# NSLab-CUK/LiteralKG

Measured on AMD Instinct MI355X. Metric: kg_edges_aggregated_per_sec, higher is better.
Workload: dtype f32

## Files before the change

### include/literalkg_hip.h

```cpp
#ifndef LITERALKG_HIP_H
#define LITERALKG_HIP_H

#include <stdint.h>

#ifdef __cplusplus
extern "C" {
#endif

typedef enum {
    LKG_OK = 0,
    LKG_ERR_INVALID_ARG = -1,
    LKG_ERR_HIP = -2,
    LKG_ERR_UNSUPPORTED = -3,
    LKG_ERR_NOMEM = -4
} lkg_status;

int lkg_version(void);
const char *lkg_last_error(void);
int lkg_preload(void);

int lkg_csr_build(int64_t n_entities, int64_t n_edges, const int64_t *h, const int64_t *t,
                  const int64_t *r, int32_t *rowptr, int32_t *col, int32_t *eptr, int32_t *rel,
                  int64_t *order, int64_t *nnz_out);

int lkg_csr_transpose(int64_t n_rows, int64_t n_cols, int64_t nnz, const int32_t *rowptr,
                      const int32_t *col, int32_t *t_rowptr, int32_t *t_col, int32_t *t_perm);

int64_t lkg_csr_build_device_workspace(int64_t n_entities, int64_t n_edges);
int lkg_csr_build_device(int64_t n_entities, int64_t n_edges, const int64_t *h, const int64_t *t, const int64_t *r,
                         int32_t *rowptr, int32_t *col, int32_t *eptr, int32_t *rel, int32_t *order,
                         int64_t *counts, void *workspace, int64_t workspace_bytes, void *stream);
int64_t lkg_csr_transpose_device_workspace(int64_t n_cols, int64_t nnz);
int lkg_csr_transpose_device(int64_t n_rows, int64_t n_cols, int64_t nnz, const int32_t *rowptr, const int32_t *col,
                             int32_t *t_rowptr, int32_t *t_col, int32_t *t_perm, void *workspace,
                             int64_t workspace_bytes, void *stream);

int lkg_csr_coo_indices_i64(int64_t n_rows, int64_t nnz, const int32_t *rowptr, const int32_t *col,
                            int64_t *indices_out, void *stream);

int lkg_row_partition(int64_t n_rows, const int32_t *rowptr, int32_t n_parts, int64_t *cuts);

int lkg_triples_count(const char *path, int64_t *n_lines);
int lkg_triples_read(const char *path, int64_t capacity, int64_t *h, int64_t *r, int64_t *t,
                     int64_t *n_read);
int lkg_triples_dedup(int64_t n, const int64_t *h, const int64_t *r, const int64_t *t, int64_t *keep,
                      int64_t *n_keep);
int lkg_laplacian_f32(int64_t n_entities, int64_t n_raw, int64_t nnz, const int32_t *rowptr,
                      const int32_t *col, const int32_t *eptr, const int32_t *rel, int32_t kind,
                      float *val_out);
int lkg_laplacian_device_f32(int64_t n_entities, int64_t nnz, int32_t n_rel, const int32_t *rowptr, const int32_t *col,
                             const int32_t *eptr, const int32_t *rel, int32_t kind, int32_t *deg_workspace,
                             float *val_out, void *stream);

int lkg_spmm_csr_f32(int64_t n_rows, int32_t d, const int32_t *rowptr, const int32_t *col,
                     const float *val, const float *x, int64_t ldx, float *out, int64_t ldo,
                     const float *self, int64_t ld_self, const int32_t *long_rows, int32_t n_long,
                     int32_t long_thresh, void *stream);

int lkg_spmm_csr_fused_f32(int64_t n_rows, int32_t d, const int32_t *rowptr, const int32_t *col,
                           const float *val, const float *x, int64_t ldx, float *out, int64_t ldo,
                           const float *self, int64_t ld_self, const float *add2, int64_t ld_add2,
                           const uint8_t *add2_rows, const float *copy_src, int64_t ld_copy_src, float *copy_dst,
                           int64_t ld_copy_dst, float *rowmax_out, const uint8_t *x_rows, const uint8_t *self_rows,
                           uint8_t *out_rows, const int32_t *long_rows, int32_t n_long, int32_t long_thresh,
                           const int32_t *rows_with_entries, int64_t n_rows_with_entries,
                           const int32_t *rows_without_entries, int64_t n_rows_without_entries, void *stream);

int lkg_csr_extract_rows(int64_t n_sel, const int64_t *sel_rows, const int32_t *rowptr, const int32_t *col,
                         const float *val, const int32_t *out_rowptr, int32_t *out_col, float *out_val,
                         void *stream);
int lkg_spmm_csr_scatter_bwd_f32(int64_t n_rows, int32_t d, const int32_t *rowptr, const int32_t *col,
                                 const float *val, const float *g_out, int64_t ldg, float *g_x,
                                 int64_t ldx, void *stream);

int lkg_edge_softmax_f32(int64_t n_rows, int64_t row_offset, int32_t d, const int32_t *rowptr,
                         const int32_t *col, const int32_t *eptr, const int32_t *rel,
                         const int32_t *rel_first, const int32_t *dup_entries,
                         const int32_t *dup_rows, int32_t n_dup, int64_t entry_lo, int64_t entry_hi,
                         const float *ent, int64_t ld_ent, const float *relemb, int64_t ld_rel,
                         float *val_out, float *logits_out, const int32_t *long_rows, int32_t n_long,
                         int32_t long_thresh, int32_t n_rel, void *stream);

int lkg_permute_f32(int64_t n, const int32_t *perm, int64_t n_src, const float *src, float *dst, void *stream);

int lkg_csr_check_i32(int64_t n_rows, const int32_t *rowptr, int64_t nnz, const int32_t *col, int64_t col_offset,
                      int64_t n_cols, int32_t *bad_out, void *stream);

int lkg_transe_score_fwd_f32(int64_t batch, int32_t dim, const float *emb, int64_t ld_emb,
                             const float *relemb, int64_t ld_rel, const int64_t *h,
                             const int64_t *r, const int64_t *pos_t, const int64_t *neg_t,
                             float *pos, float *neg, float *reg, float *rank, void *stream);

int lkg_loss_reduce_f32(int64_t batch, const float *rank, const float *reg, float lambda,
                        float *loss_out, void *stream);

int lkg_transe_score_bwd_f32(int64_t batch, int32_t dim, const float *emb, int64_t ld_emb,
                             const float *relemb, int64_t ld_rel, const int64_t *h,
                             const int64_t *r, const int64_t *pos_t, const int64_t *neg_t,
                             const float *pos, const float *neg, float lambda,
                             const float *g_loss, float *g_emb, int64_t ld_gemb, float *g_rel,
                             int64_t ld_grel, void *stream);

int lkg_group_by_key_i64(int64_t n, int32_t n_keys, const int64_t *keys, int32_t *perm, int32_t *seg,
                         int32_t *n_bad, void *stream);
int lkg_gather_rows_f32(int64_t n, int32_t d, const float *src, int64_t lds, const int64_t *idx,
                        const int32_t *perm, float *dst, int64_t ldd, void *stream);
int lkg_scatter_add_rows_f32(int64_t n, int32_t d, const float *src, int64_t lds, const int64_t *idx,
                             const int32_t *perm, float *dst, int64_t ldd, void *stream);
int lkg_fill_rows_f32(int64_t n, int32_t d, const int64_t *idx, float *dst, int64_t ldd, float value, uint8_t *flags,
                      int32_t flag, void *stream);
int lkg_gather_rows_range_f32(int64_t n, int32_t d, const float *src, int64_t lds, const int64_t *idx,
                              int64_t row_lo, int64_t row_hi, float *dst, int64_t ldd, void *stream);
int lkg_scatter_add_rows_range_f32(int64_t n, int32_t d, const float *src, int64_t lds, const int64_t *idx,
                                   int64_t row_lo, int64_t row_hi, float *dst, int64_t ldd, void *stream);
int lkg_gather_i64(int64_t n, const int64_t *src, const int32_t *perm, int64_t *dst, void *stream);

int lkg_sample_kg_batch(int64_t n_groups, int32_t neg_rate, uint64_t seed, const int64_t *heads,
                        int64_t n_entities, const int32_t *rowptr, const int32_t *col, const int32_t *eptr, const int32_t *rel,
                        int64_t nnz, int64_t n_raw, int64_t *out_h, int64_t *out_r, int64_t *out_pos_t,
                        int64_t *out_neg_t, void *stream);

int lkg_grouped_gemm_f32(int32_t mode, int32_t n_groups, const int32_t *seg, int64_t max_seg_len,
                         int32_t trans_a, int32_t trans_b, int64_t m, int64_t n, int64_t k, float alpha,
                         const float *a, int64_t lda, const float *b, int64_t ldb, int64_t stride_b,
                         int32_t b_period, float beta, float *c, int64_t ldc, int64_t stride_c, void *stream);

int lkg_dot_score_fwd_f32(int64_t batch, int32_t dim, const float *emb, int64_t ld_emb, const int64_t *h,
                          const int64_t *pos_t, const int64_t *neg_t, float *pos, float *neg, float *reg,
                          float *rank, void *stream);
int lkg_dot_score_bwd_f32(int64_t batch, int32_t dim, const float *emb, int64_t ld_emb, const int64_t *h,
                          const int64_t *pos_t, const int64_t *neg_t, const float *pos, const float *neg,
                          float lambda, const float *g_loss, float *g_emb, int64_t ld_gemb, void *stream);

int lkg_relu_batchnorm_fwd_f32(int64_t n, int32_t d, const float *z, int64_t ldz, const float *gamma,
                               const float *beta, float eps, int32_t training, float momentum,
                               float *running_mean, float *running_var, float *y, int64_t ldy,
                               float *save_mean, float *save_invstd, void *stream);
int lkg_relu_batchnorm_bwd_f32(int64_t n, int32_t d, const float *z, int64_t ldz, const float *gamma,
                               const float *save_mean, const float *save_invstd, int32_t training,
                               const float *g_y, int64_t ldgy, float *g_z, int64_t ldgz, float *g_gamma,
                               float *g_beta, void *stream);

int lkg_dense_score_fwd_f32(int64_t batch, int32_t rows_per_group, int32_t dim, const float *ph, const float *pp,
                            const float *pn, int64_t ld, const float *relemb, int64_t ld_rel,
                            const int64_t *r, float *pos, float *neg, float *reg, float *rank,
                            void *stream);
int lkg_dense_score_bwd_f32(int64_t batch, int32_t rows_per_group, int32_t dim, const float *ph, const float *pp,
                            const float *pn, int64_t ld, const float *relemb, int64_t ld_rel,
                            const int64_t *r, const float *pos, const float *neg, float lambda,
                            const float *g_loss, float *g_ph, float *g_pp, float *g_pn,
                            int64_t ldg, float *g_rel, int64_t ld_grel, void *stream);
int lkg_check_grouped_i64(int64_t n, int32_t rows_per_group, const int64_t *h, const int64_t *r,
                          const int64_t *pos_t, int32_t *n_bad, void *stream);
int lkg_expand_groups_i32(int64_t n_groups, int32_t rows_per_group, int32_t n_seg, const int32_t *perm,
                          const int32_t *seg, int32_t *perm_out, int32_t *seg_out, void *stream);

int lkg_sanitize_ids_i64(int64_t n, const int64_t *ids, int64_t lo, int64_t hi, int64_t *out, int32_t *n_bad,
                         void *stream);

int lkg_act_layernorm_fwd_f32(int64_t n, int32_t d, const float *z, int64_t ldz, float slope,
                              const float *gamma, const float *beta, float eps, float *y,
                              int64_t ldy, float *yn, int64_t ldyn, float norm_eps,
                              float *save_mean, float *save_rstd, float drop_p, uint64_t seed,
                              void *stream);

int lkg_act_layernorm_bwd_f32(int64_t n, int32_t d, const float *z, int64_t ldz, float slope,
                              const float *gamma, const float *beta, const float *y, int64_t ldy,
                              const float *save_mean, const float *save_rstd, const float *g_y,
                              int64_t ldgy, const float *g_yn, int64_t ldgyn, float norm_eps,
                              float *g_z, int64_t ldgz, float *g_gamma, float *g_beta,
                              float drop_p, uint64_t seed, float *g_z_rowmax, const uint8_t *g_yn_rows,
                              int32_t sparse_out, const int64_t *row_ids, int64_t n_row_ids, void *stream);

int lkg_gate_blend_fwd_f32(int64_t n, int32_t d, const float *x, int64_t ldx, const float *gpre,
                           int64_t ldg, const float *zpre, int64_t ldz, float *out, int64_t ldo,
                           void *stream);
int lkg_gate_blend_bwd_f32(int64_t n, int32_t d, const float *x, int64_t ldx, const float *gpre,
                           int64_t ldg, const float *zpre, int64_t ldz, const float *g_out,
                           int64_t ldgo, float *g_x, int64_t ldgx, float *g_gpre, int64_t ldgg,
                           float *g_zpre, int64_t ldgz, int32_t activated, float *g_pre_rowmax, void *stream);

int lkg_gate_blend_bwd_stats_f32(int64_t n, int32_t d, const float *x, int64_t ldx, const float *gpre, int64_t ldg,
                                 const float *zpre, int64_t ldz, const float *g_out, int64_t ldgo, float *g_x,
                                 int64_t ldgx, float *g_gpre, int64_t ldgg, float *g_zpre, int64_t ldgz,
                                 int32_t activated, float *g_pre_rowmax, const float *w, int64_t ldw, int32_t n_w,
                                 float *workspace, int64_t workspace_floats, float *stats, void *stream);

int lkg_gemm_wgrad_f32(int64_t m, int64_t n, int64_t k, const float *a, int64_t lda, const float *a_colmax,
                       const float *b, int64_t ldb, const float *b_colmax, float *c, int64_t ldc, void *stream);
int lkg_gemm_longk_ok(int64_t m, int64_t n, int64_t k, const float *a, int64_t lda, const float *b, int64_t ldb);
int lkg_gemm_longk_f32(int64_t m, int64_t n, int64_t k, const float *a, int64_t lda, const float *b, int64_t ldb,
                       float *c, int64_t ldc, void *stream);
int lkg_gemm_smallm_ok(int64_t m, int64_t n, int64_t k, const float *a, int64_t lda, const float *b, int64_t ldb);
int lkg_gemm_smallm_f32(int64_t m, int64_t n, int64_t k, const float *a, int64_t lda, const float *b, int64_t ldb,
                        float *c, int64_t ldc, void *stream);

int64_t lkg_narrow_layer_bwd_workspace(int64_t n);
int lkg_narrow_layer_bwd_ok(int64_t n, int32_t d_in, int32_t d_out, const float *x, int64_t ldx, const float *z, int64_t ldz,
                            const float *y, int64_t ldy, const float *g_y, int64_t ldgy, const float *g_yn, int64_t ldgyn);
int lkg_narrow_layer_bwd_f32(int64_t n, int32_t d_in, int32_t d_out, const float *x, int64_t ldx, const float *w, int64_t ldw,
                             const float *z, int64_t ldz, float slope, const float *gamma, const float *y, int64_t ldy,
                             const float *save_mean, const float *save_rstd, const float *g_y, int64_t ldgy,
                             const float *g_yn, int64_t ldgyn, float norm_eps, float drop_p, uint64_t seed,
                             const uint8_t *g_yn_rows, float *g_x, int64_t ldgx, float *g_w, float *g_bias,
                             float *g_gamma, float *g_beta, float *workspace, int64_t workspace_floats, void *stream);
int lkg_gemm_skinny_ok(int64_t m, int64_t n, int64_t k, const float *a, int64_t lda, const float *c, int64_t ldc);
int lkg_gemm_skinny_f32(int64_t m, int64_t n, int64_t k, const float *a, int64_t lda, const float *b, int64_t ldb,
                        int32_t trans_b, float beta, float *c, int64_t ldc, const float *bias, void *stream);
int lkg_col_absmax_f32(int64_t n, int32_t d, const float *x, int64_t ldx, float *out, void *stream);

int lkg_colsum_f32(int64_t n, int32_t d, const float *x, int64_t ldx, float *out, void *stream);
int lkg_colsum_weighted_f32(int64_t n, int32_t d, const float *x, int64_t ldx, const float *w, int64_t ldw,
                            int32_t n_w, float *out_sum, float *out_w, int64_t ld_out_w, void *stream);

int lkg_bi_mix_fwd_f32(int64_t n, int32_t d, const float *ego, int64_t lde, const float *side, int64_t lds,
                       const float *h0p, int64_t ldh, float alpha, float *out_sum, int64_t ldos, float *out_prod,
                       int64_t ldop, void *stream);
int lkg_bi_mix_bwd_f32(int64_t n, int32_t d, const float *ego, int64_t lde, const float *side, int64_t lds,
                       const float *g_sum, int64_t ldgs, const float *g_prod, int64_t ldgp, int32_t has_h0, float alpha,
                       float *g_ego, float *g_side, float *g_h0p, void *stream);

int lkg_eltwise_f32(int32_t op, int64_t n, int32_t d, const float *a, int64_t lda, const float *b,
                    int64_t ldb, float alpha, float beta, float *out, int64_t ldo, void *stream);

int lkg_adam_step_f32(int64_t n, float *param, const float *grad, float *exp_avg, float *exp_avg_sq,
                      float lr, float beta1, float beta2, float eps, float weight_decay, int64_t step,
                      void *stream);

int64_t lkg_gemm_workspace(int32_t trans_a, int64_t m, int64_t n, int64_t k);
int lkg_gemm_f32_engine(int32_t trans_a, int32_t trans_b, int64_t m, int64_t n, int64_t k, int64_t workspace_bytes);

int lkg_gemm_f64acc_f32(int32_t trans_a, int32_t trans_b, int64_t m, int64_t n, int64_t k, const float *a, int64_t lda,
                        const float *b, int64_t ldb, float *c, int64_t ldc, void *stream);
int lkg_gemm_f32(int32_t trans_a, int32_t trans_b, int64_t m, int64_t n, int64_t k, float alpha,
                 const float *a, int64_t lda, const float *b, int64_t ldb, float beta, float *c,
                 int64_t ldc, const float *bias, void *workspace, int64_t workspace_bytes, void *stream);

int lkg_row_absmax_f32(int64_t n, int32_t d, const float *x, int64_t ldx, float *out, int32_t accumulate,
                       void *stream);
int64_t lkg_gemm_tall_workspace(int32_t n, int32_t n_panels, const int32_t *ka, int32_t epilogue);
int lkg_gemm_tall_f32(int64_t m, int32_t n, int32_t n_panels, const float *const *a, const int64_t *lda,
                      const int32_t *ka, const float *a_rowmax, int32_t n_groups, const float *const *b,
                      const int64_t *ldb, int32_t trans_b, float alpha, float beta, float *c, int64_t ldc,
                      const float *bias, int32_t epilogue, const float *gate_x, int64_t ld_x, float *gate_g,
                      int64_t ld_g, float *gate_z, int64_t ld_z, void *workspace, int64_t workspace_bytes,
                      void *stream);

int64_t lkg_linear_act_layernorm_workspace(int32_t n, int32_t n_panels, const int32_t *ka);
int lkg_linear_act_layernorm_fwd_f32(int64_t m, int32_t n, int32_t n_panels, const float *const *a, const int64_t *lda,
                                     const int32_t *ka, const float *a_rowmax, const float *const *w, const int64_t *ldw,
                                     const float *bias, float slope, const float *gamma, const float *beta, float eps,
                                     float *y, int64_t ldy, float *yn, int64_t ldyn, float norm_eps, float *save_mean,
                                     float *save_rstd, float drop_p, uint64_t seed, void *workspace,
                                     int64_t workspace_bytes, void *stream);

int lkg_rank_sqnorm_f32(int64_t n, int32_t k, const float *p, int64_t ldp, float *out, void *stream);
int lkg_rank_queries_f32(int64_t n, int32_t k, const float *p, int64_t ldp, const int64_t *ids, const float *e,
                         int64_t lde, const int64_t *rel, float alpha, float *q, int64_t ldq, void *stream);
int lkg_rank_prepare_f32(int64_t n_q, int64_t n_cand, int32_t k, const float *q, int64_t ldq, const float *p,
                         int64_t ldp, const float *pn, const int64_t *truth, const int64_t *filter_row,
                         const int64_t *filter_rel, const int32_t *rowptr, const int32_t *col, const int32_t *eptr,
                         const int32_t *rel, float *thr, int32_t *better, int32_t *equal, void *stream);
int lkg_rank_count_f32(int64_t n_q, int64_t n_cand, int32_t k, const float *q, int64_t ldq, const float *p,
                       int64_t ldp, const float *pn, const float *thr, const int64_t *truth, int32_t *better,
                       int32_t *equal, void *stream);

#define LKG_TOPK_MAX 128
#define LKG_TOPK_MAX_SPLITS 64
int32_t lkg_topk_splits(int64_t n_q, int64_t n_cand, int32_t requested);
int lkg_topk_select_f32(int64_t n_q, int64_t n_cand, int32_t k, const float *q, int64_t ldq, const float *p,
                        int64_t ldp, const float *pn, const int64_t *cand_ids, const int64_t *filter_row,
                        const int64_t *filter_rel, const int32_t *rowptr, const int32_t *col, const int32_t *eptr,
                        const int32_t *rel, int32_t top_k, int32_t splits, float *ws_s, int32_t *ws_i, void *stream);
int lkg_topk_merge_f32(int64_t n_q, int32_t top_k, int32_t splits, const float *ws_s, const int32_t *ws_i,
                       const float *qn, int64_t *out_ids, float *out_scores, float *out_values, void *stream);

int lkg_accept_count_f32(int64_t n_q, int64_t n_cand, int32_t k, const float *q, int64_t ldq, const float *p,
                         int64_t ldp, const float *pn, const float *qn, const float *thr, int32_t higher,
                         const int64_t *cand_ids, const int64_t *filter_row, const int64_t *filter_rel,
                         const int32_t *rowptr, const int32_t *col, const int32_t *eptr, const int32_t *rel,
                         int32_t splits, int32_t *counts, void *stream);
int lkg_accept_emit_f32(int64_t n_q, int64_t n_cand, int32_t k, const float *q, int64_t ldq, const float *p,
                        int64_t ldp, const float *pn, const float *qn, const float *thr, int32_t higher,
                        const int64_t *cand_ids, const int64_t *filter_row, const int64_t *filter_rel,
                        const int32_t *rowptr, const int32_t *col, const int32_t *eptr, const int32_t *rel,
                        int32_t splits, const int32_t *counts, const int64_t *base, int32_t *cursor, int64_t *out_ids,
                        float *out_scores, float *out_values, int32_t *flag, void *stream);
int64_t lkg_accept_order_workspace(int64_t m, int64_t n_q);
int lkg_accept_order(int64_t m, int64_t n_q, int64_t id_bound, const int64_t *rowptr, const int64_t *ids,
                     const float *scores, const float *values, int64_t *out_ids, float *out_scores, float *out_values,
                     void *workspace, int64_t workspace_bytes, void *stream);

int lkg_pair_mlp_scores_f32(int64_t n_q, int64_t n_cand, const float *uq, int64_t ldu, const float *v, int64_t ldv,
                            const float *w2, const float *b2, const float *w3, const float *b3, float *out, int64_t ldo,
                            void *stream);
int32_t lkg_pair_mlp_splits(int64_t n_q, int64_t n_cand, int32_t requested);
int lkg_pair_mlp_select_f32(int64_t n_q, int64_t n_cand, const float *uq, int64_t ldu, const float *v, int64_t ldv,
                            const float *w2, const float *b2, const float *w3, const float *b3, const int64_t *cand_ids,
                            const int64_t *filter_row, const int64_t *filter_rel, const int32_t *rowptr,
                            const int32_t *col, const int32_t *eptr, const int32_t *rel, int32_t top_k, int32_t splits,
                            float *ws_s, int32_t *ws_i, void *stream);
int lkg_pair_mlp_prepare_f32(int64_t n_q, int64_t n_cand, const float *uq, int64_t ldu, const float *v, int64_t ldv,
                             const float *w2, const float *b2, const float *w3, const float *b3, const int64_t *truth,
                             int64_t n_rows, const int32_t *cand_slot, const int64_t *filter_row,
                             const int64_t *filter_rel, const int32_t *rowptr, const int32_t *col, const int32_t *eptr,
                             const int32_t *rel, float *thr, int32_t *better, int32_t *equal, void *stream);
int lkg_pair_mlp_count_f32(int64_t n_q, int64_t n_cand, const float *uq, int64_t ldu, const float *v, int64_t ldv,
                           const float *w2, const float *b2, const float *w3, const float *b3, const float *thr,
                           const int64_t *truth, int32_t *better, int32_t *equal, void *stream);

int lkg_pair_mlp_pairs_f32(int64_t n_pairs, const float *u, int64_t ldu, const float *v, int64_t ldv,
                           const int64_t *u_idx, const int64_t *v_idx, const float *w2, const float *b2, const float *w3,
                           const float *b3, const uint8_t *labels, float thr, float *out, int64_t *counts, void *stream);

int64_t lkg_binary_curve_workspace(int64_t n);
int lkg_binary_curve_f32(int64_t n, const float *scores, const uint8_t *labels, int64_t *out_counts, double *out_ap,
                         void *workspace, int64_t workspace_bytes, void *stream);

int lkg_triple_scores_f32(int64_t n, int32_t k, const float *p, int64_t ldp, const int64_t *q_idx, const int64_t *c_idx,
                          const float *pn, const float *e, int64_t lde, const int64_t *rel, float alpha, int32_t flags,
                          const uint8_t *labels, float thr, float *out, int64_t *counts, void *stream);

int64_t lkg_threshold_fit_workspace(int64_t n, int64_t n_relations);
int lkg_threshold_fit_f32(int64_t n, int64_t n_relations, const float *scores, const uint8_t *labels, const int64_t *rel,
                          int32_t lower_is_better, float *thr, int64_t *stats, void *workspace, int64_t workspace_bytes,
                          void *stream);

#define LKG_RELATION_MAX 4096
int lkg_relation_scores_f32(int64_t n, int32_t k, int32_t n_rel, const float *p, int64_t ldp, int64_t rel_stride,
                            const float *pn, int64_t pn_stride, const int64_t *q_idx, const int64_t *c_idx,
                            const float *e, int64_t lde, float alpha, float *out, int64_t ldo, void *stream);
int lkg_relation_order_f32(int64_t n, int32_t n_rel, const float *scores, int64_t lds, const int64_t *truth,
                           const int64_t *filter_row, const int64_t *filter_col, const int32_t *rowptr,
                           const int32_t *col, const int32_t *eptr, const int32_t *rel, int32_t top_k, int32_t *better,
                           int32_t *equal, int64_t *top_ids, float *top_scores, void *stream);

#define LKG_RETRIEVAL_SLICE 32
int lkg_retrieval_prepare_f32(int64_t n_rows, int64_t n_cand, int32_t k, const float *q, int64_t ldq,
                              const int64_t *row_q, const float *p, int64_t ldp, const float *pn, int64_t n_ids,
                              const int32_t *cand_slot, const int64_t *key_off, const int32_t *key_n,
                              const int64_t *qkey_off, const int64_t *qkey_n, const float *key_s, const int64_t *key_id,
                              const int64_t *filter_row, const int64_t *filter_rel, const int32_t *rowptr,
                              const int32_t *col, const int32_t *eptr, const int32_t *rel, int32_t *buckets,
                              void *stream);
int lkg_retrieval_count_f32(int64_t n_rows, int64_t n_cand, int32_t k, const float *q, int64_t ldq, const int64_t *row_q,
                            const float *p, int64_t ldp, const float *pn, const int64_t *cand_ids,
                            const int64_t *key_off, const int32_t *key_n, const float *key_s, const int64_t *key_id,
                            int32_t *buckets, void *stream);
int lkg_retrieval_finish(int64_t n_q, const int64_t *qkey_ptr, const int64_t *row_base, const int64_t *n_answers,
                         const int32_t *buckets, int32_t n_ks, const int64_t *ks, int64_t k_tab, const double *disc,
                         const double *icum, int64_t *before, int64_t *position, int64_t *hits, double *ndcg, double *ap,
                         double *rr, void *stream);

#define LKG_SOFTMAX_MAX_SPLITS 64
int32_t lkg_softmax_all_splits(int64_t n_q, int64_t n_cand, int32_t requested);
int lkg_softmax_all_partial_f32(int64_t n_q, int64_t n_cand, int32_t k, const float *q, int64_t ldq, const float *p,
                                int64_t ldp, const float *pn, float scale, int32_t splits, float *ws_m, float *ws_l,
                                void *stream);
int lkg_softmax_all_finish_f32(int64_t n_q, int64_t n_cand, int32_t k, const float *q, int64_t ldq, const float *p,
                               int64_t ldp, const float *pn, const int64_t *truth, float scale, int32_t splits,
                               const float *ws_m, const float *ws_l, float *lse, float *lse_lo, float *loss,
                               void *stream);
int lkg_softmax_all_weights_f32(int64_t n_q, int64_t n_cand, int32_t k, const float *q, int64_t ldq, const float *p,
                                int64_t ldp, const float *pn, int64_t c_base, const int64_t *truth, const float *lse,
                                const float *lse_lo, const float *g, float scale, float *v, int64_t ldv, void *stream);

int lkg_softmax_excluded(int64_t n_q, int64_t n_rows, int64_t n_cand, const int64_t *filter_row, const int64_t *filter_rel,
                         const int64_t *truth, const int32_t *rowptr, const int32_t *col, const int32_t *eptr,
                         const int32_t *rel, const int32_t *pos, int32_t *count, const int32_t *xptr, int32_t *xcol,
                         void *stream);
int lkg_softmax_all_partial_masked_f32(int64_t n_q, int64_t n_cand, int32_t k, const float *q, int64_t ldq, const float *p,
                                       int64_t ldp, const float *pn, float scale, int32_t splits, const int32_t *xptr,
                                       const int32_t *xcol, int64_t n_excl, float *ws_m, float *ws_l, void *stream);
int lkg_softmax_all_weights_masked_f32(int64_t n_q, int64_t n_cand, int32_t k, const float *q, int64_t ldq, const float *p,
                                       int64_t ldp, const float *pn, int64_t c_base, const int64_t *truth,
                                       const float *lse, const float *lse_lo, const float *g, float scale,
                                       const int32_t *xptr, const int32_t *xcol, int64_t n_excl, float *v, int64_t ldv,
                                       void *stream);

#ifdef __cplusplus
}
#endif
#endif
```

### literalkg_amd/_native.py

```python
import ctypes as C
import os

_LIB_PATH = os.path.join(os.path.dirname(os.path.abspath(__file__)), "lib", "liblkg_hip.so")
_lib = None

i64, i32, f32, vp, u64 = C.c_int64, C.c_int32, C.c_float, C.c_void_p, C.c_uint64

PROTOTYPES = {
    "lkg_version": [],
    "lkg_last_error": [],
    "lkg_preload": [],
    "lkg_csr_build": [i64, i64, vp, vp, vp, vp, vp, vp, vp, vp, vp],
    "lkg_csr_transpose": [i64, i64, i64, vp, vp, vp, vp, vp],
    "lkg_row_partition": [i64, vp, i32, vp],
    "lkg_csr_coo_indices_i64": [i64, i64, vp, vp, vp, vp],
    "lkg_csr_build_device_workspace": [i64, i64],
    "lkg_csr_build_device": [i64, i64, vp, vp, vp, vp, vp, vp, vp, vp, vp, vp, i64, vp],
    "lkg_csr_transpose_device_workspace": [i64, i64],
    "lkg_csr_transpose_device": [i64, i64, i64, vp, vp, vp, vp, vp, vp, i64, vp],
    "lkg_triples_count": [C.c_char_p, vp],
    "lkg_triples_read": [C.c_char_p, i64, vp, vp, vp, vp],
    "lkg_triples_dedup": [i64, vp, vp, vp, vp, vp],
    "lkg_laplacian_f32": [i64, i64, i64, vp, vp, vp, vp, i32, vp],
    "lkg_laplacian_device_f32": [i64, i64, i32, vp, vp, vp, vp, i32, vp, vp, vp],
    "lkg_spmm_csr_f32": [i64, i32, vp, vp, vp, vp, i64, vp, i64, vp, i64, vp, i32, i32, vp],
    "lkg_spmm_csr_fused_f32": [i64, i32, vp, vp, vp, vp, i64, vp, i64, vp, i64, vp, i64, vp, vp, i64, vp, i64, vp, vp,
                               vp, vp, vp, i32, i32, vp, i64, vp, i64, vp],
    "lkg_csr_extract_rows": [i64, vp, vp, vp, vp, vp, vp, vp, vp],
    "lkg_spmm_csr_scatter_bwd_f32": [i64, i32, vp, vp, vp, vp, i64, vp, i64, vp],
    "lkg_edge_softmax_f32": [i64, i64, i32, vp, vp, vp, vp, vp, vp, vp, i32, i64, i64, vp, i64, vp, i64, vp, vp, vp,
                             i32, i32, i32, vp],
    "lkg_permute_f32": [i64, vp, i64, vp, vp, vp],
    "lkg_csr_check_i32": [i64, vp, i64, vp, i64, i64, vp, vp],
    "lkg_transe_score_fwd_f32": [i64, i32, vp, i64, vp, i64, vp, vp, vp, vp, vp, vp, vp, vp, vp],
    "lkg_loss_reduce_f32": [i64, vp, vp, f32, vp, vp],
    "lkg_transe_score_bwd_f32": [i64, i32, vp, i64, vp, i64, vp, vp, vp, vp, vp, vp, f32, vp, vp, i64, vp, i64, vp],
    "lkg_group_by_key_i64": [i64, i32, vp, vp, vp, vp, vp],
    "lkg_gather_rows_f32": [i64, i32, vp, i64, vp, vp, vp, i64, vp],
    "lkg_scatter_add_rows_f32": [i64, i32, vp, i64, vp, vp, vp, i64, vp],
    "lkg_fill_rows_f32": [i64, i32, vp, vp, i64, f32, vp, i32, vp],
    "lkg_gather_i64": [i64, vp, vp, vp, vp],
    "lkg_gather_rows_range_f32": [i64, i32, vp, i64, vp, i64, i64, vp, i64, vp],
    "lkg_scatter_add_rows_range_f32": [i64, i32, vp, i64, vp, i64, i64, vp, i64, vp],
    "lkg_sample_kg_batch": [i64, i32, u64, vp, i64, vp, vp, vp, vp, i64, i64, vp, vp, vp, vp, vp],
    "lkg_grouped_gemm_f32": [i32, i32, vp, i64, i32, i32, i64, i64, i64, f32, vp, i64, vp, i64, i64, i32, f32, vp, i64,
                             i64, vp],
    "lkg_dense_score_fwd_f32": [i64, i32, i32, vp, vp, vp, i64, vp, i64, vp, vp, vp, vp, vp, vp],
    "lkg_dense_score_bwd_f32": [i64, i32, i32, vp, vp, vp, i64, vp, i64, vp, vp, vp, f32, vp, vp, vp, vp, i64, vp, i64,
                                vp],
    "lkg_check_grouped_i64": [i64, i32, vp, vp, vp, vp, vp],
    "lkg_sanitize_ids_i64": [i64, vp, i64, i64, vp, vp, vp],
    "lkg_expand_groups_i32": [i64, i32, i32, vp, vp, vp, vp, vp],
    "lkg_act_layernorm_fwd_f32": [i64, i32, vp, i64, f32, vp, vp, f32, vp, i64, vp, i64, f32, vp, vp, f32, u64, vp],
    "lkg_act_layernorm_bwd_f32": [i64, i32, vp, i64, f32, vp, vp, vp, i64, vp, vp, vp, i64, vp, i64, f32, vp, i64, vp,
                                  vp, f32, u64, vp, vp, i32, vp, i64, vp],
    "lkg_dot_score_fwd_f32": [i64, i32, vp, i64, vp, vp, vp, vp, vp, vp, vp, vp],
    "lkg_dot_score_bwd_f32": [i64, i32, vp, i64, vp, vp, vp, vp, vp, f32, vp, vp, i64, vp],
    "lkg_relu_batchnorm_fwd_f32": [i64, i32, vp, i64, vp, vp, f32, i32, f32, vp, vp, vp, i64, vp, vp, vp],
    "lkg_relu_batchnorm_bwd_f32": [i64, i32, vp, i64, vp, vp, vp, i32, vp, i64, vp, i64, vp, vp, vp],
    "lkg_gate_blend_fwd_f32": [i64, i32, vp, i64, vp, i64, vp, i64, vp, i64, vp],
    "lkg_gate_blend_bwd_f32": [i64, i32, vp, i64, vp, i64, vp, i64, vp, i64, vp, i64, vp, i64, vp, i64, i32, vp, vp],
    "lkg_gate_blend_bwd_stats_f32": [i64, i32, vp, i64, vp, i64, vp, i64, vp, i64, vp, i64, vp, i64, vp, i64, i32, vp, vp,
                                     i64, i32, vp, i64, vp, vp],
    "lkg_row_absmax_f32": [i64, i32, vp, i64, vp, i32, vp],
    "lkg_gemm_tall_workspace": [i32, i32, vp, i32],
    "lkg_gemm_tall_f32": [i64, i32, i32, vp, vp, vp, vp, i32, vp, vp, i32, f32, f32, vp, i64, vp, i32, vp, i64, vp, i64,
                          vp, i64, vp, i64, vp],
    "lkg_linear_act_layernorm_workspace": [i32, i32, vp],
    "lkg_linear_act_layernorm_fwd_f32": [i64, i32, i32, vp, vp, vp, vp, vp, vp, vp, f32, vp, vp, f32, vp, i64, vp, i64, f32,
                                         vp, vp, f32, u64, vp, i64, vp],
    "lkg_gemm_workspace": [i32, i64, i64, i64],
    "lkg_gemm_f32_engine": [i32, i32, i64, i64, i64, i64],
    "lkg_gemm_f32": [i32, i32, i64, i64, i64, f32, vp, i64, vp, i64, f32, vp, i64, vp, vp, i64, vp],
    "lkg_gemm_f64acc_f32": [i32, i32, i64, i64, i64, vp, i64, vp, i64, vp, i64, vp],
    "lkg_colsum_f32": [i64, i32, vp, i64, vp, vp],
    "lkg_col_absmax_f32": [i64, i32, vp, i64, vp, vp],
    "lkg_gemm_longk_ok": [i64, i64, i64, vp, i64, vp, i64],
    "lkg_gemm_longk_f32": [i64, i64, i64, vp, i64, vp, i64, vp, i64, vp],
    "lkg_gemm_smallm_ok": [i64, i64, i64, vp, i64, vp, i64],
    "lkg_gemm_skinny_ok": [i64, i64, i64, vp, i64, vp, i64],
    "lkg_gemm_skinny_f32": [i64, i64, i64, vp, i64, vp, i64, i32, f32, vp, i64, vp, vp],
    "lkg_gemm_smallm_f32": [i64, i64, i64, vp, i64, vp, i64, vp, i64, vp],
    "lkg_gemm_wgrad_f32": [i64, i64, i64, vp, i64, vp, vp, i64, vp, vp, i64, vp],
    "lkg_narrow_layer_bwd_ok": [i64, i32, i32, vp, i64, vp, i64, vp, i64, vp, i64, vp, i64],
    "lkg_narrow_layer_bwd_workspace": [i64],
    "lkg_narrow_layer_bwd_f32": [i64, i32, i32, vp, i64, vp, i64, vp, i64, f32, vp, vp, i64, vp, vp, vp, i64, vp, i64, f32, f32,
                                 u64, vp, vp, i64, vp, vp, vp, vp, vp, i64, vp],
    "lkg_colsum_weighted_f32": [i64, i32, vp, i64, vp, i64, i32, vp, vp, i64, vp],
    "lkg_eltwise_f32": [i32, i64, i32, vp, i64, vp, i64, f32, f32, vp, i64, vp],
    "lkg_bi_mix_fwd_f32": [i64, i32, vp, i64, vp, i64, vp, i64, f32, vp, i64, vp, i64, vp],
    "lkg_bi_mix_bwd_f32": [i64, i32, vp, i64, vp, i64, vp, i64, vp, i64, i32, f32, vp, vp, vp, vp],
    "lkg_adam_step_f32": [i64, vp, vp, vp, vp, f32, f32, f32, f32, f32, i64, vp],
    "lkg_rank_sqnorm_f32": [i64, i32, vp, i64, vp, vp],
    "lkg_rank_queries_f32": [i64, i32, vp, i64, vp, vp, i64, vp, f32, vp, i64, vp],
    "lkg_rank_prepare_f32": [i64, i64, i32, vp, i64, vp, i64, vp, vp, vp, vp, vp, vp, vp, vp, vp, vp, vp, vp],
    "lkg_rank_count_f32": [i64, i64, i32, vp, i64, vp, i64, vp, vp, vp, vp, vp, vp],
    "lkg_topk_splits": [i64, i64, i32],
    "lkg_topk_select_f32": [i64, i64, i32, vp, i64, vp, i64, vp, vp, vp, vp, vp, vp, vp, vp, i32, i32, vp, vp, vp],
    "lkg_topk_merge_f32": [i64, i32, i32, vp, vp, vp, vp, vp, vp, vp],
    "lkg_pair_mlp_scores_f32": [i64, i64, vp, i64, vp, i64, vp, vp, vp, vp, vp, i64, vp],
    "lkg_pair_mlp_splits": [i64, i64, i32],
    "lkg_pair_mlp_select_f32": [i64, i64, vp, i64, vp, i64, vp, vp, vp, vp, vp, vp, vp, vp, vp, vp, vp, i32, i32, vp, vp,
                                vp],
    "lkg_pair_mlp_prepare_f32": [i64, i64, vp, i64, vp, i64, vp, vp, vp, vp, vp, i64, vp, vp, vp, vp, vp, vp, vp, vp, vp,
                                 vp, vp],
    "lkg_pair_mlp_count_f32": [i64, i64, vp, i64, vp, i64, vp, vp, vp, vp, vp, vp, vp, vp, vp],
    "lkg_pair_mlp_pairs_f32": [i64, vp, i64, vp, i64, vp, vp, vp, vp, vp, vp, vp, f32, vp, vp, vp],
    "lkg_binary_curve_workspace": [i64],
    "lkg_binary_curve_f32": [i64, vp, vp, vp, vp, vp, i64, vp],
    "lkg_triple_scores_f32": [i64, i32, vp, i64, vp, vp, vp, vp, i64, vp, f32, i32, vp, f32, vp, vp, vp],
    "lkg_threshold_fit_workspace": [i64, i64],
    "lkg_threshold_fit_f32": [i64, i64, vp, vp, vp, i32, vp, vp, vp, i64, vp],
    "lkg_relation_scores_f32": [i64, i32, i32, vp, i64, i64, vp, i64, vp, vp, vp, i64, f32, vp, i64, vp],
    "lkg_relation_order_f32": [i64, i32, vp, i64, vp, vp, vp, vp, vp, vp, vp, i32, vp, vp, vp, vp, vp],
    "lkg_accept_count_f32": [i64, i64, i32, vp, i64, vp, i64, vp, vp, vp, i32, vp, vp, vp, vp, vp, vp, vp, i32, vp, vp],
    "lkg_accept_emit_f32": [i64, i64, i32, vp, i64, vp, i64, vp, vp, vp, i32, vp, vp, vp, vp, vp, vp, vp, i32, vp, vp, vp,
                            vp, vp, vp, vp, vp],
    "lkg_accept_order_workspace": [i64, i64],
    "lkg_accept_order": [i64, i64, i64, vp, vp, vp, vp, vp, vp, vp, vp, i64, vp],
    "lkg_retrieval_prepare_f32": [i64, i64, i32, vp, i64, vp, vp, i64, vp, i64, vp, vp, vp, vp, vp, vp, vp, vp, vp, vp, vp,
                                  vp, vp, vp, vp],
    "lkg_retrieval_count_f32": [i64, i64, i32, vp, i64, vp, vp, i64, vp, vp, vp, vp, vp, vp, vp, vp],
    "lkg_retrieval_finish": [i64, vp, vp, vp, vp, i32, vp, i64, vp, vp, vp, vp, vp, vp, vp, vp, vp],
    "lkg_softmax_all_splits": [i64, i64, i32],
    "lkg_softmax_all_partial_f32": [i64, i64, i32, vp, i64, vp, i64, vp, f32, i32, vp, vp, vp],
    "lkg_softmax_all_finish_f32": [i64, i64, i32, vp, i64, vp, i64, vp, vp, f32, i32, vp, vp, vp, vp, vp, vp],
    "lkg_softmax_all_weights_f32": [i64, i64, i32, vp, i64, vp, i64, vp, i64, vp, vp, vp, vp, f32, vp, i64, vp],
    "lkg_softmax_excluded": [i64, i64, i64, vp, vp, vp, vp, vp, vp, vp, vp, vp, vp, vp, vp],
    "lkg_softmax_all_partial_masked_f32": [i64, i64, i32, vp, i64, vp, i64, vp, f32, i32, vp, vp, i64, vp, vp, vp],
    "lkg_softmax_all_weights_masked_f32": [i64, i64, i32, vp, i64, vp, i64, vp, i64, vp, vp, vp, vp, f32, vp, vp, i64, vp,
                                           i64, vp],
}
f64 = C.c_double
EXTRA_PROTOTYPES = {
    "lkg_sigmoid_all_partial_f32": [i64, i64, i32, vp, i64, vp, i64, vp, vp, f32, f64, i32, vp, vp, i64, vp, vp],
    "lkg_sigmoid_all_finish_f32": [i64, i32, vp, vp, vp],
    "lkg_sigmoid_all_weights_f32": [i64, i64, i32, vp, i64, vp, i64, vp, vp, i64, i64, vp, f32, f64, vp, vp, i64, vp, i64,
                                    vp, vp],
}
TRAIN_PROTOTYPES = {
    "lkg_nssa_fwd_f32": [i64, i64, i32, vp, i64, vp, i64, vp, i64, i32, f32, f32, f32, vp, vp, vp, vp, vp],
    "lkg_nssa_bwd_f32": [i64, i64, i32, vp, i64, vp, i64, vp, i64, i32, f32, vp, vp, vp, vp, vp, i64, vp, i64, vp, i64, vp],
}
SAMPLE_PROTOTYPES = {
    "lkg_sample_negatives": [i64, i64, u64, i64, vp, vp, vp, i64, i64, i32, i32, i32, vp, vp, vp, vp, vp, vp, vp, vp, vp, vp,
                             vp, i64, vp, i64, vp, vp, vp, vp],
    "lkg_relation_cardinality": [i64, i64, i64, vp, vp, vp, i64, vp, vp, vp, vp, vp, vp, vp],
    "lkg_answer_counts": [i64, vp, vp, vp, i64, vp, vp, vp, vp, vp, vp, vp, vp, vp],
}
RELATION_TRAIN_PROTOTYPES = {
    "lkg_relation_loss_fwd_f32": [i64, i32, i32, vp, i64, i64, vp, i64, vp, vp, vp, vp, vp, vp, vp, f32, vp, i64, vp, vp, vp],
    "lkg_relation_loss_bwd_f32": [i64, i32, i32, vp, i64, i64, vp, i64, vp, f32, vp, vp, i64, vp, i64, vp, i64, vp],
}
ORDERED_GEMM_PROTOTYPES = {
    "lkg_gemm_ordered_splits": [i32, i32, i64, i64, i64],
    "lkg_gemm_ordered_partition": [i64, i32, vp],
    "lkg_gemm_ordered_workspace": [i64, i64, i64, i32],
    "lkg_gemm_ordered_f32": [i32, i32, i64, i64, i64, i32, f32, vp, i64, vp, i64, f32, vp, i64, vp, vp, i64, vp],
}
_RESTYPE = {"lkg_last_error": C.c_char_p, "lkg_csr_build_device_workspace": C.c_int64,
            "lkg_gemm_tall_workspace": C.c_int64, "lkg_gemm_workspace": C.c_int64,
            "lkg_linear_act_layernorm_workspace": C.c_int64, "lkg_narrow_layer_bwd_workspace": C.c_int64,
            "lkg_csr_transpose_device_workspace": C.c_int64, "lkg_binary_curve_workspace": C.c_int64,
            "lkg_threshold_fit_workspace": C.c_int64, "lkg_accept_order_workspace": C.c_int64,
            "lkg_gemm_ordered_splits": C.c_int32, "lkg_gemm_ordered_partition": C.c_int64,
            "lkg_gemm_ordered_workspace": C.c_int64}


class LkgError(RuntimeError):
    pass


def lib_path():
    return _LIB_PATH


def load():
    global _lib
    if _lib is not None:
        return _lib
    if not os.path.exists(_LIB_PATH):
        raise LkgError(
            f"{_LIB_PATH} is missing: the HIP extension has not been built. Run "
            "`python -c 'import __graft_entry__ as g; g.build()'` (or `python -m literalkg_amd.build`). "
            "literalkg_amd has no CPU fallback.")
    lib = C.CDLL(_LIB_PATH)
    for name, argtypes in list(PROTOTYPES.items()) + list(EXTRA_PROTOTYPES.items()) + list(TRAIN_PROTOTYPES.items()) + \
            list(SAMPLE_PROTOTYPES.items()) + list(RELATION_TRAIN_PROTOTYPES.items()) + \
            list(ORDERED_GEMM_PROTOTYPES.items()):
        fn = getattr(lib, name)
        fn.argtypes = argtypes
        fn.restype = _RESTYPE.get(name, C.c_int)
    _lib = lib
    return lib


_preloaded = False


def preload():
    global _preloaded
    if _preloaded:
        return
    import torch
    if not torch.cuda.is_initialized():
        return
    _preloaded = True
    lib = load()
    if lib.lkg_preload() != 0:
        msg = lib.lkg_last_error()
        raise LkgError(f"lkg_preload failed: {msg.decode() if msg else '?'}")


def call(name, *args):
    lib = load()
    if not _preloaded:
        preload()
    rc = getattr(lib, name)(*args)
    if rc != 0:
        msg = lib.lkg_last_error()
        raise LkgError(f"{name} failed ({rc}): {msg.decode() if msg else '?'}")


_empty_stand_ins = {}


def ptr(t):
    if t is None:
        return None
    if hasattr(t, "data_ptr"):
        p = t.data_ptr()
        if p == 0 and t.numel() == 0:
            key = str(t.device)
            if key not in _empty_stand_ins:
                import torch
                _empty_stand_ins[key] = torch.zeros(64, dtype=torch.float32, device=t.device)
            p = _empty_stand_ins[key].data_ptr()
        return p
    return t.ctypes.data
```

### literalkg_amd/build.py

```python
import hashlib
import os
import shutil
import subprocess
import sys
from concurrent.futures import ThreadPoolExecutor

HERE = os.path.dirname(os.path.abspath(__file__))
CSRC = os.path.join(HERE, "csrc")
LIB = os.path.join(HERE, "lib", "liblkg_hip.so")
OBJ = os.path.join(HERE, "lib", "obj")
SOURCES = ["lkg_graph_host.cpp", "lkg_spmm.hip", "lkg_attention.hip", "lkg_score.hip", "lkg_rowwise.hip",
           "lkg_gemm.hip", "lkg_batch.hip", "lkg_csr_device.hip", "lkg_gemm_tall.hip", "lkg_gemm_wgrad.hip", "lkg_layer.hip",
           "lkg_rank.hip", "lkg_topk.hip", "lkg_pairmlp.hip", "lkg_triples.hip", "lkg_relations.hip",
           "lkg_accept.hip", "lkg_retrieval.hip", "lkg_softmax.hip", "lkg_kvsall.hip", "lkg_nssa.hip", "lkg_negatives.hip",
           "lkg_relation_loss.hip", "lkg_gemm_ordered.hip"]
FLAGS = ["-O3", "--offload-arch=gfx950", "-fPIC", "-std=c++17"]


def _headers():
    return [os.path.join(CSRC, f) for f in sorted(os.listdir(CSRC)) if f.endswith(".h")] + \
           [os.path.join(HERE, "..", "include", h) for h in ("literalkg_hip.h", "literalkg_hip_ext.h", "literalkg_hip_train.h",
                                                                "literalkg_hip_sample.h", "literalkg_hip_relation_train.h",
                                                                "literalkg_hip_gemm_ordered.h")]


TAG_FILE = os.path.join(HERE, "lib", "flags.tag")


def _stale(tag):
    if not os.path.exists(LIB):
        return True
    if os.path.exists(TAG_FILE) and open(TAG_FILE).read().strip() != tag:
        return True
    t = os.path.getmtime(LIB)
    deps = [os.path.join(CSRC, f) for f in os.listdir(CSRC)] + _headers()
    return any(os.path.getmtime(d) > t for d in deps)


def _flag_tag(extra):
    return hashlib.sha256(" ".join(FLAGS + extra).encode()).hexdigest()[:12]


def build(force=False, verbose=True):
    extra = os.environ.get("LKG_EXTRA_HIPCC_FLAGS", "").split()
    tag = _flag_tag(extra)
    if not force and not _stale(tag):
        return LIB
    hipcc = shutil.which("hipcc") or "/opt/rocm/bin/hipcc"
    if not os.path.exists(hipcc):
        raise RuntimeError("hipcc not found: cannot build literalkg_amd/lib/liblkg_hip.so")
    os.makedirs(OBJ, exist_ok=True)
    newest_header = max(os.path.getmtime(h) for h in _headers())
    todo, objs = [], []
    for s in SOURCES:
        src = os.path.join(CSRC, s)
        obj = os.path.join(OBJ, f"{os.path.splitext(s)[0]}.{tag}.o")
        objs.append(obj)
        if force or not os.path.exists(obj) or os.path.getmtime(obj) < max(os.path.getmtime(src), newest_header):
            todo.append((src, obj))

    def compile_one(job):
        src, obj = job
        cmd = [hipcc] + FLAGS + extra + ["-c", src, "-o", obj]
        if verbose:
            print(" ".join(cmd), file=sys.stderr)
        subprocess.run(cmd, check=True)

    workers = max(1, min(len(todo), int(os.environ.get("LKG_BUILD_JOBS", "6"))))
    if todo:
        with ThreadPoolExecutor(workers) as pool:
            list(pool.map(compile_one, todo))
    cmd = [hipcc, "--offload-arch=gfx950", "-fPIC", "-shared", "-o", LIB] + objs
    if verbose:
        print(" ".join(cmd), file=sys.stderr)
    subprocess.run(cmd, check=True)
    with open(TAG_FILE, "w") as f:
        f.write(tag + "\n")
    return LIB


if __name__ == "__main__":
    build(force="--force" in sys.argv)
```

### literalkg_amd/csrc/lkg_gemm_wgrad.hip

```cpp
#include <algorithm>
#include <cstdlib>
#include <type_traits>

#include "lkg_common.h"

namespace {

constexpr int BM = 128, BN = 128, BK = 16, PLANE = BM * BK;
typedef _Float16 f16x8 __attribute__((ext_vector_type(8)));
typedef __fp16 fp16x2 __attribute__((ext_vector_type(2)));
typedef float f32x16 __attribute__((ext_vector_type(16)));
typedef short s16x4 __attribute__((ext_vector_type(4)));
typedef short s16x8 __attribute__((ext_vector_type(8)));

struct WgArgs {
    const float *a, *b;
    long lda, ldb;
    const float *a_colmax, *b_colmax;
    float *c;
    long ldc;
    long m, n, k;
    int tiles_m, tiles_n, k_splits;
    int a_aligned, b_aligned;
};

__device__ __forceinline__ int kmajor_off(int k, int c) {
    return k * BM + ((((c >> 5) ^ (k & 3)) << 5) | (c & 31));
}
__device__ __forceinline__ f16x8 kmajor_frag(const _Float16 *plane, int c0, int lane) {
    const int q = (lane & 15) >> 2, pp = lane & 3;
    const int col = c0 + (lane & 16) + 4 * pp;
    const int k0 = 8 * (lane >> 5) + q;
    typedef __attribute__((address_space(3))) s16x4 lds_s16x4;
    const s16x4 lo = __builtin_amdgcn_ds_read_tr16_b64_v4i16((lds_s16x4 *)(plane + kmajor_off(k0, col)));
    const s16x4 hi = __builtin_amdgcn_ds_read_tr16_b64_v4i16((lds_s16x4 *)(plane + kmajor_off(k0 + 4, col)));
    const s16x8 both = __builtin_shufflevector(lo, hi, 0, 1, 2, 3, 4, 5, 6, 7);
    return __builtin_bit_cast(f16x8, both);
}

__device__ __forceinline__ void split_store(const float (&v)[8], const int *exp8, _Float16 *planes, int t) {
    typedef __fp16 fp16x8 __attribute__((ext_vector_type(8)));
    fp16x8 hv, mv;
    const int4 s0 = *reinterpret_cast<const int4 *>(exp8), s1 = *reinterpret_cast<const int4 *>(exp8 + 4);
    const int sc[8] = {s0.x, s0.y, s0.z, s0.w, s1.x, s1.y, s1.z, s1.w};
#pragma unroll
    for (int j = 0; j < 8; j += 2) {
        const float a0 = ldexpf(v[j], sc[j]), a1 = ldexpf(v[j + 1], sc[j + 1]);
        const fp16x2 h = __builtin_amdgcn_cvt_pkrtz(a0, a1);
        const fp16x2 m = __builtin_amdgcn_cvt_pkrtz((a0 - (float)h[0]) * 2048.f, (a1 - (float)h[1]) * 2048.f);
        hv[j] = h[0]; hv[j + 1] = h[1];
        mv[j] = m[0]; mv[j + 1] = m[1];
    }
    _Float16 *p = planes + kmajor_off(t >> 4, (t & 15) * 8);
    *reinterpret_cast<fp16x8 *>(p) = hv;
    *reinterpret_cast<fp16x8 *>(p + PLANE) = mv;
}

__global__ __launch_bounds__(256) __attribute__((amdgpu_waves_per_eu(3, 3))) void wgrad_f16x2_kernel(WgArgs g) {
    __shared__ __attribute__((aligned(16))) _Float16 smem[2][2][2 * PLANE];
    const int t = threadIdx.x, lane = t & 63, wave = t >> 6;
    const int wm = wave >> 1, wn = wave & 1;
    const int tiles = g.tiles_m * g.tiles_n;
    const int xcd = blockIdx.x & 7, slot = blockIdx.x >> 3;
    const int split = (slot / tiles) * 8 + xcd, tile = slot % tiles;
    if (split >= g.k_splits) return;
    const int tm = tile / g.tiles_n, tn = tile % g.tiles_n;
    const long m0 = (long)tm * BM, n0 = (long)tn * BN;
    const long per = ((g.k + g.k_splits - 1) / g.k_splits + BK - 1) / BK * BK;
    const long k_lo = (long)split * per, k_hi = min(g.k, k_lo + per);
    if (k_lo >= k_hi) return;

    const int kr = t >> 4, c8 = (t & 15) * 8;
    __shared__ __attribute__((aligned(16))) int scale_s[2][BM];
    if (t < BM) scale_s[0][t] = scale_exponent(g.a_colmax[min(m0 + t, g.m - 1)]);
    else scale_s[1][t - BM] = scale_exponent(g.b_colmax[min(n0 + t - BM, g.n - 1)]);
    __syncthreads();

    f32x16 acc[2][2];
#pragma unroll
    for (int i = 0; i < 2; ++i)
#pragma unroll
        for (int j = 0; j < 2; ++j)
#pragma unroll
            for (int r = 0; r < 16; ++r) acc[i][j][r] = 0.f;

    float la[8], lb[8];
    auto load8 = [&](float (&v)[8], const float *src, long ld, long c0, long c_end, long k, bool fast) {
        if (fast) {
            const float4 *p = reinterpret_cast<const float4 *>(src + k * ld + c0 + c8);
            const float4 x0 = p[0], x1 = p[1];
            v[0] = x0.x; v[1] = x0.y; v[2] = x0.z; v[3] = x0.w; v[4] = x1.x; v[5] = x1.y; v[6] = x1.z; v[7] = x1.w;
        } else {
            const float *row = src + min(k, k_hi - 1) * ld;
#pragma unroll
            for (int j = 0; j < 8; ++j) {
                const float x = row[min(c0 + c8 + j, c_end - 1)];
                v[j] = (k < k_hi && c0 + c8 + j < c_end) ? x : 0.f;
            }
        }
    };
    auto stage = [&](_Float16 (*D)[2 * PLANE]) {
        split_store(la, scale_s[0] + c8, D[0], t);
        __builtin_amdgcn_sched_barrier(0);
        split_store(lb, scale_s[1] + c8, D[1], t);
    };
    auto mma = [&](const _Float16 (*S)[2 * PLANE]) {
        f16x8 ah[2], am[2], bh[2], bm[2];
#pragma unroll
        for (int i = 0; i < 2; ++i) {
            ah[i] = kmajor_frag(S[0], wm * 64 + i * 32, lane);
            bh[i] = kmajor_frag(S[1], wn * 64 + i * 32, lane);
        }
#pragma unroll
        for (int i = 0; i < 2; ++i)
#pragma unroll
            for (int j = 0; j < 2; ++j) acc[i][j] = __builtin_amdgcn_mfma_f32_32x32x16_f16(ah[i], bh[j], acc[i][j], 0, 0, 0);
        const _Float16 sc = (_Float16)(1.f / 2048.f);
#pragma unroll
        for (int i = 0; i < 2; ++i) {
            bm[i] = kmajor_frag(S[1] + PLANE, wn * 64 + i * 32, lane);
            ah[i] = ah[i] * sc;
        }
#pragma unroll
        for (int i = 0; i < 2; ++i)
#pragma unroll
            for (int j = 0; j < 2; ++j) acc[i][j] = __builtin_amdgcn_mfma_f32_32x32x16_f16(ah[i], bm[j], acc[i][j], 0, 0, 0);
#pragma unroll
        for (int i = 0; i < 2; ++i) {
            am[i] = kmajor_frag(S[0] + PLANE, wm * 64 + i * 32, lane);
            bh[i] = bh[i] * sc;
        }
#pragma unroll
        for (int i = 0; i < 2; ++i)
#pragma unroll
            for (int j = 0; j < 2; ++j) acc[i][j] = __builtin_amdgcn_mfma_f32_32x32x16_f16(am[i], bh[j], acc[i][j], 0, 0, 0);
    };
    auto pipeline = [&](auto fast_tag) {
        constexpr int FAST = decltype(fast_tag)::value;
        auto fetch = [&](long tile_k) {
            const long k = k_lo + tile_k * BK + kr;
            load8(la, g.a, g.lda, m0, g.m, k, (FAST & 2) != 0);
            load8(lb, g.b, g.ldb, n0, g.n, k, (FAST & 1) != 0);
            __builtin_amdgcn_sched_barrier(0);
        };
        const long count = (k_hi - k_lo + BK - 1) / BK;
        fetch(0);
        stage(smem[0]);
        fetch(min(1L, count - 1));
        for (long it = 0; it < count; ++it) {
            __syncthreads();
            stage(smem[(it + 1) & 1]);
            fetch(min(it + 2, count - 1));
            mma(smem[it & 1]);
        }
    };
    const bool a_fast = g.a_aligned && m0 + BM <= g.m, b_fast = g.b_aligned && n0 + BN <= g.n;
    if (a_fast && b_fast) pipeline(std::integral_constant<int, 3>{});
    else if (a_fast) pipeline(std::integral_constant<int, 2>{});
    else if (b_fast) pipeline(std::integral_constant<int, 1>{});
    else pipeline(std::integral_constant<int, 0>{});

    const bool atomic_out = g.k_splits > 1;
#pragma unroll
    for (int i = 0; i < 2; ++i)
#pragma unroll
        for (int j = 0; j < 2; ++j) {
            const long col = n0 + wn * 64 + j * 32 + (lane & 31);
            const long row0 = m0 + wm * 64 + i * 32 + 4 * (lane >> 5);
            if (col >= g.n) continue;
            const int ecol = scale_exponent(g.b_colmax[col]);
#pragma unroll
            for (int r = 0; r < 16; ++r) {
                const long row = row0 + (r & 3) + 8 * (r >> 2);
                if (row >= g.m) continue;
                const float v = ldexpf(acc[i][j][r], -(scale_exponent(g.a_colmax[row]) + ecol));
                if (atomic_out) atomicAdd(g.c + row * g.ldc + col, v);
                else g.c[row * g.ldc + col] = v;
            }
        }
}

__global__ __launch_bounds__(256) void col_absmax_kernel(long n, int d, const float *__restrict__ x, long ldx,
                                                          int *__restrict__ out, long rows_per_block) {
    const long r0 = (long)blockIdx.x * rows_per_block, r1 = min(n, r0 + rows_per_block);
    for (int c = threadIdx.x; c < d; c += blockDim.x) {
        float m0 = 0.f, m1 = 0.f, m2 = 0.f, m3 = 0.f;
        long r = r0;
        for (; r + 4 <= r1; r += 4) {
            m0 = fmaxf(m0, fabsf(x[r * ldx + c]));
            m1 = fmaxf(m1, fabsf(x[(r + 1) * ldx + c]));
            m2 = fmaxf(m2, fabsf(x[(r + 2) * ldx + c]));
            m3 = fmaxf(m3, fabsf(x[(r + 3) * ldx + c]));
        }
        for (; r < r1; ++r) m0 = fmaxf(m0, fabsf(x[r * ldx + c]));
        atomicMax(out + c, __float_as_int(fmaxf(fmaxf(m0, m1), fmaxf(m2, m3))));
    }
}

}

extern "C" int lkg_col_absmax_f32(int64_t n, int32_t d, const float *x, int64_t ldx, float *out, void *stream) {
    LKG_REQUIRE(n >= 0 && d > 0 && ldx >= d && out, "lkg_col_absmax_f32: bad arguments");
    hipStream_t s = (hipStream_t)stream;
    if (hipMemsetAsync(out, 0, sizeof(float) * d, s) != hipSuccess) {
        lkg_set_error("lkg_col_absmax_f32: hipMemsetAsync failed");
        return LKG_ERR_HIP;
    }
    if (n == 0) return LKG_OK;
    LKG_REQUIRE(x, "lkg_col_absmax_f32: null pointer");
    const long blocks = std::min<int64_t>((n + 63) / 64, 2048);
    const long rpb = (n + blocks - 1) / blocks;
    hipLaunchKernelGGL(col_absmax_kernel, dim3((unsigned)blocks), dim3(256), 0, s, (long)n, d, x, (long)ldx,
                       reinterpret_cast<int *>(out), rpb);
    LKG_CHECK_LAUNCH("lkg_col_absmax_f32");
    return LKG_OK;
}

extern "C" int lkg_gemm_longk_ok(int64_t m, int64_t n, int64_t k, const float *a, int64_t lda, const float *b, int64_t ldb);
static int longk_launch(bool f16, int64_t m, int64_t n, int64_t k, const float *a, int64_t lda, const float *a_colmax,
                        const float *b, int64_t ldb, const float *b_colmax, float *c, int64_t ldc, hipStream_t s);

extern "C" int lkg_gemm_wgrad_f32(int64_t m, int64_t n, int64_t k, const float *a, int64_t lda, const float *a_colmax,
                                  const float *b, int64_t ldb, const float *b_colmax, float *c, int64_t ldc,
                                  void *stream) {
    LKG_REQUIRE(m >= 0 && n >= 0 && k >= 0, "lkg_gemm_wgrad_f32: negative size");
    if (m == 0 || n == 0) return LKG_OK;
    LKG_REQUIRE(c && ldc >= n, "lkg_gemm_wgrad_f32: bad C (ldc=%lld, n=%lld)", (long long)ldc, (long long)n);
    if (a && b && a_colmax && b_colmax && lda >= m && ldb >= n && lkg_gemm_longk_ok(m, n, k, a, lda, b, ldb))
        return longk_launch(true, m, n, k, a, lda, a_colmax, b, ldb, b_colmax, c, ldc, (hipStream_t)stream);
    hipStream_t s = (hipStream_t)stream;
    WgArgs g{};
    g.a = a; g.b = b; g.lda = lda; g.ldb = ldb; g.a_colmax = a_colmax; g.b_colmax = b_colmax; g.c = c; g.ldc = ldc;
    g.m = m; g.n = n; g.k = k;
    g.tiles_m = (int)((m + BM - 1) / BM);
    g.tiles_n = (int)((n + BN - 1) / BN);
    const long tiles = (long)g.tiles_m * g.tiles_n;
    LKG_REQUIRE(tiles < INT32_MAX, "lkg_gemm_wgrad_f32: too many tiles");
    int splits = 1;
    if (tiles < 256 && k >= 8192) splits = (int)std::max<long>(1, std::min<long>(std::min<long>(1024 / tiles, k / 2048), 65535));
    g.k_splits = splits;
    if (splits > 1 || k == 0) {
        const hipError_t rc = ldc == n ? hipMemsetAsync(c, 0, sizeof(float) * m * n, s)
                                       : hipMemset2DAsync(c, sizeof(float) * ldc, 0, sizeof(float) * n, m, s);
        if (rc != hipSuccess) {
            lkg_set_error("lkg_gemm_wgrad_f32: hipMemsetAsync failed");
            return LKG_ERR_HIP;
        }
        if (k == 0) return LKG_OK;
    }
    LKG_REQUIRE(a && b && a_colmax && b_colmax && lda >= m && ldb >= n, "lkg_gemm_wgrad_f32: null operand / leading dimension too small");
    g.a_aligned = k % BK == 0 && lda % 4 == 0 && lkg_aligned16(a);
    g.b_aligned = k % BK == 0 && ldb % 4 == 0 && lkg_aligned16(b);
    const long groups = ((long)splits + 7) / 8;
    LKG_REQUIRE(groups * tiles * 8 < INT32_MAX, "lkg_gemm_wgrad_f32: grid too large");
    hipLaunchKernelGGL(wgrad_f16x2_kernel, dim3((unsigned)(groups * tiles * 8)), dim3(256), 0, s, g);
    LKG_CHECK_LAUNCH("lkg_gemm_wgrad_f32");
    return LKG_OK;
}


namespace {

typedef __bf16 bf16x8 __attribute__((ext_vector_type(8)));
typedef __bf16 bf16x4 __attribute__((ext_vector_type(4)));
typedef __bf16 bf16x2 __attribute__((ext_vector_type(2)));
typedef float f32x2 __attribute__((ext_vector_type(2)));
typedef float f32x4 __attribute__((ext_vector_type(4)));
constexpr int RM = 256, RN = 128, RK = 16;
constexpr int RA_PLANE = RM * RK, RB_PLANE = RN * RK;
constexpr int RBUF = 3 * (RA_PLANE + RB_PLANE);

template <int COLS>
__device__ __forceinline__ int roff(int k, int c) {
    return k * COLS + ((((c >> 5) ^ (k & 3)) << 5) | (c & 31));
}
template <int COLS>
__device__ __forceinline__ bf16x8 rfrag(const __bf16 *plane, int c0, int lane) {
    const int q = (lane & 15) >> 2, pp = lane & 3;
    const int col = c0 + (lane & 16) + 4 * pp;
    const int k0 = 8 * (lane >> 5) + q;
    typedef __attribute__((address_space(3))) s16x4 lds_s16x4;
    const s16x4 lo = __builtin_amdgcn_ds_read_tr16_b64_v4i16((lds_s16x4 *)(plane + roff<COLS>(k0, col)));
    const s16x4 hi = __builtin_amdgcn_ds_read_tr16_b64_v4i16((lds_s16x4 *)(plane + roff<COLS>(k0 + 4, col)));
    const s16x8 both = __builtin_shufflevector(lo, hi, 0, 1, 2, 3, 4, 5, 6, 7);
    return __builtin_bit_cast(bf16x8, both);
}

__global__ __launch_bounds__(512) __attribute__((amdgpu_waves_per_eu(2, 2))) void wgrad_longk_kernel(WgArgs g) {
    extern __shared__ __attribute__((aligned(16))) unsigned char longk_smem[];
    __bf16 *planes = reinterpret_cast<__bf16 *>(longk_smem);

    const int t = threadIdx.x, lane = t & 63, wave = t >> 6;
    const int wm = wave >> 1, wn = wave & 1;
    const int tiles = g.tiles_m * g.tiles_n;
    const int xcd = blockIdx.x & 7, slot = blockIdx.x >> 3;
    const int split = (slot / tiles) * 8 + xcd, tile = slot % tiles;
    if (split >= g.k_splits) return;
    const int tm = tile / g.tiles_n, tn = tile % g.tiles_n;
    const long m0 = (long)tm * RM, n0 = (long)tn * RN;
    const long per = ((g.k + g.k_splits - 1) / g.k_splits + RK - 1) / RK * RK;
    const long k_lo = (long)split * per, k_hi = min(g.k, k_lo + per);
    if (k_lo >= k_hi) return;
    const int count = (int)((k_hi - k_lo) / RK);

    const int ka = t >> 6, ca = 4 * (t & 63), kb = t >> 5, cb = 4 * (t & 31);
    const int keep_a = (m0 + ca + 3 < g.m) ? -1 : 0, keep_b = (n0 + cb + 3 < g.n) ? -1 : 0;
    const float *pa0 = g.a + (k_lo + ka) * g.lda + min(m0 + ca, g.m - 4);
// ... 43 lines not shown
    auto write_piece = [&](int p, __bf16 *D) {
        __bf16 *plane0 = p == 2 ? D + 3 * RA_PLANE : D;
        const int pe = p == 2 ? RB_PLANE : RA_PLANE, off = p == 0 ? off_a0 : (p == 1 ? off_a1 : off_b);
        const bf16x4 h = {ph[2 * p][0], ph[2 * p][1], ph[2 * p + 1][0], ph[2 * p + 1][1]};
        const bf16x4 m = {pm[2 * p][0], pm[2 * p][1], pm[2 * p + 1][0], pm[2 * p + 1][1]};
        const bf16x4 l = {pl[2 * p][0], pl[2 * p][1], pl[2 * p + 1][0], pl[2 * p + 1][1]};
        *reinterpret_cast<bf16x4 *>(plane0 + off) = h;
        *reinterpret_cast<bf16x4 *>(plane0 + pe + off) = m;
        *reinterpret_cast<bf16x4 *>(plane0 + 2 * pe + off) = l;
    };
    auto slice = [&](f32x4 (&r)[3], int i, __bf16 *D, int live) {
        if (i == 21) { fetch(r); return; }
        if (i > 21) return;
        const int p = i / 7, rr = i % 7;
        if (rr < 2) s1(r, 2 * p + rr, live);
        else if (rr < 4) s2(2 * p + rr - 2);
        else if (rr < 6) s3(2 * p + rr - 4);
        else write_piece(p, D);
    };
#define LKG_PIN() __builtin_amdgcn_sched_barrier(0)
#define LKG_MF(I, J, PA, PB) acc[I][J] = __builtin_amdgcn_mfma_f32_32x32x16_bf16(a[I][PA], b[J][PB], acc[I][J], 0, 0, 0)
#define LKG_TERM4(PA, PB, S0)                                                                                       \
    LKG_MF(0, 0, PA, PB); slice(r, S0, D, live); LKG_PIN(); LKG_MF(0, 1, PA, PB); slice(r, S0 + 1, D, live); LKG_PIN();  \
    LKG_MF(1, 0, PA, PB); slice(r, S0 + 2, D, live); LKG_PIN(); LKG_MF(1, 1, PA, PB); slice(r, S0 + 3, D, live); LKG_PIN();
    auto step = [&](const __bf16 *S, __bf16 *D, f32x4 (&r)[3], int live) {
        const __bf16 *SA = S, *SB = S + 3 * RA_PLANE;
        bf16x8 a[2][3], b[2][3];
#pragma unroll
        for (int i = 0; i < 2; ++i) {
            a[i][2] = rfrag<RM>(SA + 2 * RA_PLANE, wm * 64 + i * 32, lane);
            b[i][0] = rfrag<RN>(SB, wn * 64 + i * 32, lane);
        }
#pragma unroll
        for (int i = 0; i < 2; ++i) {
            a[i][0] = rfrag<RM>(SA, wm * 64 + i * 32, lane);
            b[i][2] = rfrag<RN>(SB + 2 * RB_PLANE, wn * 64 + i * 32, lane);
            a[i][1] = rfrag<RM>(SA + RA_PLANE, wm * 64 + i * 32, lane);
            b[i][1] = rfrag<RN>(SB + RB_PLANE, wn * 64 + i * 32, lane);
        }
        LKG_PIN();
        LKG_TERM4(2, 0, 0)
        LKG_TERM4(0, 2, 4)
        LKG_TERM4(1, 1, 8)
        LKG_TERM4(1, 0, 12)
        LKG_TERM4(0, 1, 16)
        LKG_TERM4(0, 0, 20)
    };
#undef LKG_TERM4
#undef LKG_MF
#undef LKG_PIN

    fetch(rs0);
    fetch(rs1);
    fetch(rs2);
    for (int i = 0; i < 21; ++i) slice(rs0, i, planes, -1);
    fetch(rs0);
    auto P = [&](int j) { return planes + (j & 1) * RBUF; };
    for (int it = 0; it < count; it += 3) {
        __syncthreads();
        step(P(it), P(it + 1), rs1, it + 1 < count ? -1 : 0);
        __syncthreads();
        step(P(it + 1), P(it + 2), rs2, it + 2 < count ? -1 : 0);
        __syncthreads();
        step(P(it + 2), P(it + 3), rs0, it + 3 < count ? -1 : 0);
    }

    const bool atomic_out = g.k_splits > 1;
#pragma unroll
    for (int i = 0; i < 2; ++i)
#pragma unroll
        for (int j = 0; j < 2; ++j) {
            const long col = n0 + wn * 64 + j * 32 + (lane & 31);
            const long row0 = m0 + wm * 64 + i * 32 + 4 * (lane >> 5);
            if (col >= g.n) continue;
#pragma unroll
            for (int r = 0; r < 16; ++r) {
                const long row = row0 + (r & 3) + 8 * (r >> 2);
                if (row >= g.m) continue;
                if (atomic_out) atomicAdd(g.c + row * g.ldc + col, acc[i][j][r]);
                else g.c[row * g.ldc + col] = acc[i][j][r];
            }
        }
}

}

namespace {
constexpr int HBUF = 2 * (RA_PLANE + RB_PLANE);

__global__ __launch_bounds__(512) __attribute__((amdgpu_waves_per_eu(2, 2))) void wgrad_longk_f16_kernel(WgArgs g) {
    extern __shared__ __attribute__((aligned(16))) unsigned char longk_smem[];
    _Float16 *planes = reinterpret_cast<_Float16 *>(longk_smem);
    typedef __fp16 fp16x4 __attribute__((ext_vector_type(4)));

    const int t = threadIdx.x, lane = t & 63, wave = t >> 6;
    const int tiles = g.tiles_m * g.tiles_n;
    const int xcd = blockIdx.x & 7, slot = blockIdx.x >> 3;
    const int split = (slot / tiles) * 8 + xcd, tile = slot % tiles;
    if (split >= g.k_splits) return;
    const int tm = tile / g.tiles_n, tn = tile % g.tiles_n;
    const long m0 = (long)tm * RM, n0 = (long)tn * RN;
    const long per = ((g.k + g.k_splits - 1) / g.k_splits + RK - 1) / RK * RK;
    const long k_lo = (long)split * per, k_hi = min(g.k, k_lo + per);
    if (k_lo >= k_hi) return;
    const int count = (int)((k_hi - k_lo) / RK);
    const int m_live = (int)min(4l, (g.m - m0 + 63) / 64), n_live = (int)min(2l, (g.n - n0 + 63) / 64);
    const int wave_u = __builtin_amdgcn_readfirstlane(wave);
    const bool by_cols = n_live == 1;
    const int wm = by_cols ? (wave & 3) : (wave >> 1), wn = by_cols ? (wave >> 2) : (wave & 1);
    const bool wave_live = (by_cols ? (wave_u & 3) : (wave_u >> 1)) < m_live && (by_cols ? (wave_u >> 2) : (wave_u & 1)) < n_live;

    const int ka = t >> 6, ca = 4 * (t & 63), kb = t >> 5, cb = 4 * (t & 31);
    const int keep_a = (m0 + ca + 3 < g.m) ? -1 : 0, keep_b = (n0 + cb + 3 < g.n) ? -1 : 0;
    const float *pa0 = g.a + (k_lo + ka) * g.lda + min(m0 + ca, g.m - 4);
    const float *pa1 = pa0 + 8 * g.lda;
    const float *pb = g.b + (k_lo + kb) * g.ldb + min(n0 + cb, g.n - 4);
    const long step_a = RK * g.lda, step_b = RK * g.ldb;
    int sa[4], sb[4];
#pragma unroll
    for (int j = 0; j < 4; ++j) {
        sa[j] = scale_exponent(g.a_colmax[min(m0 + ca + j, g.m - 1)]);
        sb[j] = scale_exponent(g.b_colmax[min(n0 + cb + j, g.n - 1)]);
    }

    f32x16 acc[2][2];
#pragma unroll
    for (int i = 0; i < 2; ++i)
#pragma unroll
        for (int j = 0; j < 2; ++j)
#pragma unroll
            for (int r = 0; r < 16; ++r) acc[i][j][r] = 0.f;

    f32x4 rs0[3], rs1[3], rs2[3];
    int fetched = 0;
    auto fetch = [&](f32x4 (&r)[3]) {
        r[0] = *reinterpret_cast<const f32x4 *>(pa0);
        r[1] = *reinterpret_cast<const f32x4 *>(pa1);
        r[2] = *reinterpret_cast<const f32x4 *>(pb);
        ++fetched;
        const bool more = fetched < count;
        pa0 += more ? step_a : 0;
        pa1 += more ? step_a : 0;
        pb += more ? step_b : 0;
    };
    float px[6][2];
    fp16x2 ph[6], pm[6];
    auto t1 = [&](const f32x4 (&r)[3], int q, int live) {
        const f32x4 v = r[q >> 1];
        const bool isb = (q >> 1) == 2;
        const int keep = (isb ? keep_b : keep_a) & live, e0 = 2 * (q & 1);
        px[q][0] = ldexpf(__int_as_float(__float_as_int(v[e0]) & keep), isb ? sb[e0] : sa[e0]);
        px[q][1] = ldexpf(__int_as_float(__float_as_int(v[e0 + 1]) & keep), isb ? sb[e0 + 1] : sa[e0 + 1]);
        ph[q] = __builtin_amdgcn_cvt_pkrtz(px[q][0], px[q][1]);
    };
    auto t2 = [&](int q) {
        pm[q] = __builtin_amdgcn_cvt_pkrtz((px[q][0] - (float)ph[q][0]) * 2048.f, (px[q][1] - (float)ph[q][1]) * 2048.f);
    };
    const int off_a0 = roff<RM>(ka, ca), off_a1 = roff<RM>(ka + 8, ca), off_b = roff<RN>(kb, cb);
    auto write_piece = [&](int p, _Float16 *D) {
        _Float16 *plane0 = p == 2 ? D + 2 * RA_PLANE : D;
        const int pe = p == 2 ? RB_PLANE : RA_PLANE, off = p == 0 ? off_a0 : (p == 1 ? off_a1 : off_b);
        const fp16x4 h = {ph[2 * p][0], ph[2 * p][1], ph[2 * p + 1][0], ph[2 * p + 1][1]};
        const fp16x4 m = {pm[2 * p][0], pm[2 * p][1], pm[2 * p + 1][0], pm[2 * p + 1][1]};
        *reinterpret_cast<fp16x4 *>(plane0 + off) = h;
        *reinterpret_cast<fp16x4 *>(plane0 + pe + off) = m;
    };
#define LKG_PIN() __builtin_amdgcn_sched_barrier(0)
#define LKG_MF(C, A_, B_) C = __builtin_amdgcn_mfma_f32_32x32x16_f16(A_, B_, C, 0, 0, 0)
    auto hfrag = [&](const _Float16 *plane, int cols, int c0) {
        return cols == RM ? __builtin_bit_cast(f16x8, rfrag<RM>(reinterpret_cast<const __bf16 *>(plane), c0, lane))
                          : __builtin_bit_cast(f16x8, rfrag<RN>(reinterpret_cast<const __bf16 *>(plane), c0, lane));
    };
    auto step = [&](const _Float16 *S, _Float16 *D, f32x4 (&r)[3], int live, auto LIVE) {
        if constexpr (!decltype(LIVE)::value) {
#pragma unroll
            for (int q = 0; q < 6; ++q) { t1(r, q, live); t2(q); }
#pragma unroll
            for (int p = 0; p < 3; ++p) write_piece(p, D);
            fetch(r);
            return;
        }
        const _Float16 *SA = S, *SB = S + 2 * RA_PLANE;
        f16x8 ah[2], am[2], bh[2], bm[2], ahs[2], bhs[2];
#pragma unroll
        for (int i = 0; i < 2; ++i) {
            ah[i] = hfrag(SA, RM, wm * 64 + i * 32);
            bh[i] = hfrag(SB, RN, wn * 64 + i * 32);
        }
#pragma unroll
        for (int i = 0; i < 2; ++i) {
            bm[i] = hfrag(SB + RB_PLANE, RN, wn * 64 + i * 32);
            am[i] = hfrag(SA + RA_PLANE, RM, wm * 64 + i * 32);
        }
        const _Float16 sc = (_Float16)(1.f / 2048.f);
        LKG_PIN();
        LKG_MF(acc[0][0], ah[0], bh[0]); ahs[0] = ah[0] * sc; t1(r, 0, live); LKG_PIN();
        LKG_MF(acc[0][1], ah[0], bh[1]); ahs[1] = ah[1] * sc; t1(r, 1, live); LKG_PIN();
        LKG_MF(acc[1][0], ah[1], bh[0]); t1(r, 2, live); t1(r, 3, live); LKG_PIN();
        LKG_MF(acc[1][1], ah[1], bh[1]); t1(r, 4, live); t1(r, 5, live); LKG_PIN();
        LKG_MF(acc[0][0], ahs[0], bm[0]); bhs[0] = bh[0] * sc; t2(0); LKG_PIN();
        LKG_MF(acc[0][1], ahs[0], bm[1]); bhs[1] = bh[1] * sc; t2(1); LKG_PIN();
        LKG_MF(acc[1][0], ahs[1], bm[0]); t2(2); write_piece(0, D); LKG_PIN();
        LKG_MF(acc[1][1], ahs[1], bm[1]); t2(3); LKG_PIN();
        LKG_MF(acc[0][0], am[0], bhs[0]); t2(4); write_piece(1, D); LKG_PIN();
        LKG_MF(acc[0][1], am[0], bhs[1]); t2(5); LKG_PIN();
        LKG_MF(acc[1][0], am[1], bhs[0]); write_piece(2, D); LKG_PIN();
        LKG_MF(acc[1][1], am[1], bhs[1]); fetch(r);
    };
#undef LKG_MF
#undef LKG_PIN

    fetch(rs0);
    fetch(rs1);
    fetch(rs2);
    for (int q = 0; q < 6; ++q) { t1(rs0, q, -1); t2(q); }
    for (int p = 0; p < 3; ++p) write_piece(p, planes);
    fetch(rs0);
    auto P = [&](int j) { return planes + (j & 1) * HBUF; };
    auto k_loop = [&](auto LIVE) {
        for (int it = 0; it < count; it += 3) {
            __syncthreads();
            step(P(it), P(it + 1), rs1, it + 1 < count ? -1 : 0, LIVE);
            __syncthreads();
            step(P(it + 1), P(it + 2), rs2, it + 2 < count ? -1 : 0, LIVE);
            __syncthreads();
            step(P(it + 2), P(it + 3), rs0, it + 3 < count ? -1 : 0, LIVE);
        }
    };
    if (wave_live) k_loop(std::true_type{});
    else { k_loop(std::false_type{}); return; }

    const bool atomic_out = g.k_splits > 1;
#pragma unroll
    for (int i = 0; i < 2; ++i)
#pragma unroll
        for (int j = 0; j < 2; ++j) {
            const long col = n0 + wn * 64 + j * 32 + (lane & 31);
            const long row0 = m0 + wm * 64 + i * 32 + 4 * (lane >> 5);
            if (col >= g.n) continue;
            const int ecol = scale_exponent(g.b_colmax[col]);
#pragma unroll
            for (int r = 0; r < 16; ++r) {
                const long row = row0 + (r & 3) + 8 * (r >> 2);
                if (row >= g.m) continue;
                const float v = ldexpf(acc[i][j][r], -(scale_exponent(g.a_colmax[row]) + ecol));
                if (atomic_out) atomicAdd(g.c + row * g.ldc + col, v);
                else g.c[row * g.ldc + col] = v;
            }
        }
}
}

extern "C" int lkg_gemm_longk_ok(int64_t m, int64_t n, int64_t k, const float *a, int64_t lda, const float *b, int64_t ldb) {
    return k >= 8192 && k % RK == 0 && m >= 4 && n >= 4 && m % 4 == 0 && n % 4 == 0 && lda % 4 == 0 && ldb % 4 == 0 &&
           lkg_aligned16(a) && lkg_aligned16(b);
}

static int longk_launch(bool f16, int64_t m, int64_t n, int64_t k, const float *a, int64_t lda, const float *a_colmax,
                        const float *b, int64_t ldb, const float *b_colmax, float *c, int64_t ldc, hipStream_t s) {
    WgArgs g{};
    g.a = a; g.b = b; g.lda = lda; g.ldb = ldb; g.a_colmax = a_colmax; g.b_colmax = b_colmax; g.c = c; g.ldc = ldc;
    g.m = m; g.n = n; g.k = k;
    g.tiles_m = (int)((m + RM - 1) / RM);
    g.tiles_n = (int)((n + RN - 1) / RN);
    const long tiles = (long)g.tiles_m * g.tiles_n;
    LKG_REQUIRE(tiles < 65536, "lkg_gemm_longk_f32: too many tiles");
    int splits = (int)std::max<long>(1, std::min<long>((512 + tiles - 1) / tiles, k / 1024));
    g.k_splits = splits;
    if (splits > 1) {
        const hipError_t rc = ldc == n ? hipMemsetAsync(c, 0, sizeof(float) * m * n, s)
                                       : hipMemset2DAsync(c, sizeof(float) * ldc, 0, sizeof(float) * n, m, s);
        if (rc != hipSuccess) {
            lkg_set_error("lkg_gemm_longk_f32: hipMemsetAsync failed");
            return LKG_ERR_HIP;
        }
    }
    const int lds = (f16 ? HBUF : RBUF) * 2 * 2;
    static bool raised[2] = {false, false};
    if (!raised[f16]) {
        const void *fn = f16 ? reinterpret_cast<const void *>(wgrad_longk_f16_kernel) : reinterpret_cast<const void *>(wgrad_longk_kernel);
        if (hipFuncSetAttribute(fn, hipFuncAttributeMaxDynamicSharedMemorySize, lds) != hipSuccess) {
            lkg_set_error("lkg_gemm_longk_f32: cannot raise the dynamic LDS limit");
            return LKG_ERR_HIP;
        }
        raised[f16] = true;
    }
    const long groups = ((long)splits + 7) / 8;
    if (f16) hipLaunchKernelGGL(wgrad_longk_f16_kernel, dim3((unsigned)(groups * tiles * 8)), dim3(512), lds, s, g);
    else hipLaunchKernelGGL(wgrad_longk_kernel, dim3((unsigned)(groups * tiles * 8)), dim3(512), lds, s, g);
    LKG_CHECK_LAUNCH("lkg_gemm_longk_f32");
    return LKG_OK;
}

extern "C" int lkg_gemm_longk_f32(int64_t m, int64_t n, int64_t k, const float *a, int64_t lda, const float *b, int64_t ldb,
                                  float *c, int64_t ldc, void *stream) {
    LKG_REQUIRE(m > 0 && n > 0 && k > 0 && a && b && c && ldc >= n && lda >= m && ldb >= n, "lkg_gemm_longk_f32: bad arguments");
    LKG_REQUIRE(lkg_gemm_longk_ok(m, n, k, a, lda, b, ldb), "lkg_gemm_longk_f32: needs k >= 8192 in whole 16-row tiles, widths and "
                "row strides that are multiples of 4 floats and 16-byte aligned operands (lkg_gemm_longk_ok)");
    return longk_launch(false, m, n, k, a, lda, nullptr, b, ldb, nullptr, c, ldc, (hipStream_t)stream);
}

namespace {

template <int MT>
__global__ __launch_bounds__(256) void smallm_wgrad_kernel(long m, long n, long k, const float *__restrict__ a, long lda,
                                                            const float *__restrict__ b, long ldb, float *__restrict__ c,
                                                            long ldc, long rows_per_block) {
    constexpr int RM_ = MT / 16;
    constexpr int R = 32;
    __shared__ __attribute__((aligned(16))) float as[R][MT], bs[R][64];
    const int t = threadIdx.x;
    const int bi = t >> 4, bj = t & 15;
    const long n0 = (long)blockIdx.y * 64;
    const long k_lo = (long)blockIdx.x * rows_per_block, k_hi = min(k, k_lo + rows_per_block);
    if (k_lo >= k_hi) return;
    float acc[RM_][4];
#pragma unroll
    for (int i = 0; i < RM_; ++i)
#pragma unroll
        for (int j = 0; j < 4; ++j) acc[i][j] = 0.f;
    constexpr int APIECES = R * MT / 4, A_PER_ROW = MT / 4, NA = APIECES / 256, NB = 2;
    float4 ra[NA], rb[NB];
    auto load_tile = [&](long k0) {
#pragma unroll
        for (int q = 0; q < NA; ++q) {
            const int p = t + 256 * q, r = p / A_PER_ROW, cq = (p % A_PER_ROW) * 4;
            const long row = min(k0 + r, k_hi - 1);
            const bool on = k0 + r < k_hi && cq < m;
            const float4 v = *reinterpret_cast<const float4 *>(a + row * lda + (cq < m ? cq : 0));
            ra[q] = on ? v : make_float4(0.f, 0.f, 0.f, 0.f);
        }
#pragma unroll
        for (int q = 0; q < NB; ++q) {
            const int p = t + 256 * q, r = p >> 4, cq = (p & 15) * 4;
            const long row = min(k0 + r, k_hi - 1);
            const bool on = k0 + r < k_hi && n0 + cq < n;
            const float4 v = *reinterpret_cast<const float4 *>(b + row * ldb + (n0 + cq < n ? n0 + cq : 0));
            rb[q] = on ? v : make_float4(0.f, 0.f, 0.f, 0.f);
        }
    };
    auto store_tile = [&]() {
#pragma unroll
        for (int q = 0; q < NA; ++q) {
            const int p = t + 256 * q;
            *reinterpret_cast<float4 *>(&as[p / A_PER_ROW][(p % A_PER_ROW) * 4]) = ra[q];
        }
#pragma unroll
        for (int q = 0; q < NB; ++q) {
            const int p = t + 256 * q;
            *reinterpret_cast<float4 *>(&bs[p >> 4][(p & 15) * 4]) = rb[q];
        }
    };
    load_tile(k_lo);
    store_tile();
    __syncthreads();
    for (long k0 = k_lo; k0 < k_hi; k0 += R) {
        const bool more = k0 + R < k_hi;
        if (more) load_tile(k0 + R);
#pragma unroll 8
        for (int r = 0; r < R; ++r) {
            const float4 bv = *reinterpret_cast<const float4 *>(&bs[r][4 * bj]);
            float av[RM_];
            if constexpr (RM_ == 4) {
                const float4 x = *reinterpret_cast<const float4 *>(&as[r][4 * bi]);
                av[0] = x.x; av[1] = x.y; av[2] = x.z; av[3] = x.w;
            } else {
                const float2 x = *reinterpret_cast<const float2 *>(&as[r][2 * bi]);
                av[0] = x.x; av[1] = x.y;
            }
#pragma unroll
            for (int i = 0; i < RM_; ++i) {
                acc[i][0] = fmaf(av[i], bv.x, acc[i][0]);
                acc[i][1] = fmaf(av[i], bv.y, acc[i][1]);
                acc[i][2] = fmaf(av[i], bv.z, acc[i][2]);
                acc[i][3] = fmaf(av[i], bv.w, acc[i][3]);
            }
        }
        __syncthreads();
        if (more) store_tile();
        __syncthreads();
    }
#pragma unroll
    for (int i = 0; i < RM_; ++i) {
        const long row = RM_ * bi + i;
        if (row >= m) continue;
#pragma unroll
        for (int j = 0; j < 4; ++j) {
            const long col = n0 + 4 * bj + j;
            if (col < n) atomicAdd(c + row * ldc + col, acc[i][j]);
        }
    }
}

}

extern "C" int lkg_gemm_smallm_ok(int64_t m, int64_t n, int64_t k, const float *a, int64_t lda, const float *b, int64_t ldb) {
    return k >= 4096 && m >= 4 && m <= 64 && n >= 4 && m % 4 == 0 && n % 4 == 0 && lda % 4 == 0 && ldb % 4 == 0 &&
           lkg_aligned16(a) && lkg_aligned16(b);
}

extern "C" int lkg_gemm_smallm_f32(int64_t m, int64_t n, int64_t k, const float *a, int64_t lda, const float *b, int64_t ldb,
                                   float *c, int64_t ldc, void *stream) {
    LKG_REQUIRE(m > 0 && n > 0 && k > 0 && a && b && c && ldc >= n && lda >= m && ldb >= n, "lkg_gemm_smallm_f32: bad arguments");
    LKG_REQUIRE(lkg_gemm_smallm_ok(m, n, k, a, lda, b, ldb), "lkg_gemm_smallm_f32: needs m <= 64, k >= 4096, widths and row "
                "strides that are multiples of 4 floats and 16-byte aligned operands (lkg_gemm_smallm_ok)");
    hipStream_t s = (hipStream_t)stream;
    const hipError_t rc = ldc == n ? hipMemsetAsync(c, 0, sizeof(float) * m * n, s)
                                   : hipMemset2DAsync(c, sizeof(float) * ldc, 0, sizeof(float) * n, m, s);
    if (rc != hipSuccess) {
        lkg_set_error("lkg_gemm_smallm_f32: hipMemsetAsync failed");
        return LKG_ERR_HIP;
    }
    const int64_t chunks = (n + 63) / 64;
    static const int64_t target = getenv("LKG_SMALLM_BLOCKS") ? atoll(getenv("LKG_SMALLM_BLOCKS")) : 768;
    int64_t blocks = std::max<int64_t>(1, std::min<int64_t>(target / chunks + 1, k / 256));
    int64_t per = ((k + blocks - 1) / blocks + 31) / 32 * 32;
    blocks = (k + per - 1) / per;
    const dim3 grid((unsigned)blocks, (unsigned)chunks);
    if (m <= 32)
        hipLaunchKernelGGL((smallm_wgrad_kernel<32>), grid, dim3(256), 0, s, (long)m, (long)n, (long)k, a, (long)lda, b, (long)ldb,
                           c, (long)ldc, (long)per);
    else
        hipLaunchKernelGGL((smallm_wgrad_kernel<64>), grid, dim3(256), 0, s, (long)m, (long)n, (long)k, a, (long)lda, b, (long)ldb,
                           c, (long)ldc, (long)per);
    LKG_CHECK_LAUNCH("lkg_gemm_smallm_f32");
    return LKG_OK;
}

namespace {

template <int CPT>
__global__ __launch_bounds__(256) void skinny_gemm_kernel(long m, int n, int k, const float *__restrict__ a, long lda,
                                                           const float *__restrict__ b, long ldb, int trans_b, float beta,
                                                           float *__restrict__ c, long ldc, const float *__restrict__ bias) {
    constexpr int KP = 68;
    __shared__ __attribute__((aligned(16))) float ws[64][4 * CPT], xs[64][KP];
    const int t = threadIdx.x;
    const int r = t >> 2, cg = t & 3;
    for (int i = t; i < k * 4 * CPT; i += 256) {
        const int kk = i / (4 * CPT), col = i % (4 * CPT);
        ws[kk][col] = col < n ? (trans_b ? b[(long)col * ldb + kk] : b[(long)kk * ldb + col]) : 0.f;
    }
    float bv[CPT];
#pragma unroll
    for (int j = 0; j < CPT; ++j) bv[j] = (bias && cg * CPT + j < n) ? bias[cg * CPT + j] : 0.f;
    const int k4 = k >> 2;
    for (long m0 = (long)blockIdx.x * 64; m0 < m; m0 += (long)gridDim.x * 64) {
        __syncthreads();
        for (int p = t; p < 64 * k4; p += 256) {
            const int rr = p / k4, q = p % k4;
            const long row = min(m0 + rr, m - 1);
            *reinterpret_cast<float4 *>(&xs[rr][4 * q]) = *reinterpret_cast<const float4 *>(a + row * lda + 4 * q);
        }
        __syncthreads();
        float acc[CPT];
#pragma unroll
        for (int j = 0; j < CPT; ++j) acc[j] = bv[j];
        for (int q = 0; q < k4; ++q) {
            const float4 xv = *reinterpret_cast<const float4 *>(&xs[r][4 * q]);
            const float xe[4] = {xv.x, xv.y, xv.z, xv.w};
#pragma unroll
            for (int e = 0; e < 4; ++e)
#pragma unroll
                for (int j = 0; j < CPT; j += 4) {
                    const float4 wv = *reinterpret_cast<const float4 *>(&ws[4 * q + e][cg * CPT + j]);
                    acc[j] = fmaf(xe[e], wv.x, acc[j]);
                    acc[j + 1] = fmaf(xe[e], wv.y, acc[j + 1]);
                    acc[j + 2] = fmaf(xe[e], wv.z, acc[j + 2]);
                    acc[j + 3] = fmaf(xe[e], wv.w, acc[j + 3]);
                }
        }
        const long row = m0 + r;
        if (row < m) {
            float *dst = c + row * ldc + cg * CPT;
#pragma unroll
            for (int j = 0; j < CPT; j += 4) {
                if (cg * CPT + j >= n) break;
                float4 o = make_float4(acc[j], acc[j + 1], acc[j + 2], acc[j + 3]);
                if (beta != 0.f) {
                    const float4 old = *reinterpret_cast<const float4 *>(dst + j);
                    o.x = fmaf(beta, old.x, o.x); o.y = fmaf(beta, old.y, o.y); o.z = fmaf(beta, old.z, o.z); o.w = fmaf(beta, old.w, o.w);
                }
                *reinterpret_cast<float4 *>(dst + j) = o;
            }
        }
    }
}

}

extern "C" int lkg_gemm_skinny_ok(int64_t m, int64_t n, int64_t k, const float *a, int64_t lda, const float *c, int64_t ldc) {
    return m >= 4096 && k >= 4 && k <= 64 && n >= 4 && n <= 64 && k % 4 == 0 && n % 4 == 0 && lda % 4 == 0 && ldc % 4 == 0 &&
           lkg_aligned16(a) && lkg_aligned16(c);
}

extern "C" int lkg_gemm_skinny_f32(int64_t m, int64_t n, int64_t k, const float *a, int64_t lda, const float *b, int64_t ldb,
                                   int32_t trans_b, float beta, float *c, int64_t ldc, const float *bias, void *stream) {
    LKG_REQUIRE(m > 0 && a && b && c && lda >= k && ldc >= n && ldb >= (trans_b ? k : n), "lkg_gemm_skinny_f32: bad arguments");
    LKG_REQUIRE(lkg_gemm_skinny_ok(m, n, k, a, lda, c, ldc), "lkg_gemm_skinny_f32: needs m >= 4096, k and n <= 64 in multiples "
                "of 4 and 16-byte aligned rows (lkg_gemm_skinny_ok)");
    hipStream_t s = (hipStream_t)stream;
    const unsigned blocks = (unsigned)std::min<int64_t>((m + 63) / 64, 256 * 8);
#define LKG_SKINNY(CPT_)                                                                                                    \
    hipLaunchKernelGGL((skinny_gemm_kernel<CPT_>), dim3(blocks), dim3(256), 0, s, (long)m, (int)n, (int)k, a, (long)lda, b,  \
                       (long)ldb, (int)trans_b, beta, c, (long)ldc, bias)
    if (n <= 16) LKG_SKINNY(4);
    else if (n <= 32) LKG_SKINNY(8);
    else if (n <= 48) LKG_SKINNY(12);
    else LKG_SKINNY(16);
#undef LKG_SKINNY
    LKG_CHECK_LAUNCH("lkg_gemm_skinny_f32");
    return LKG_OK;
}

int lkg_internal_preload_gemm_wgrad() {
    hipFuncAttributes attr;
    return hipFuncGetAttributes(&attr, reinterpret_cast<const void *>(&wgrad_f16x2_kernel)) == hipSuccess ? 0 : 1;
}
```

### literalkg_amd/csrc/lkg_graph_host.cpp

```cpp
#include <fcntl.h>
#include <sys/mman.h>
#include <sys/stat.h>
#include <unistd.h>

#include <algorithm>
#include <atomic>
#include <cerrno>
#include <cmath>
#include <cstdlib>
#include <cstring>
#include <new>
#include <thread>
#include <vector>

#include "lkg_common.h"

static thread_local char g_err[512] = "";

void lkg_set_error(const char *fmt, ...) {
    va_list ap;
    va_start(ap, fmt);
    vsnprintf(g_err, sizeof(g_err), fmt, ap);
    va_end(ap);
}

extern "C" const char *lkg_last_error(void) { return g_err; }
extern "C" int lkg_version(void) { return 100;  }

int lkg_internal_preload_spmm();
int lkg_internal_preload_attention();
int lkg_internal_preload_batch();
int lkg_internal_preload_csr_device();
int lkg_internal_preload_gemm();
int lkg_internal_preload_gemm_tall();
int lkg_internal_preload_gemm_wgrad();
int lkg_internal_preload_rowwise();
int lkg_internal_preload_score();
int lkg_internal_preload_layer();
int lkg_internal_preload_rank();
int lkg_internal_preload_topk();
int lkg_internal_preload_pairmlp();
int lkg_internal_preload_triples();
int lkg_internal_preload_relations();
int lkg_internal_preload_accept();
int lkg_internal_preload_retrieval();
int lkg_internal_preload_softmax();
int lkg_internal_preload_kvsall();
int lkg_internal_preload_nssa();
int lkg_internal_preload_negatives();
int lkg_internal_preload_relation_loss();
int lkg_internal_preload_gemm_ordered();

extern "C" int lkg_preload(void) {
    const int failed = lkg_internal_preload_spmm() + lkg_internal_preload_attention() + lkg_internal_preload_batch() + lkg_internal_preload_csr_device() + lkg_internal_preload_gemm() + lkg_internal_preload_gemm_tall() + lkg_internal_preload_gemm_wgrad() + lkg_internal_preload_rowwise() + lkg_internal_preload_score() + lkg_internal_preload_layer() + lkg_internal_preload_rank() + lkg_internal_preload_topk() + lkg_internal_preload_pairmlp() + lkg_internal_preload_triples() + lkg_internal_preload_relations() + lkg_internal_preload_accept() + lkg_internal_preload_retrieval() + lkg_internal_preload_softmax() + lkg_internal_preload_kvsall() + lkg_internal_preload_nssa() + lkg_internal_preload_negatives() + lkg_internal_preload_relation_loss() + lkg_internal_preload_gemm_ordered();
    if (failed) {
        lkg_set_error("lkg_preload: %d of the library's code objects could not be loaded on the current device", failed);
        return LKG_ERR_HIP;
    }
    return LKG_OK;
}

namespace {
template <class F>
void parallel_rows(int64_t n, F &&fn) {
    unsigned hw = std::thread::hardware_concurrency();
    int nt = (int)std::min<int64_t>(std::max(1u, std::min(hw, 32u)), std::max<int64_t>(1, n / 65536));
    if (nt <= 1) {
        fn(0, n);
        return;
    }
    std::vector<std::thread> th;
    int64_t step = (n + nt - 1) / nt;
    for (int i = 0; i < nt; ++i) {
        int64_t lo = i * step, hi = std::min(n, lo + step);
        if (lo < hi) th.emplace_back([=, &fn] { fn(lo, hi); });
    }
    for (auto &x : th) x.join();
}
}

extern "C" int lkg_csr_build(int64_t n_entities, int64_t n_edges, const int64_t *h,
                             const int64_t *t, const int64_t *r, int32_t *rowptr, int32_t *col,
                             int32_t *eptr, int32_t *rel, int64_t *order, int64_t *nnz_out) {
    LKG_REQUIRE(n_entities >= 0 && n_entities < INT32_MAX, "lkg_csr_build: n_entities %lld out of int32 range",
                (long long)n_entities);
    LKG_REQUIRE(n_edges >= 0 && n_edges < INT32_MAX, "lkg_csr_build: n_edges %lld out of int32 range",
                (long long)n_edges);
    LKG_REQUIRE(rowptr && nnz_out && (n_edges == 0 || (h && t && col && eptr && rel && order)),
                "lkg_csr_build: null pointer");
    for (int64_t e = 0; e < n_edges; ++e) {
        if ((uint64_t)h[e] >= (uint64_t)n_entities || (uint64_t)t[e] >= (uint64_t)n_entities) {
            lkg_set_error("lkg_csr_build: edge %lld (%lld -> %lld) outside [0, %lld)", (long long)e,
                          (long long)h[e], (long long)t[e], (long long)n_entities);
            return LKG_ERR_INVALID_ARG;
        }
        if (r && (r[e] < 0 || r[e] > INT32_MAX)) {
            lkg_set_error("lkg_csr_build: relation id %lld of edge %lld out of range", (long long)r[e],
                          (long long)e);
            return LKG_ERR_INVALID_ARG;
        }
    }
    std::vector<int64_t> start;
    try {
        start.assign((size_t)n_entities + 1, 0);
    } catch (...) {
        lkg_set_error("lkg_csr_build: out of host memory");
        return LKG_ERR_NOMEM;
    }
    for (int64_t e = 0; e < n_edges; ++e) start[h[e] + 1]++;
    for (int64_t i = 0; i < n_entities; ++i) start[i + 1] += start[i];
    {
        std::vector<int64_t> pos(start.begin(), start.end() - 1);
        for (int64_t e = 0; e < n_edges; ++e) order[pos[h[e]]++] = e;
    }
    parallel_rows(n_entities, [&](int64_t lo, int64_t hi) {
        for (int64_t i = lo; i < hi; ++i) {
            int64_t a = start[i], b = start[i + 1];
            if (b - a > 1)
                std::stable_sort(order + a, order + b, [&](int64_t x, int64_t y) { return t[x] < t[y]; });
        }
    });
    int64_t nnz = 0;
    for (int64_t i = 0; i < n_entities; ++i) {
        rowptr[i] = (int32_t)nnz;
        int64_t prev_t = -1;
        for (int64_t k = start[i]; k < start[i + 1]; ++k) {
            int64_t e = order[k];
            rel[k] = r ? (int32_t)r[e] : 0;
            if (t[e] != prev_t) {
                col[nnz] = (int32_t)t[e];
                eptr[nnz] = (int32_t)k;
                ++nnz;
                prev_t = t[e];
            }
        }
    }
    rowptr[n_entities] = (int32_t)nnz;
    if (eptr) eptr[nnz] = (int32_t)n_edges;
    *nnz_out = nnz;
    return LKG_OK;
}

extern "C" int lkg_csr_transpose(int64_t n_rows, int64_t n_cols, int64_t nnz, const int32_t *rowptr,
                                 const int32_t *col, int32_t *t_rowptr, int32_t *t_col,
                                 int32_t *t_perm) {
    LKG_REQUIRE(n_rows >= 0 && n_cols >= 0 && nnz >= 0 && nnz < INT32_MAX, "lkg_csr_transpose: bad sizes");
    LKG_REQUIRE(rowptr && t_rowptr && (nnz == 0 || (col && t_col && t_perm)), "lkg_csr_transpose: null pointer");
    LKG_REQUIRE(rowptr[n_rows] == nnz, "lkg_csr_transpose: rowptr[n_rows]=%d != nnz=%lld", rowptr[n_rows],
                (long long)nnz);
    std::vector<int32_t> pos((size_t)n_cols + 1, 0);
    for (int64_t j = 0; j < nnz; ++j) {
        if ((uint32_t)col[j] >= (uint64_t)n_cols) {
            lkg_set_error("lkg_csr_transpose: col[%lld]=%d outside [0,%lld)", (long long)j, col[j],
                          (long long)n_cols);
            return LKG_ERR_INVALID_ARG;
        }
        pos[col[j] + 1]++;
    }
    for (int64_t c = 0; c < n_cols; ++c) pos[c + 1] += pos[c];
    std::memcpy(t_rowptr, pos.data(), sizeof(int32_t) * ((size_t)n_cols + 1));
    for (int64_t i = 0; i < n_rows; ++i)
        for (int32_t j = rowptr[i]; j < rowptr[i + 1]; ++j) {
            int32_t p = pos[col[j]]++;
            t_col[p] = (int32_t)i;
            t_perm[p] = j;
        }
    return LKG_OK;
}

extern "C" int lkg_row_partition(int64_t n_rows, const int32_t *rowptr, int32_t n_parts, int64_t *cuts) {
    LKG_REQUIRE(n_rows >= 0 && n_parts >= 1 && rowptr && cuts, "lkg_row_partition: bad arguments");
    int64_t nnz = rowptr[n_rows] - rowptr[0];
    cuts[0] = 0;
    for (int32_t p = 1; p < n_parts; ++p) {
        int64_t want = rowptr[0] + (nnz * p) / n_parts;
        const int32_t *it = std::lower_bound(rowptr, rowptr + n_rows + 1, (int32_t)want);
        int64_t row = it - rowptr;
        cuts[p] = std::max(cuts[p - 1], std::min<int64_t>(row, n_rows));
    }
    cuts[n_parts] = n_rows;
    return LKG_OK;
}

namespace {
struct Mapped {
    const char *p = nullptr;
    size_t n = 0;
    int fd = -1;
    ~Mapped() {
        if (p && n) munmap(const_cast<char *>(p), n);
        if (fd >= 0) close(fd);
    }
};

int map_file(const char *path, Mapped &m) {
    m.fd = open(path, O_RDONLY);
    if (m.fd < 0) {
        lkg_set_error("cannot open %s: %s", path, strerror(errno));
        return LKG_ERR_INVALID_ARG;
    }
    struct stat st;
    if (fstat(m.fd, &st) != 0) {
        lkg_set_error("cannot stat %s: %s", path, strerror(errno));
        return LKG_ERR_INVALID_ARG;
    }
    m.n = (size_t)st.st_size;
    if (m.n == 0) return LKG_OK;
    void *a = mmap(nullptr, m.n, PROT_READ, MAP_PRIVATE, m.fd, 0);
    if (a == MAP_FAILED) {
        m.n = 0;
        lkg_set_error("cannot mmap %s: %s", path, strerror(errno));
        return LKG_ERR_NOMEM;
    }
    m.p = (const char *)a;
    return LKG_OK;
}

inline bool parse_line(const char *&c, const char *end, int64_t out[3], bool &bad) {
    while (c < end && (*c == ' ' || *c == '\t' || *c == '\r')) ++c;
    if (c >= end || *c == '\n') {
        if (c < end) ++c;
        return false;
    }
    for (int f = 0; f < 3; ++f) {
        while (c < end && (*c == ' ' || *c == '\t')) ++c;
        bool neg = false;
        if (c < end && *c == '-') {
            neg = true;
            ++c;
        }
        if (c >= end || *c < '0' || *c > '9') {
            bad = true;
            return false;
        }
        int64_t v = 0;
        while (c < end && *c >= '0' && *c <= '9') v = v * 10 + (*c++ - '0');
        out[f] = neg ? -v : v;
    }
    while (c < end && (*c == ' ' || *c == '\t' || *c == '\r')) ++c;
    if (c < end && *c != '\n') {
        bad = true;
        return false;
    }
    if (c < end) ++c;
    return true;
}
}

namespace {
std::vector<size_t> line_chunks(const Mapped &m, int n_chunks) {
    std::vector<size_t> cut((size_t)n_chunks + 1, m.n);
    cut[0] = 0;
    for (int k = 1; k < n_chunks; ++k) {
        size_t p = std::max(cut[k - 1], m.n / n_chunks * (size_t)k);
        while (p < m.n && m.p[p] != '\n') ++p;
        cut[k] = std::min(m.n, p + 1);
    }
    return cut;
}

int parser_threads(size_t bytes) {
    const unsigned hw = std::max(1u, std::thread::hardware_concurrency());
    return (int)std::max<size_t>(1, std::min<size_t>(std::min(hw, 32u), bytes / (4u << 20)));
}

int64_t parse_range(const Mapped &m, size_t lo, size_t hi, int64_t *h, int64_t *r, int64_t *t, int64_t at) {
    const char *c = m.p + lo, *end = m.p + hi;
    int64_t n = 0, v[3];
    bool bad = false;
    while (c < end) {
        if (parse_line(c, end, v, bad)) {
            if (h) {
                h[at + n] = v[0];
                r[at + n] = v[1];
                t[at + n] = v[2];
            }
            ++n;
        }
        if (bad) return -1 - (int64_t)(c - m.p);
    }
    return n;
}

void parse_chunks(const Mapped &m, const std::vector<size_t> &cut, std::vector<int64_t> &counts, int64_t *h, int64_t *r,
                  int64_t *t, const std::vector<int64_t> *offsets) {
    const int nc = (int)cut.size() - 1;
    counts.assign((size_t)nc, 0);
    std::vector<std::thread> th;
    for (int k = 0; k < nc; ++k)
        th.emplace_back([&, k] { counts[k] = parse_range(m, cut[k], cut[k + 1], h, r, t, offsets ? (*offsets)[k] : 0); });
    for (auto &x : th) x.join();
}
}

extern "C" int lkg_triples_count(const char *path, int64_t *n_lines) {
    LKG_REQUIRE(path && n_lines, "lkg_triples_count: null pointer");
    Mapped m;
    int rc = map_file(path, m);
    if (rc != LKG_OK) return rc;
    const auto cut = line_chunks(m, parser_threads(m.n));
    std::vector<int64_t> counts;
    parse_chunks(m, cut, counts, nullptr, nullptr, nullptr, nullptr);
    int64_t n = 0;
    for (int64_t c : counts) {
        if (c < 0) {
            lkg_set_error("%s: malformed line near byte %lld (expected 'h r t')", path, (long long)(-1 - c));
            return LKG_ERR_INVALID_ARG;
        }
        n += c;
    }
    *n_lines = n;
    return LKG_OK;
}

extern "C" int lkg_triples_read(const char *path, int64_t capacity, int64_t *h, int64_t *r, int64_t *t,
                                int64_t *n_read) {
    LKG_REQUIRE(path && n_read && (capacity == 0 || (h && r && t)), "lkg_triples_read: null pointer");
    Mapped m;
    int rc = map_file(path, m);
    if (rc != LKG_OK) return rc;
    const auto cut = line_chunks(m, parser_threads(m.n));
    std::vector<int64_t> counts, offsets(cut.size() - 1, 0);
    parse_chunks(m, cut, counts, nullptr, nullptr, nullptr, nullptr);
    int64_t n = 0;
    for (size_t k = 0; k < counts.size(); ++k) {
        if (counts[k] < 0) {
            lkg_set_error("%s: malformed line near byte %lld (expected 'h r t')", path, (long long)(-1 - counts[k]));
            return LKG_ERR_INVALID_ARG;
        }
        offsets[k] = n;
        n += counts[k];
    }
    if (n > capacity) {
        lkg_set_error("%s holds more than the %lld triples the caller sized for", path, (long long)capacity);
        return LKG_ERR_INVALID_ARG;
    }
    parse_chunks(m, cut, counts, h, r, t, &offsets);
    *n_read = n;
    return LKG_OK;
}

extern "C" int lkg_triples_dedup(int64_t n, const int64_t *h, const int64_t *r, const int64_t *t, int64_t *keep,
                                 int64_t *n_keep) {
    LKG_REQUIRE(n >= 0 && n_keep && (n == 0 || (h && r && t && keep)), "lkg_triples_dedup: bad arguments");
    const unsigned hw = std::max(1u, std::thread::hardware_concurrency());
    const int nt = (int)std::min<int64_t>(std::min(hw, 32u), n / (1 << 18));
    if (nt <= 1) {
        std::vector<int64_t> idx((size_t)n);
        for (int64_t i = 0; i < n; ++i) idx[i] = i;
        std::sort(idx.begin(), idx.end(), [&](int64_t a, int64_t b) {
            if (h[a] != h[b]) return h[a] < h[b];
            if (r[a] != r[b]) return r[a] < r[b];
            if (t[a] != t[b]) return t[a] < t[b];
            return a < b;
        });
        int64_t m = 0;
        for (int64_t i = 0; i < n; ++i) {
// ... 113 lines not shown
```

### literalkg_amd/ops.py

```python
from __future__ import annotations

from typing import Optional, Sequence, Tuple

import torch
from torch.autograd import Function

from . import _native as N
from .graph import KGStructure, LONG_ROW_THRESHOLD

LEAKY_SLOPE = 0.01
LN_EPS = 1e-5
NORMALIZE_EPS = 1e-12


_raw_stream = getattr(torch._C, "_cuda_getCurrentRawStream", None)


def _stream():
    if _raw_stream is not None:
        return _raw_stream(torch.cuda.current_device())
    return torch.cuda.current_stream().cuda_stream


def _need_gpu(*ts):
    for t in ts:
        if t is not None and not t.is_cuda:
            raise RuntimeError(
                "literalkg_amd ops run only on an MI355X device tensor (got a CPU tensor); there is no CPU "
                "fallback -- move the model and its inputs to the GPU (model.to('cuda')).")


def _f32_rows(t: torch.Tensor) -> torch.Tensor:
    if t.dtype != torch.float32:
        raise TypeError(f"expected float32, got {t.dtype}")
    if t.dim() != 2:
        raise ValueError(f"expected a 2-D tensor, got shape {tuple(t.shape)}")
    if t.stride(1) != 1 or (t.shape[0] > 1 and t.stride(0) < t.shape[1]):
        t = t.contiguous()
    return t


def _ld(t: torch.Tensor) -> int:
    return t.stride(0) if t.shape[0] > 1 else max(t.shape[1], t.stride(0))


def _i64(t: torch.Tensor) -> torch.Tensor:
    if t.dtype != torch.int64:
        t = t.long()
    return t.contiguous()


class _Deferred:
    pending = []
    _lock = None

    @classmethod
    def _guard(cls):
        if cls._lock is None:
            import threading
            cls._lock = threading.Lock()
        return cls._lock

    @classmethod
    def watch(cls, counter: torch.Tensor, exc, message: str):
        host = torch.empty(counter.shape, dtype=counter.dtype, pin_memory=True)
        host.copy_(counter, non_blocking=True)
        ev = torch.cuda.Event()
        ev.record()
        with cls._guard():
            cls.pending.append((ev, host, exc, message))

    @classmethod
    def poll(cls, wait: bool = False):
        with cls._guard():
            mine, cls.pending = cls.pending, []
        keep, err = [], None
        for ev, host, exc, message in mine:
            if wait:
                ev.synchronize()
            if not ev.query():
                keep.append((ev, host, exc, message))
            elif int(host.sum()) != 0 and err is None:
                err = exc(message.format(n=int(host.sum())))
        if keep:
            with cls._guard():
                cls.pending = keep + cls.pending
        if err is not None:
            raise err


def check_deferred_errors():
    _Deferred.poll(wait=True)


def checked_ids(n_rows: int, *id_lists: torch.Tensor, what: str = "entity"):
    _need_gpu(*id_lists)
    shapes = [tuple(i.shape) for i in id_lists]
    flat = [_i64(i.reshape(-1)) for i in id_lists]
    src = flat[0] if len(flat) == 1 else torch.cat(flat)
    out = torch.empty_like(src)
    bad = torch.empty(1, dtype=torch.int32, device=src.device)
    N.call("lkg_sanitize_ids_i64", src.numel(), N.ptr(src), 0, int(n_rows), N.ptr(out), N.ptr(bad), _stream())
    _Deferred.poll()
    _Deferred.watch(bad, IndexError, "{n} " + what + f" id(s) outside [0, {int(n_rows)}) in the ids handed to the model "
                    "(replaced by row 0 on the device; the results of that call are meaningless)")
    res, o = [], 0
    for sh, f in zip(shapes, flat):
        res.append(out[o:o + f.numel()].view(sh))
        o += f.numel()
    return res


def count_ids_outside(n_rows: int, ids: torch.Tensor) -> int:
    _need_gpu(ids)
    src = _i64(ids.reshape(-1))
    if src.numel() == 0:
        return 0
    out = torch.empty_like(src)
    bad = torch.empty(1, dtype=torch.int32, device=src.device)
    N.call("lkg_sanitize_ids_i64", src.numel(), N.ptr(src), 0, int(n_rows), N.ptr(out), N.ptr(bad), _stream())
    return int(bad.item())


import os as _os

CHECK_STRUCTURES = _os.environ.get("LKG_CHECK_STRUCTURES", "0") not in ("", "0")


def check_csr(rowptr: torch.Tensor, col: torch.Tensor, n_rows: int, n_cols: int, col_offset: int = 0,
              what: str = "structure") -> None:
    _need_gpu(rowptr, col)
    if rowptr.dtype != torch.int32 or col.dtype != torch.int32 or not rowptr.is_contiguous() or not col.is_contiguous():
        raise TypeError(f"{what}: rowptr and col must be contiguous int32 tensors")
    if rowptr.numel() < n_rows + 1:
        raise ValueError(f"{what}: {rowptr.numel()} offsets for {n_rows} rows")
    bad = torch.empty(1, dtype=torch.int32, device=col.device)
    N.call("lkg_csr_check_i32", int(n_rows), N.ptr(rowptr), col.numel(), N.ptr(col), int(col_offset), int(n_cols),
           N.ptr(bad), _stream())
    n_bad = int(bad.item())
    if n_bad:
        raise N.LkgError(f"{what}: {n_bad} offset(s) / column id(s) would make the SpMM read outside its operands "
                         f"({n_rows} rows, {col.numel()} stored entries, a source table of {n_cols} rows at offset {col_offset})")


def spmm_raw(rowptr, col, val, x, n_rows: int, out: Optional[torch.Tensor] = None,
             x_row_offset: int = 0, long_rows: Optional[torch.Tensor] = None,
             add_self: Optional[torch.Tensor] = None, add2: Optional[torch.Tensor] = None,
             copy: Optional[Tuple[torch.Tensor, torch.Tensor]] = None,
             rowmax: Optional[torch.Tensor] = None, add2_rows: Optional[torch.Tensor] = None,
             x_rows: Optional[torch.Tensor] = None, self_rows: Optional[torch.Tensor] = None,
             out_rows: Optional[torch.Tensor] = None, bias: Optional[torch.Tensor] = None,
             row_lists: Optional[Tuple[torch.Tensor, torch.Tensor]] = None) -> torch.Tensor:
    _need_gpu(x, val, rowptr, col)
    x = _f32_rows(x)
    d = x.shape[1]
    if out is None:
        out = torch.empty((n_rows, d), dtype=torch.float32, device=x.device)
    elif tuple(out.shape) != (n_rows, d) or out.dtype != torch.float32 or out.stride(1) != 1:
        raise ValueError(f"spmm_raw: out must be a float32 {n_rows} x {d} tensor with unit column stride (got {tuple(out.shape)})")
    if rowptr.numel() < n_rows + 1 or col.numel() != val.numel():
        raise ValueError("spmm_raw: rowptr needs n_rows + 1 offsets, col and val one element per stored entry")
    if rowptr.dtype != torch.int32 or col.dtype != torch.int32 or val.dtype != torch.float32:
        raise TypeError("spmm_raw: int32 offsets and column ids, float32 values")
    if CHECK_STRUCTURES:
        check_csr(rowptr, col, n_rows, x.shape[0], x_row_offset, what="spmm_raw")
    if bias is not None:
        if add2 is not None or bias.numel() != d or bias.dtype != torch.float32 or not bias.is_contiguous():
            raise ValueError(f"spmm_raw: bias must be a contiguous float32 vector of {d} elements and excludes add2")
    for name_, t_ in (("add_self", add_self), ("add2", add2)):
        if t_ is not None and tuple(t_.shape) != (n_rows, d):
            raise ValueError(f"spmm_raw: {name_} must be {n_rows} x {d} (got {tuple(t_.shape)})")
    if add_self is not None:
        add_self = _f32_rows(add_self)
    if add2 is not None:
        add2 = _f32_rows(add2)
    csrc, cdst = (_f32_rows(copy[0]), copy[1]) if copy is not None else (None, None)
    if cdst is not None and (cdst.stride(1) != 1 or cdst.shape != (n_rows, d)):
        raise ValueError("spmm_raw: copy destination must be an n_rows x d view with unit column stride")
    N.call("lkg_spmm_csr_fused_f32", n_rows, d, N.ptr(rowptr), N.ptr(col), N.ptr(val),
           N.ptr(x) - 4 * x_row_offset * _ld(x), _ld(x), N.ptr(out), _ld(out), N.ptr(add_self),
           _ld(add_self) if add_self is not None else 0, N.ptr(add2 if bias is None else bias),
           _ld(add2) if add2 is not None else 0, N.ptr(add2_rows if add2 is not None else None), N.ptr(csrc), _ld(csrc) if csrc is not None else 0, N.ptr(cdst), _ld(cdst) if cdst is not None else 0,
           N.ptr(rowmax), (x_rows.data_ptr() - x_row_offset) if x_rows is not None else None,
           N.ptr(self_rows if add_self is not None else None), N.ptr(out_rows), N.ptr(long_rows),
           0 if long_rows is None else long_rows.numel(), LONG_ROW_THRESHOLD,
           *((N.ptr(row_lists[0]), row_lists[0].numel(), N.ptr(row_lists[1]), row_lists[1].numel())
             if (row_lists is not None and x_rows is None and row_lists[0].numel() + row_lists[1].numel() == n_rows)
             else (None, 0, None, 0)), _stream())
    return out


GEMM_F32_ENGINES = ("f32_mfma", "bf16x3_rows", "bf16x3_kmajor")


def gemm_engine(a: torch.Tensor, b: torch.Tensor, trans_a: bool = False, trans_b: bool = False, alpha: float = 1.0,
                beta: float = 0.0, out: Optional[torch.Tensor] = None, bias: Optional[torch.Tensor] = None) -> str:
    a_, b_ = _f32_rows(a), _f32_rows(b)
    m, k = (a_.shape[1], a_.shape[0]) if trans_a else a_.shape
    n = b_.shape[0] if trans_b else b_.shape[1]
    out_ptr, out_ld = (N.ptr(out), _ld(out)) if out is not None else (None, n)
    if (not trans_a and alpha == 1.0 and _ENGINE != "f32" and (k * n <= 2048 or m < TALL_MIN_ROWS)
            and N.load().lkg_gemm_skinny_ok(m, n, k, N.ptr(a_), _ld(a_), out_ptr if out is not None else N.ptr(a_), out_ld)):
        return "skinny"
    if not trans_a and k > 0 and tall_ok(m, n, (k,), single_panel_too=tagged_rowmax(a) is not None):
        return "tall_f16x2"
    if trans_a and not trans_b and alpha == 1.0 and beta == 0.0 and bias is None and _WGRAD_ENGINE == "longk":
        if N.load().lkg_gemm_smallm_ok(m, n, k, N.ptr(a_), _ld(a_), N.ptr(b_), _ld(b_)):
            return "smallm"
        if N.load().lkg_gemm_longk_ok(m, n, k, N.ptr(a_), _ld(a_), N.ptr(b_), _ld(b_)):
            return "longk"
    need = int(N.load().lkg_gemm_workspace(int(trans_a), m, n, k)) if _ENGINE != "f32" else 0
    return GEMM_F32_ENGINES[int(N.load().lkg_gemm_f32_engine(int(trans_a), int(trans_b), m, n, k, need))]


def gemm(a: torch.Tensor, b: torch.Tensor, trans_a: bool = False, trans_b: bool = False, alpha: float = 1.0,
         beta: float = 0.0, out: Optional[torch.Tensor] = None, bias: Optional[torch.Tensor] = None) -> torch.Tensor:
    a, b = _f32_rows(a), _f32_rows(b)
    m, k = (a.shape[1], a.shape[0]) if trans_a else a.shape
    kb, n = (b.shape[1], b.shape[0]) if trans_b else b.shape
    if k != kb:
        raise ValueError(f"gemm: inner dimensions differ ({k} vs {kb})")
    if out is None:
        if beta != 0.0:
            raise ValueError("gemm: beta != 0 needs out")
        out = torch.empty((m, n), dtype=torch.float32, device=a.device)
    elif tuple(out.shape) != (m, n) or out.dtype != torch.float32 or out.stride(1) != 1:
        raise ValueError(f"gemm: out must be a float32 {m} x {n} tensor with unit column stride (got {tuple(out.shape)})")
    if bias is not None and bias.numel() != n:
        raise ValueError(f"gemm: bias of {bias.numel()} elements for {n} output columns")
    engine = gemm_engine(a, b, trans_a, trans_b, alpha, beta, out, bias)
    if engine == "skinny":
        N.call("lkg_gemm_skinny_f32", m, n, k, N.ptr(a), _ld(a), N.ptr(b), _ld(b), int(trans_b), float(beta), N.ptr(out),
               _ld(out), N.ptr(bias), _stream())
        return out
    if engine == "tall_f16x2":
        return gemm_tall((a,), ((b,),), bool(trans_b), bias, alpha, beta, out)
    if engine == "smallm":
        N.call("lkg_gemm_smallm_f32", m, n, k, N.ptr(a), _ld(a), N.ptr(b), _ld(b), N.ptr(out), _ld(out), _stream())
        return out
    if engine == "longk":
        N.call("lkg_gemm_longk_f32", m, n, k, N.ptr(a), _ld(a), N.ptr(b), _ld(b), N.ptr(out), _ld(out), _stream())
        return out
    need = int(N.load().lkg_gemm_workspace(int(trans_a), m, n, k)) if _ENGINE != "f32" else 0
    ws = _workspace(need, out.device) if need else None
    N.call("lkg_gemm_f32", int(trans_a), int(trans_b), m, n, k, float(alpha), N.ptr(a), _ld(a), N.ptr(b), _ld(b),
           float(beta), N.ptr(out), _ld(out), N.ptr(bias), N.ptr(ws), ws.numel() if ws is not None else 0, _stream())
    return out


def colsum(x: torch.Tensor) -> torch.Tensor:
    x = _f32_rows(x)
    out = torch.empty(x.shape[1], dtype=torch.float32, device=x.device)
    N.call("lkg_colsum_f32", x.shape[0], x.shape[1], N.ptr(x), _ld(x), N.ptr(out), _stream())
    return out


def col_absmax(x: torch.Tensor) -> torch.Tensor:
    _need_gpu(x)
    x = _f32_rows(x)
    out = torch.empty(x.shape[1], dtype=torch.float32, device=x.device)
    N.call("lkg_col_absmax_f32", x.shape[0], x.shape[1], N.ptr(x), _ld(x), N.ptr(out), _stream())
    return out


def tag_colmax(t: torch.Tensor, cm: Optional[torch.Tensor]) -> torch.Tensor:
    if cm is not None:
        t._lkg_colmax = (t._version, cm)
    return t


def tagged_colmax(t: torch.Tensor, cache: bool = False) -> Optional[torch.Tensor]:
    tag = getattr(t, "_lkg_colmax", None)
    if tag is not None and tag[0] == t._version and tag[1].shape[0] == t.shape[1] and tag[1].device == t.device:
        return tag[1]
    if not cache:
        return None
    cm = col_absmax(t)
    try:
        t._lkg_colmax = (t._version, cm)
    except AttributeError:
        pass
    return cm


def gemm_wgrad(a: torch.Tensor, b: torch.Tensor, a_colmax: torch.Tensor, b_colmax: torch.Tensor) -> torch.Tensor:
    _need_gpu(a, b, a_colmax, b_colmax)
    a, b = _f32_rows(a), _f32_rows(b)
    if a.shape[0] != b.shape[0]:
        raise ValueError(f"gemm_wgrad: the operands have {a.shape[0]} and {b.shape[0]} rows")
    out = torch.empty((a.shape[1], b.shape[1]), dtype=torch.float32, device=a.device)
    N.call("lkg_gemm_wgrad_f32", a.shape[1], b.shape[1], a.shape[0], N.ptr(a), _ld(a), N.ptr(a_colmax), N.ptr(b), _ld(b),
           N.ptr(b_colmax), N.ptr(out), b.shape[1], _stream())
    return out


FRONTIER_GROWTH = 24
NARROW_PANEL = 8


def narrow_weight_grad(gy: torch.Tensor, panel: torch.Tensor, want_sum: bool):
    gy, panel = _f32_rows(gy), _f32_rows(panel)
    d, n_w = gy.shape[1], panel.shape[1]
    gw = torch.empty((d, n_w), dtype=torch.float32, device=gy.device)
    gs = torch.empty(d, dtype=torch.float32, device=gy.device) if want_sum else None
    N.call("lkg_colsum_weighted_f32", gy.shape[0], d, N.ptr(gy), _ld(gy), N.ptr(panel), _ld(panel), n_w, N.ptr(gs),
           N.ptr(gw), n_w, _stream())
    return gw, gs


def weight_grads(gy: torch.Tensor, panels: Sequence[torch.Tensor], needed: Sequence[bool], want_sum: bool):
    gws = [None] * len(panels)
    gs = None
    for i, p in enumerate(panels):
        if needed[i] and p.shape[1] <= NARROW_PANEL and gy.shape[0] >= 2048:
            gws[i], s_ = narrow_weight_grad(gy, p, want_sum and gs is None)
            gs = s_ if s_ is not None else gs
    if want_sum and gs is None:
        gs = colsum(gy)
    for i, p in enumerate(panels):
        if needed[i] and gws[i] is None:
            gws[i] = gemm(gy, p, trans_a=True)
    return gws, gs


import ctypes as _C
import os as _os

TALL_MIN_ROWS = 16384
_ENGINE = _os.environ.get("LKG_GEMM_ENGINE", "f16x2")
_WGRAD_ENGINE = _os.environ.get("LKG_WGRAD_ENGINE", "longk")
_workspaces = {}


def _workspace(nbytes: int, device) -> torch.Tensor:
    key = (device, _stream())
    w = _workspaces.get(key)
    if w is None or w.numel() < nbytes:
        w = torch.empty(max(nbytes, 1 << 20), dtype=torch.uint8, device=device)
        _workspaces[key] = w
    return w


def _wants_rowmax(n_rows: int) -> bool:
    return _ENGINE in ("f16x2", "f16x2-all") and n_rows >= TALL_MIN_ROWS


def tag_rowmax(t: torch.Tensor, rm: Optional[torch.Tensor]) -> torch.Tensor:
    if rm is not None:
        t._lkg_rowmax = (t._version, rm)
    return t


def tagged_rowmax(t: torch.Tensor) -> Optional[torch.Tensor]:
    tag = getattr(t, "_lkg_rowmax", None)
    if tag is None or tag[0] != t._version or tag[1].shape[0] != t.shape[0] or tag[1].device != t.device:
        return None
    return tag[1]


class RowSet:

    def __init__(self, flags: torch.Tensor, id_lists: Sequence[torch.Tensor], unique: bool = False):
        self.flags = flags
        self.id_lists = [i.reshape(-1) for i in id_lists]
        self.n_max = sum(i.numel() for i in self.id_lists)
        self._ids = self.id_lists[0] if (unique and len(self.id_lists) == 1) else None

    def compact_ids(self) -> torch.Tensor:
        if self._ids is None:
            s_ = torch.sort(torch.cat(self.id_lists)).values
            dup = torch.zeros_like(s_, dtype=torch.bool)
            dup[1:] = s_[1:] == s_[:-1]
            self._ids = torch.where(dup, torch.full_like(s_, -1), s_)
        return self._ids


def union_rows(a: Optional[RowSet], b: Optional[RowSet]) -> Optional[RowSet]:
    if a is None or b is None:
        return a if b is None else b
    if a is b:
        return a
    for ids in b.id_lists:
        N.call("lkg_fill_rows_f32", ids.numel(), 0, N.ptr(ids), None, 0, 0.0, N.ptr(a.flags), 1, _stream())
    return RowSet(a.flags, [a.compact_ids(), *b.id_lists])


def tag_rows(t: torch.Tensor, rows: Optional[RowSet]) -> torch.Tensor:
    if rows is not None:
        t._lkg_rows = (t._version, rows)
    return t


def tagged_rows(t: Optional[torch.Tensor]) -> Optional[RowSet]:
    tag = getattr(t, "_lkg_rows", None) if t is not None else None
    if tag is None or tag[0] != t._version or tag[1].flags.shape[0] != t.shape[0] or tag[1].flags.device != t.device:
        return None
    return tag[1]


def _flags(rows: Optional[RowSet]) -> Optional[torch.Tensor]:
    return rows.flags if rows is not None else None


def rows_worth_compacting(rows: Optional[RowSet], n: int) -> bool:
    return rows is not None and n >= TALL_MIN_ROWS and rows.n_max * 8 <= n


_HAS_USE_COUNT = hasattr(torch._C, "_storage_Use_Count")


def _storage_users(t: torch.Tensor) -> int:
    if not _HAS_USE_COUNT:
        return -1
    return torch._C._storage_Use_Count(t.untyped_storage()._cdata)


import threading as _threading


class _RowScratch:

    _tables: dict = {}
    _lock = _threading.Lock()
    MAX_TABLES = 16

    def __init__(self, shape, device, with_flags: bool):
        self.buf = torch.zeros(tuple(shape), dtype=torch.float32, device=device)
        self.flags = torch.zeros(shape[0], dtype=torch.uint8, device=device) if with_flags else None
        self.users = _storage_users(self.buf)
        self.dirty: list = []
        self.unknown = False

    @classmethod
    def acquire(cls, n: int, c: int, device, pool: str = "loss") -> "_RowScratch":
        key = (device, n, c, pool, _stream())
        with cls._lock:
            ent = cls._tables.pop(key, None)
        if ent is None or ent.users < 0 or _storage_users(ent.buf) != ent.users:
            ent = _RowScratch((n, c), device, pool == "loss")
        with cls._lock:
            cls._tables[key] = ent
            while len(cls._tables) > cls.MAX_TABLES:
                cls._tables.pop(next(iter(cls._tables)))
        if ent.unknown:
            ent.buf.zero_()
            if ent.flags is not None:
                ent.flags.zero_()
            ent.unknown = False
        else:
            for ids in ent.dirty:
                N.call("lkg_fill_rows_f32", ids.numel(), ent.buf.shape[1], N.ptr(ids), N.ptr(ent.buf), _ld(ent.buf), 0.0,
                       N.ptr(ent.flags), 0, _stream())
        ent.dirty = []
        return ent

    def mark(self, *id_lists: torch.Tensor):
        for ids in id_lists:
            if self.flags is not None:
                N.call("lkg_fill_rows_f32", ids.numel(), 0, N.ptr(ids), None, 0, 0.0, N.ptr(self.flags), 1, _stream())
            self.dirty.append(ids)

    def table(self, rows: RowSet) -> torch.Tensor:
        return tag_rows(self.buf.view(self.buf.shape), rows)


def _loss_grad_table(emb: torch.Tensor, sparse_rows: bool, *id_lists: torch.Tensor) -> torch.Tensor:
    if not sparse_rows:
        return torch.zeros_like(emb, memory_format=torch.contiguous_format)
    ent = _RowScratch.acquire(emb.shape[0], emb.shape[1], emb.device)
    ent.mark(*id_lists)
    return ent.table(RowSet(ent.flags, id_lists))


def gather_rows_range(table: torch.Tensor, ids: torch.Tensor, lo: int, hi: int) -> torch.Tensor:
    table = _f32_rows(table)
    out = torch.empty((ids.numel(), table.shape[1]), dtype=torch.float32, device=table.device)
    N.call("lkg_gather_rows_range_f32", ids.numel(), table.shape[1], N.ptr(table), _ld(table), N.ptr(ids), int(lo), int(hi),
           N.ptr(out), table.shape[1], _stream())
    return out


def zero_table_for(rows: RowSet, n: int, c: int, device, pool: str) -> torch.Tensor:
    ent = _RowScratch.acquire(n, c, device, pool)
    ent.mark(rows.compact_ids())
    return ent.table(rows)


def row_absmax(x: torch.Tensor, out: Optional[torch.Tensor] = None, accumulate: bool = False) -> torch.Tensor:
    _need_gpu(x)
    x = _f32_rows(x)
    if out is None:
        out = torch.empty(x.shape[0], dtype=torch.float32, device=x.device)
        accumulate = False
    N.call("lkg_row_absmax_f32", x.shape[0], x.shape[1], N.ptr(x), _ld(x), N.ptr(out), int(accumulate), _stream())
    return out


def rows_absmax(panels: Sequence[torch.Tensor]) -> torch.Tensor:
    out = None
    for p in panels:
        rm = tagged_rowmax(p)
        if rm is not None and out is None and len(panels) == 1:
            return rm
        if rm is not None:
            out = rm.clone() if out is None else torch.maximum(out, rm, out=out)
        else:
            out = row_absmax(p, out, accumulate=out is not None)
    return out


def tall_ok(m: int, n: int, ks: Sequence[int], single_panel_too: bool = False) -> bool:
    if _ENGINE not in ("f16x2", "f16x2-all") or m < TALL_MIN_ROWS or not 1 <= len(ks) <= 3 or min(ks) <= 0:
        return False
    if len(ks) == 1 and not (single_panel_too or _ENGINE == "f16x2-all"):
        return False
    return n * sum(ks) <= (1 << 22)


TALL_VARIANTS = {"256x2": 0, "128x1": 1, "256x1": 2, "256x1w": 3, "ws": 4, "256r": 5}
DEFAULT_TALL_VARIANT: Optional[str] = None


def gemm_tall(a_panels: Sequence[torch.Tensor], b_blocks: Sequence[Sequence[torch.Tensor]], trans_b: bool,
              bias: Optional[torch.Tensor] = None, alpha: float = 1.0, beta: float = 0.0,
              out: Optional[torch.Tensor] = None, rowmax: Optional[torch.Tensor] = None, gate_x=None, keep=None,
              variant: Optional[str] = None):
    if rowmax is None:
        rowmax = rows_absmax(a_panels)
    a_panels = [_f32_rows(a) for a in a_panels]
    m = a_panels[0].shape[0]
    if any(a.shape[0] != m for a in a_panels):
        raise ValueError(f"gemm_tall: the K-panels have {[a.shape[0] for a in a_panels]} rows")
    if rowmax.numel() != m:
        raise ValueError(f"gemm_tall: {rowmax.numel()} row maxima for {m} rows")
    ks = [a.shape[1] for a in a_panels]
    n_groups = len(b_blocks)
    gate = gate_x is not None
    if gate != (n_groups == 2):
        raise ValueError("gemm_tall: two weight groups go with the gate epilogue (and only with it)")
    blocks = [[_f32_rows(b) for b in grp] for grp in b_blocks]
    rows = blocks[0][0].shape[0] if trans_b else blocks[0][0].shape[1]
# ... 46 lines not shown
                             drop_p: float, seed: int, want_y: bool = True, want_norm: bool = True,
                             yn_out: Optional[torch.Tensor] = None, rowmax: Optional[torch.Tensor] = None):
    if rowmax is None:
        rowmax = rows_absmax(a_panels)
    a_panels = [_f32_rows(a) for a in a_panels]
    ws_ = [_f32_rows(w) for w in w_blocks]
    _need_gpu(*a_panels, *ws_, gamma, beta)
    m, n = a_panels[0].shape[0], ws_[0].shape[0]
    ks = [a.shape[1] for a in a_panels]
    if any(a.shape[0] != m for a in a_panels) or any(tuple(w.shape) != (n, k) for w, k in zip(ws_, ks)) or len(ws_) != len(ks):
        raise ValueError("linear_act_layernorm: panels / weight blocks do not match")
    if not (want_y or want_norm):
        raise ValueError("linear_act_layernorm: neither output wanted")
    if rowmax.numel() != m or gamma.numel() != n or beta.numel() != n or (bias is not None and bias.numel() != n):
        raise ValueError("linear_act_layernorm: row maxima / gamma / beta / bias do not match the product's shape")
    dev = a_panels[0].device
    y = torch.empty((m, n), dtype=torch.float32, device=dev) if want_y else None
    yn = None
    if want_norm:
        yn = yn_out if yn_out is not None else torch.empty((m, n), dtype=torch.float32, device=dev)
        if tuple(yn.shape) != (m, n) or yn.stride(1) != 1 or yn.dtype != torch.float32:
            raise ValueError("linear_act_layernorm: the normalised copy's destination must be an m x n float32 view with unit column stride")
    mean = torch.empty(m, dtype=torch.float32, device=dev)
    rstd = torch.empty(m, dtype=torch.float32, device=dev)
    np_ = len(ks)
    a_ptr = (_C.c_void_p * np_)(*[a.data_ptr() for a in a_panels])
    a_ld = (_C.c_int64 * np_)(*[_ld(a) for a in a_panels])
    a_k = (_C.c_int32 * np_)(*ks)
    w_ptr = (_C.c_void_p * np_)(*[w.data_ptr() for w in ws_])
    w_ld = (_C.c_int64 * np_)(*[_ld(w) for w in ws_])
    need = N.load().lkg_linear_act_layernorm_workspace(n, np_, a_k)
    ws = _workspace(int(need), dev)
    N.call("lkg_linear_act_layernorm_fwd_f32", m, n, np_, a_ptr, a_ld, a_k, N.ptr(rowmax), w_ptr, w_ld, N.ptr(bias),
           float(slope), N.ptr(gamma), N.ptr(beta), float(eps), N.ptr(y), _ld(y) if y is not None else 0, N.ptr(yn),
           _ld(yn) if yn is not None else 0, float(norm_eps), N.ptr(mean), N.ptr(rstd), float(drop_p), int(seed), N.ptr(ws),
           ws.numel(), _stream())
    return y, yn, mean, rstd


@torch.no_grad()
def edge_softmax(g: KGStructure, ent: torch.Tensor, relemb: torch.Tensor, want_logits: bool = False,
                 row_lo: int = 0, row_hi: Optional[int] = None, out: Optional[torch.Tensor] = None
                 ) -> Tuple[torch.Tensor, Optional[torch.Tensor]]:
    _need_gpu(ent, relemb, g.rowptr)
    ent, relemb = _f32_rows(ent), _f32_rows(relemb)
    if ent.shape[1] != relemb.shape[1]:
        raise ValueError("update_att adds entity and relation embeddings: embed_dim must equal relation_dim "
                         "(model.py:441)")
    row_hi = g.n if row_hi is None else row_hi
    if ent.shape[0] != g.n or not 0 <= row_lo <= row_hi <= g.n:
        raise ValueError(f"edge_softmax: entity table of {ent.shape[0]} rows / row range [{row_lo}, {row_hi}) for a structure "
                         f"of {g.n} entities")
    if out is not None and (out.numel() != g.nnz or out.dtype != torch.float32 or not out.is_contiguous()):
        raise ValueError(f"edge_softmax: out must be a contiguous float32 array of {g.nnz} values")
    long_rows = g.long_rows(False, row_lo, row_hi)
    val = out if out is not None else torch.empty(g.nnz, dtype=torch.float32, device=ent.device)
    logits = torch.empty(g.nnz, dtype=torch.float32, device=ent.device) if want_logits else None
    if g.nnz == 0:
        return val, logits
    dup = (None, None, 0)
    if g.has_dups:
        de, dr = g.dup_entries, g.dup_rows
        if row_lo != 0 or row_hi != g.n:
            keep = (dr >= row_lo) & (dr < row_hi)
            de, dr = de[keep].contiguous(), (dr[keep] - row_lo).contiguous()
        dup = (N.ptr(de), N.ptr(dr), de.numel())
    if row_lo == 0 and row_hi == g.n:
        e_lo, e_hi = 0, g.nnz
    else:
        rp = g.host("rowptr")
        e_lo, e_hi = int(rp[row_lo]), int(rp[row_hi])
    N.call("lkg_edge_softmax_f32", row_hi - row_lo, row_lo, ent.shape[1], g.rowptr.data_ptr() + 4 * row_lo,
           N.ptr(g.col), N.ptr(g.eptr), N.ptr(g.rel), N.ptr(g.rel_first), *dup, e_lo, e_hi,
           N.ptr(ent), _ld(ent), N.ptr(relemb), _ld(relemb), N.ptr(val),
           N.ptr(logits), N.ptr(long_rows), 0 if long_rows is None else long_rows.numel(), LONG_ROW_THRESHOLD,
           relemb.shape[0], _stream())
    return val, logits


def permute_values(val: torch.Tensor, perm: torch.Tensor) -> torch.Tensor:
    _need_gpu(val, perm)
    if perm.dtype != torch.int32 or val.dtype != torch.float32 or not perm.is_contiguous() or not val.is_contiguous():
        raise TypeError("permute_values: contiguous float32 values and a contiguous int32 index list")
    out = torch.empty(perm.numel(), dtype=val.dtype, device=val.device)
    N.call("lkg_permute_f32", perm.numel(), N.ptr(perm), val.numel(), N.ptr(val), N.ptr(out), _stream())
    return out


def _check_table(ego: torch.Tensor, g: KGStructure, val: torch.Tensor):
    if ego.dim() != 2 or ego.shape[0] != g.n:
        raise ValueError(f"aggregate: the table has shape {tuple(ego.shape)}, the structure {g.n} entities")
    if val.numel() != g.nnz:
        raise ValueError(f"aggregate: {val.numel()} attention values for {g.nnz} stored entries")


class _Aggregate(Function):

    @staticmethod
    def forward(ctx, ego, g: KGStructure, val, val_t, plus_self, bias=None):
        _need_gpu(ego, val, bias)
        _check_table(ego, g, val)
        ctx.g = g
        ctx.val_t = val_t
        ctx.plus_self = plus_self
        ctx.has_bias = bias is not None
        rm = torch.empty(g.n, dtype=torch.float32, device=ego.device) if _wants_rowmax(g.n) else None
        return tag_rowmax(spmm_raw(g.rowptr, g.col, val, ego, g.n, long_rows=g.long_rows(False),
                                   add_self=ego if plus_self else None, rowmax=rm,
                                   bias=bias.detach().contiguous() if bias is not None else None,
                                   row_lists=g.row_lists(False)), rm)

    @staticmethod
    def backward(ctx, grad):
        g_ego, *rest = _Aggregate._backward_ego(ctx, grad)
        g_bias = None
        if ctx.has_bias and ctx.needs_input_grad[5]:
            rs = tagged_rows(grad)
            g_bias = (colsum(gather_rows_range(grad, rs.compact_ids(), 0, grad.shape[0]))
                      if rows_worth_compacting(rs, grad.shape[0]) else colsum(grad))
        return (g_ego, *rest, g_bias)

    @staticmethod
    def _backward_ego(ctx, grad):
        g = ctx.g
        if g.t_rowptr is None:
            raise RuntimeError("KGStructure was built without its transpose; backward needs the CSC")
        rs = tagged_rows(grad)
        rows = _flags(rs) if rows_worth_compacting(rs, g.n) else None
        grad = _f32_rows(grad)
        d = grad.shape[1]
        if (rows_worth_compacting(rs, g.n) and rs.n_max * FRONTIER_GROWTH <= g.n and d % 4 == 0 and d <= 1024
                and grad.data_ptr() % 16 == 0 and _ld(grad) % 4 == 0):
            ent = _RowScratch.acquire(g.n, d, grad.device, "g_agg")
            out = ent.buf.view(ent.buf.shape)
            reached = torch.empty(g.n, dtype=torch.uint8, device=grad.device)
            ent.unknown = True
            spmm_raw(g.t_rowptr, g.t_col, ctx.val_t, grad, g.n, out=out, long_rows=g.long_rows(True),
                     add_self=grad if ctx.plus_self else None, x_rows=rows, self_rows=rows, out_rows=reached)
            ids = torch.nonzero(reached).flatten()
            ent.dirty.append(ids)
            ent.unknown = False
            return tag_rows(out, RowSet(reached, [ids], unique=True)), None, None, None, None
        return spmm_raw(g.t_rowptr, g.t_col, ctx.val_t, grad, g.n, long_rows=g.long_rows(True),
                        add_self=grad if ctx.plus_self else None, x_rows=rows, self_rows=rows,
                        row_lists=g.row_lists(True)), None, None, None, None


def aggregate(ego: torch.Tensor, g: KGStructure, val: torch.Tensor, val_t: torch.Tensor,
              plus_self: bool = False, bias: Optional[torch.Tensor] = None) -> torch.Tensor:
    return _Aggregate.apply(ego, g, val, val_t, plus_self, bias)


class _AggregateKeep(Function):

    @staticmethod
    def forward(ctx, ego, g: KGStructure, val, val_t, plus_self, keep_dst):
        _need_gpu(ego, val)
        _check_table(ego, g, val)
        ctx.g, ctx.val_t, ctx.plus_self = g, val_t, plus_self
        ctx.follow_frontier = not ego.is_leaf
        ctx.set_materialize_grads(False)
        copy = None
        kept = ego
        if keep_dst is not None and not _same_view(keep_dst, ego):
            copy, kept = (ego, keep_dst), keep_dst
        rm = torch.empty(g.n, dtype=torch.float32, device=ego.device) if _wants_rowmax(g.n) else None
        side = spmm_raw(g.rowptr, g.col, val, ego, g.n, long_rows=g.long_rows(False),
                        add_self=ego if plus_self else None, copy=copy, rowmax=rm, row_lists=g.row_lists(False))
        return tag_rowmax(side, rm), kept

    @staticmethod
    def backward(ctx, g_side, g_kept):
        g = ctx.g
        if g_side is None:
            return g_kept, None, None, None, None, None
        if g.t_rowptr is None:
            raise RuntimeError("KGStructure was built without its transpose; backward needs the CSC")
        rs = tagged_rows(g_side)
        rows = _flags(rs) if rows_worth_compacting(rs, g.n) else None
        g_side = _f32_rows(g_side)
        rk = tagged_rows(g_kept)
        d = g_side.shape[1]
        if (ctx.follow_frontier and rows is not None and (g_kept is None or rk is not None) and rs.n_max * FRONTIER_GROWTH <= g.n and d % 4 == 0
                and d <= 1024 and g_side.data_ptr() % 16 == 0 and _ld(g_side) % 4 == 0
                and (g_kept is None or (g_kept.data_ptr() % 16 == 0 and _ld(g_kept) % 4 == 0))):
            ent = _RowScratch.acquire(g.n, d, g_side.device, "g_agg_keep")
            out = ent.buf.view(ent.buf.shape)
            reached = torch.empty(g.n, dtype=torch.uint8, device=g_side.device)
            ent.unknown = True
            spmm_raw(g.t_rowptr, g.t_col, ctx.val_t, g_side, g.n, out=out, long_rows=g.long_rows(True),
                     add_self=g_side if ctx.plus_self else None, add2=g_kept, add2_rows=_flags(rk), x_rows=rows, self_rows=rows,
                     out_rows=reached)
            ids = torch.nonzero(reached).flatten()
            ent.dirty.append(ids)
            ent.unknown = False
            return tag_rows(out, RowSet(reached, [ids], unique=True)), None, None, None, None, None
        return spmm_raw(g.t_rowptr, g.t_col, ctx.val_t, g_side, g.n, long_rows=g.long_rows(True),
                        add_self=g_side if ctx.plus_self else None, add2=g_kept,
                        add2_rows=_flags(rk), x_rows=rows, self_rows=rows, row_lists=g.row_lists(True)), None, None, None, None, None


def aggregate_keep(ego, g: KGStructure, val, val_t, plus_self: bool = False, keep_dst: Optional[torch.Tensor] = None):
    return _AggregateKeep.apply(ego, g, val, val_t, plus_self, keep_dst)


class _Fanout(Function):

    @staticmethod
    def forward(ctx, x):
        ctx.set_materialize_grads(False)
        return x.view_as(x), x.view_as(x)

    @staticmethod
    def backward(ctx, ga, gb):
        if ga is None or gb is None:
            return ga if gb is None else gb
        ra, rb = tagged_rows(ga), tagged_rows(gb)
        n, d = ga.shape
        if ra is not None and rb is not None and rows_worth_compacting(ra, n) and rows_worth_compacting(rb, n):
            flags = ra.flags.clone()
            rows = union_rows(RowSet(flags, ra.id_lists), rb)
            if rows_worth_compacting(rows, n):
                out = zero_table_for(rows, n, d, ga.device, "g_fanout")
                for g_, r_ in ((ga, ra), (gb, rb)):
                    ids = r_.compact_ids()
                    part = gather_rows_range(g_, ids, 0, n)
                    N.call("lkg_scatter_add_rows_range_f32", ids.numel(), d, N.ptr(part), d, N.ptr(ids), 0, n, N.ptr(out), _ld(out),
                           _stream())
                return out
        return _elt(0, ga, gb, 1.0, 1.0)


def fanout(x: torch.Tensor):
    return _Fanout.apply(x)


class _MultiLinear(Function):

    @staticmethod
    def forward(ctx, bias, n_terms, *xw):
        xs, ws = xw[:n_terms], xw[n_terms:]
        _need_gpu(*xs, *ws)
        y = None
        if n_terms == 1 and _skinny(xs[0], ws[0].shape[0]):
            y = gemm(xs[0], ws[0], trans_b=True, bias=bias)
        elif tall_ok(xs[0].shape[0], ws[0].shape[0], [x.shape[1] for x in xs],
                     single_panel_too=tagged_rowmax(xs[0]) is not None):
            y = gemm_tall(xs, (ws,), True, bias)
        else:
            for i, (x, w) in enumerate(zip(xs, ws)):
                y = gemm(x, w, trans_b=True, beta=0.0 if i == 0 else 1.0, out=y, bias=bias if i == 0 else None)
        ctx.save_for_backward(*xs, *ws)
        ctx.n_terms = n_terms
        ctx.has_bias = bias is not None
        return y

    @staticmethod
    def backward(ctx, gy):
        n = ctx.n_terms
        saved = ctx.saved_tensors
        xs, ws = saved[:n], saved[n:]
        rows = tagged_rows(gy)
        if rows_worth_compacting(rows, gy.shape[0]):
            return _MultiLinear._backward_on_rows(ctx, gy, rows, xs, ws)
        gy = _f32_rows(gy)
        gxs = []
        rm = None
        for i in range(n):
            if not ctx.needs_input_grad[2 + i]:
                gxs.append(None)
            elif _skinny(gy, ws[i].shape[1]):
                gxs.append(gemm(gy, ws[i]))
            elif tall_ok(gy.shape[0], ws[i].shape[1], (gy.shape[1],), single_panel_too=tagged_rowmax(gy) is not None):
                rm = rows_absmax((gy,)) if rm is None else rm
                gxs.append(gemm_tall((gy,), ((ws[i],),), False, rowmax=rm))
            else:
                gxs.append(gemm(gy, ws[i]))
        gws, gb = weight_grads(gy, xs, ctx.needs_input_grad[2 + n:2 + 2 * n], ctx.has_bias and ctx.needs_input_grad[0])
        return (gb, None, *gxs, *gws)

    @staticmethod
    def _backward_on_rows(ctx, gy, rows: RowSet, xs, ws):
        n = ctx.n_terms
        ids = rows.compact_ids()
        n_rows = gy.shape[0]
        gc = gather_rows_range(gy, ids, 0, n_rows)
        gb = colsum(gc) if (ctx.has_bias and ctx.needs_input_grad[0]) else None
        gxs, gws = [], []
        for i in range(n):
            if not ctx.needs_input_grad[2 + i]:
                gxs.append(None)
                continue
            gx = zero_table_for(rows, n_rows, ws[i].shape[1], gy.device, f"g_x{i}")
            N.call("lkg_scatter_add_rows_range_f32", ids.numel(), ws[i].shape[1], N.ptr(gemm(gc, ws[i])), ws[i].shape[1],
                   N.ptr(ids), 0, n_rows, N.ptr(gx), _ld(gx), _stream())
            gxs.append(gx)
        for i in range(n):
            gws.append(gemm(gc, gather_rows_range(xs[i], ids, 0, n_rows), trans_a=True)
                       if ctx.needs_input_grad[2 + n + i] else None)
        return (gb, None, *gxs, *gws)


def _skinny(x: torch.Tensor, n_out: int) -> bool:
    return (x.dim() == 2 and x.shape[0] >= 4096 and 4 <= x.shape[1] <= 64 and 4 <= n_out <= 64 and x.shape[1] % 4 == 0
            and x.shape[1] * n_out <= 2048
            and n_out % 4 == 0 and _ENGINE != "f32" and x.stride(1) == 1 and x.stride(0) % 4 == 0 and x.data_ptr() % 16 == 0)


def linear(x, w, b=None):
    return _MultiLinear.apply(b, 1, x, w)


def multi_linear(xs: Sequence[torch.Tensor], ws: Sequence[torch.Tensor], b=None):
    return _MultiLinear.apply(b, len(xs), *xs, *ws)


class _StackedLinear(Function):

    @staticmethod
    def forward(ctx, x, n_lin, *wb):
        ws, bs = wb[:n_lin], wb[n_lin:]
        _need_gpu(x, *ws, *bs)
        x = _f32_rows(x)
        w_all = torch.cat([w.detach() for w in ws], 0).contiguous()
        b_all = torch.cat([b.detach() for b in bs]).contiguous()
        m, k = x.shape
        n = w_all.shape[0]
        if tall_ok(m, n, (k,), single_panel_too=True):
            y = gemm_tall((x,), ((w_all,),), True, b_all)
        else:
            y = gemm(x, w_all, trans_b=True, bias=b_all)
        ctx.save_for_backward(x, w_all)
        ctx.widths = [int(w.shape[0]) for w in ws]
        ctx.set_materialize_grads(False)
        outs, o = [], 0
        for wd in ctx.widths:
            outs.append(y[:, o:o + wd])
            o += wd
        return tuple(outs)

    @staticmethod
    def backward(ctx, *gs):
        x, w_all = ctx.saved_tensors
        m, n = x.shape[0], w_all.shape[0]
        g_all = torch.empty((m, n), dtype=torch.float32, device=x.device)
        o = 0
        for wd, g in zip(ctx.widths, gs):
            if g is None:
                g_all[:, o:o + wd].zero_()
            else:
                fill_slot(g_all, o, g)
            o += wd
        n_lin = len(ctx.widths)
        need = ctx.needs_input_grad
        gx = gemm(g_all, w_all) if need[0] else None
        gws, gbs = [None] * n_lin, [None] * n_lin
        if any(need[2:2 + n_lin]):
            gw_all = gemm(g_all, x, trans_a=True)
            o = 0
            for i, wd in enumerate(ctx.widths):
                gws[i] = gw_all[o:o + wd] if need[2 + i] else None
                o += wd
        if any(need[2 + n_lin:]):
            gb_all = colsum(g_all)
            o = 0
            for i, wd in enumerate(ctx.widths):
                gbs[i] = gb_all[o:o + wd] if need[2 + n_lin + i] else None
                o += wd
        return (gx, None, *gws, *gbs)


def stacked_linear(x: torch.Tensor, ws: Sequence[torch.Tensor], bs: Sequence[torch.Tensor]):
    return _StackedLinear.apply(x, len(ws), *ws, *bs)


class _MatMul(Function):
    @staticmethod
    def forward(ctx, a, b):
        _need_gpu(a, b)
        ctx.save_for_backward(a, b)
        return gemm(a, b)

    @staticmethod
    def backward(ctx, gc):
        a, b = ctx.saved_tensors
        gc = _f32_rows(gc)
        ga = gemm(gc, b, trans_b=True) if ctx.needs_input_grad[0] else None
        gb = gemm(a, gc, trans_a=True) if ctx.needs_input_grad[1] else None
        return ga, gb


def matmul(a, b):
    return _MatMul.apply(a, b)


def gemm_f64acc(a: torch.Tensor, b: torch.Tensor, trans_a: bool = False, trans_b: bool = False) -> torch.Tensor:
    a, b = _f32_rows(a), _f32_rows(b)
    _need_gpu(a, b)
    m, k = (a.shape[1], a.shape[0]) if trans_a else a.shape
    kb, n = (b.shape[1], b.shape[0]) if trans_b else b.shape
    if k != kb:
        raise ValueError(f"gemm_f64acc: inner dimensions {k} and {kb} differ")
    out = torch.empty((m, n), dtype=torch.float32, device=a.device)
    N.call("lkg_gemm_f64acc_f32", int(trans_a), int(trans_b), m, n, k, N.ptr(a), _ld(a), N.ptr(b), _ld(b), N.ptr(out), _ld(out),
           _stream())
    return out


class _FoldNT(Function):

    @staticmethod
    def forward(ctx, a, b):
        ctx.save_for_backward(a, b)
        return gemm_f64acc(a, b, trans_b=True)

    @staticmethod
    def backward(ctx, g):
        a, b = ctx.saved_tensors
        ga = gemm_f64acc(g, b) if ctx.needs_input_grad[0] else None
        gb = gemm_f64acc(g, a, trans_a=True) if ctx.needs_input_grad[1] else None
        return ga, gb


FOLD_F64 = _os.environ.get("LKG_FOLD_F32", "0") in ("", "0")


def fold_nt(a, b):
    return _FoldNT.apply(a, b) if FOLD_F64 else matmul(a, b.t())


def _elt(op, a, b=None, alpha=1.0, beta=0.0):
    a = _f32_rows(a)
    b = _f32_rows(b) if b is not None else None
    if b is not None and b.shape != a.shape:
        raise ValueError(f"element-wise operands differ in shape: {tuple(a.shape)} vs {tuple(b.shape)}")
    out = torch.empty(a.shape, dtype=torch.float32, device=a.device)
    N.call("lkg_eltwise_f32", op, a.shape[0], a.shape[1], N.ptr(a), _ld(a), N.ptr(b), _ld(b) if b is not None else 0,
           float(alpha), float(beta), N.ptr(out), _ld(out), _stream())
    return out


class _Axpby(Function):

    @staticmethod
    def forward(ctx, a, b, alpha, beta):
        _need_gpu(a, b)
        ctx.ab = (alpha, beta, b is not None)
        return _elt(0, a, b, alpha, beta)

    @staticmethod
    def backward(ctx, g):
        alpha, beta, has_b = ctx.ab
        rows = tagged_rows(g)
        ga = tag_rows(_elt(0, g, None, alpha, 0.0), rows) if ctx.needs_input_grad[0] else None
        gb = tag_rows(_elt(0, g, None, beta, 0.0), rows) if has_b and ctx.needs_input_grad[1] else None
        return ga, gb, None, None


def axpby(a, b, alpha=1.0, beta=1.0):
    return _Axpby.apply(a, b, alpha, beta)


class _Mul(Function):
    @staticmethod
    def forward(ctx, a, b):
        _need_gpu(a, b)
        ctx.save_for_backward(a, b)
        return _elt(1, a, b)

    @staticmethod
    def backward(ctx, g):
        a, b = ctx.saved_tensors
        rows = tagged_rows(g)
        return (tag_rows(_elt(1, g, b), rows) if ctx.needs_input_grad[0] else None,
                tag_rows(_elt(1, g, a), rows) if ctx.needs_input_grad[1] else None)


def mul(a, b):
    return _Mul.apply(a, b)


class _BiMix(Function):

    @staticmethod
    def forward(ctx, ego, side, h0p, alpha):
        _need_gpu(ego, side, h0p)
        ego, side = _f32_rows(ego), _f32_rows(side)
        h = _f32_rows(h0p) if h0p is not None else None
        if side.shape != ego.shape or (h is not None and h.shape != ego.shape):
            raise ValueError("bi_mix: ego, side (and h0p) must have one shape")
        n, d = ego.shape
        out_sum = torch.empty((n, d), dtype=torch.float32, device=ego.device)
        out_prod = torch.empty((n, d), dtype=torch.float32, device=ego.device)
        N.call("lkg_bi_mix_fwd_f32", n, d, N.ptr(ego), _ld(ego), N.ptr(side), _ld(side), N.ptr(h), _ld(h) if h is not None else 0,
               float(alpha), N.ptr(out_sum), d, N.ptr(out_prod), d, _stream())
        ctx.save_for_backward(ego, side)
        ctx.cfg = (h is not None, float(alpha))
        ctx.set_materialize_grads(False)
        return out_sum, out_prod

    @staticmethod
    def backward(ctx, g_sum, g_prod):
        ego, side = ctx.saved_tensors
        has_h0, alpha = ctx.cfg
        if g_sum is None and g_prod is None:
            return None, None, None, None
        rs, rp = tagged_rows(g_sum), tagged_rows(g_prod)
        rows = rs if (rs is rp or g_prod is None) else (rp if g_sum is None else None)
        g_sum = _f32_rows(g_sum) if g_sum is not None else torch.zeros_like(ego)
        g_prod = _f32_rows(g_prod) if g_prod is not None else torch.zeros_like(ego)
        n, d = ego.shape
        g_ego = torch.empty((n, d), dtype=torch.float32, device=ego.device)
        g_side = torch.empty((n, d), dtype=torch.float32, device=ego.device)
        g_h = torch.empty((n, d), dtype=torch.float32, device=ego.device) if has_h0 else None
        N.call("lkg_bi_mix_bwd_f32", n, d, N.ptr(ego), _ld(ego), N.ptr(side), _ld(side), N.ptr(g_sum), _ld(g_sum), N.ptr(g_prod),
               _ld(g_prod), int(has_h0), float(alpha), N.ptr(g_ego), N.ptr(g_side), N.ptr(g_h), _stream())
        return tag_rows(g_ego, rows), tag_rows(g_side, rows), (tag_rows(g_h, rows) if has_h0 else None), None


def bi_mix(ego, side, h0p=None, alpha: float = 0.0):
    return _BiMix.apply(ego, side, h0p, alpha)


class _LeakySum(Function):

    @staticmethod
    def forward(ctx, a, b, slope):
        _need_gpu(a, b)
        ctx.save_for_backward(a, b) if b is not None else ctx.save_for_backward(a)
        ctx.slope = slope
        return _elt(2, a, b, slope)

    @staticmethod
    def backward(ctx, g):
        saved = ctx.saved_tensors
        rows = tagged_rows(g)
        if rows_worth_compacting(rows, g.shape[0]):
            ids = rows.compact_ids()
            n_rows, d = g.shape
            gc = gather_rows_range(g, ids, 0, n_rows)
            outs = []
            for i in range(len(saved)):
                if not ctx.needs_input_grad[i]:
                    outs.append(None)
                    continue
                part = _elt(3, gc, gather_rows_range(saved[i], ids, 0, n_rows), ctx.slope)
                dst = zero_table_for(rows, n_rows, d, g.device, f"g_leaky{i}")
                N.call("lkg_scatter_add_rows_range_f32", ids.numel(), d, N.ptr(part), d, N.ptr(ids), 0, n_rows, N.ptr(dst),
                       _ld(dst), _stream())
                outs.append(dst)
            return (outs[0], outs[1] if len(outs) > 1 else None, None)
        ga = tag_rows(_elt(3, g, saved[0], ctx.slope), rows) if ctx.needs_input_grad[0] else None
        gb = tag_rows(_elt(3, g, saved[1], ctx.slope), rows) if len(saved) > 1 and ctx.needs_input_grad[1] else None
        return ga, gb, None


def leaky_relu(a, slope=LEAKY_SLOPE):
    return _LeakySum.apply(a, None, slope)


def leaky_relu_sum(a, b, slope=LEAKY_SLOPE):
    return _LeakySum.apply(a, b, slope)


class _ActLayerNorm(Function):

    @staticmethod
    def forward(ctx, z, gamma, beta, want_norm, slope, eps, norm_eps, drop_p, seed, yn_out, want_y):
        _need_gpu(z, gamma, beta)
        z = _f32_rows(z)
        n, d = z.shape
        if not want_y and not want_norm:
            raise ValueError("act_layernorm: neither output wanted")
        y = torch.empty((n, d), dtype=torch.float32, device=z.device) if want_y else None
        yn = None
        if want_norm:
            yn = yn_out if yn_out is not None else torch.empty((n, d), dtype=torch.float32, device=z.device)
        mean = torch.empty(n, dtype=torch.float32, device=z.device)
        rstd = torch.empty(n, dtype=torch.float32, device=z.device)
        N.call("lkg_act_layernorm_fwd_f32", n, d, N.ptr(z), _ld(z), float(slope), N.ptr(gamma), N.ptr(beta),
               float(eps), N.ptr(y), _ld(y) if y is not None else 0, N.ptr(yn), _ld(yn) if yn is not None else 0,
               float(norm_eps), N.ptr(mean), N.ptr(rstd), float(drop_p), int(seed), _stream())
        ctx.save_for_backward(z, gamma, beta, mean, rstd, *([y] if y is not None else []))
        ctx.cfg = (slope, norm_eps, drop_p, seed)
        ctx.set_materialize_grads(False)
        if want_norm:
            return y, yn
        return y, None

    @staticmethod
    def backward(ctx, gy, gyn):
        z, gamma, beta, mean, rstd, *kept_y = ctx.saved_tensors
        y = kept_y[0] if kept_y else None
        slope, norm_eps, drop_p, seed = ctx.cfg
        n, d = z.shape
        none = (None,) * 11
        if gy is None and gyn is None:
            return none
        rows_n = tagged_rows(gyn)
        rows_y = tagged_rows(gy)
        gy = _f32_rows(gy) if gy is not None else None
        gyn = _f32_rows(gyn) if gyn is not None else None
        gg = torch.zeros(d, dtype=torch.float32, device=z.device)
        gb = torch.zeros(d, dtype=torch.float32, device=z.device)
        rows = None
        if (gy is None or rows_y is not None) and (gyn is None or rows_n is not None):
            rows = union_rows(rows_y, rows_n)
        sparse_out = rows_worth_compacting(rows, n)
        ids = rows.compact_ids() if sparse_out else None
# ... 1590 lines not shown
```

Before: 6.664 billion.

## Add MFMA thin-N GEMM for long-K skinny shapes and slice-reduce smallm wgrad

Adds a new thin-N GEMM kernel that keeps the whole weight panel in LDS and runs f32 MFMA 32x32x2 over 32-row tiles, with register prefetch of the next A chunk. Skinny dispatch now covers n<=64 with k up to 1024, which previously fell to the general or tall paths. The smallm weight-gradient kernel is rewritten to write per-slice partials into a workspace, followed by a second reduction kernel. This trades an extra launch and workspace traffic for better parallelism, and relies on large dynamic LDS allocations.

```diff
diff --git a/include/literalkg_hip.h b/include/literalkg_hip.h
--- a/include/literalkg_hip.h
+++ b/include/literalkg_hip.h
@@ -193,7 +193,7 @@
                        float *c, int64_t ldc, void *stream);
 int lkg_gemm_smallm_ok(int64_t m, int64_t n, int64_t k, const float *a, int64_t lda, const float *b, int64_t ldb);
 int lkg_gemm_smallm_f32(int64_t m, int64_t n, int64_t k, const float *a, int64_t lda, const float *b, int64_t ldb,
-                        float *c, int64_t ldc, void *stream);
+                        float *c, int64_t ldc, float *workspace, int64_t workspace_floats, void *stream);
 
 int64_t lkg_narrow_layer_bwd_workspace(int64_t n);
 int lkg_narrow_layer_bwd_ok(int64_t n, int32_t d_in, int32_t d_out, const float *x, int64_t ldx, const float *z, int64_t ldz,
diff --git a/include/literalkg_hip_gemm_thin.h b/include/literalkg_hip_gemm_thin.h
--- /dev/null
+++ b/include/literalkg_hip_gemm_thin.h
@@ -0,0 +1,19 @@
+#ifndef LITERALKG_HIP_GEMM_THIN_H
+#define LITERALKG_HIP_GEMM_THIN_H
+
+#include "literalkg_hip.h"
+
+#ifdef __cplusplus
+extern "C" {
+#endif
+
+int64_t lkg_gemm_smallm_slice_rows(int64_t m, int64_t n);
+int64_t lkg_gemm_smallm_workspace(int64_t m, int64_t n, int64_t k);
+
+int32_t lkg_gemm_skinny_kernel(int64_t m, int64_t n, int64_t k);
+
+#ifdef __cplusplus
+}
+#endif
+
+#endif
diff --git a/literalkg_amd/_native.py b/literalkg_amd/_native.py
--- a/literalkg_amd/_native.py
+++ b/literalkg_amd/_native.py
@@ -80,7 +80,7 @@
     "lkg_gemm_smallm_ok": [i64, i64, i64, vp, i64, vp, i64],
     "lkg_gemm_skinny_ok": [i64, i64, i64, vp, i64, vp, i64],
     "lkg_gemm_skinny_f32": [i64, i64, i64, vp, i64, vp, i64, i32, f32, vp, i64, vp, vp],
-    "lkg_gemm_smallm_f32": [i64, i64, i64, vp, i64, vp, i64, vp, i64, vp],
+    "lkg_gemm_smallm_f32": [i64, i64, i64, vp, i64, vp, i64, vp, i64, vp, i64, vp],
     "lkg_gemm_wgrad_f32": [i64, i64, i64, vp, i64, vp, vp, i64, vp, vp, i64, vp],
     "lkg_narrow_layer_bwd_ok": [i64, i32, i32, vp, i64, vp, i64, vp, i64, vp, i64, vp, i64],
     "lkg_narrow_layer_bwd_workspace": [i64],
@@ -158,13 +158,19 @@
     "lkg_gemm_ordered_workspace": [i64, i64, i64, i32],
     "lkg_gemm_ordered_f32": [i32, i32, i64, i64, i64, i32, f32, vp, i64, vp, i64, f32, vp, i64, vp, vp, i64, vp],
 }
+THIN_GEMM_PROTOTYPES = {
+    "lkg_gemm_smallm_slice_rows": [i64, i64],
+    "lkg_gemm_smallm_workspace": [i64, i64, i64],
+    "lkg_gemm_skinny_kernel": [i64, i64, i64],
+}
 _RESTYPE = {"lkg_last_error": C.c_char_p, "lkg_csr_build_device_workspace": C.c_int64,
             "lkg_gemm_tall_workspace": C.c_int64, "lkg_gemm_workspace": C.c_int64,
             "lkg_linear_act_layernorm_workspace": C.c_int64, "lkg_narrow_layer_bwd_workspace": C.c_int64,
             "lkg_csr_transpose_device_workspace": C.c_int64, "lkg_binary_curve_workspace": C.c_int64,
             "lkg_threshold_fit_workspace": C.c_int64, "lkg_accept_order_workspace": C.c_int64,
             "lkg_gemm_ordered_splits": C.c_int32, "lkg_gemm_ordered_partition": C.c_int64,
-            "lkg_gemm_ordered_workspace": C.c_int64}
+            "lkg_gemm_ordered_workspace": C.c_int64, "lkg_gemm_smallm_slice_rows": C.c_int64,
+            "lkg_gemm_smallm_workspace": C.c_int64, "lkg_gemm_skinny_kernel": C.c_int32}
 
 
 class LkgError(RuntimeError):
@@ -187,7 +193,7 @@
     lib = C.CDLL(_LIB_PATH)
     for name, argtypes in list(PROTOTYPES.items()) + list(EXTRA_PROTOTYPES.items()) + list(TRAIN_PROTOTYPES.items()) + \
             list(SAMPLE_PROTOTYPES.items()) + list(RELATION_TRAIN_PROTOTYPES.items()) + \
-            list(ORDERED_GEMM_PROTOTYPES.items()):
+            list(ORDERED_GEMM_PROTOTYPES.items()) + list(THIN_GEMM_PROTOTYPES.items()):
         fn = getattr(lib, name)
         fn.argtypes = argtypes
         fn.restype = _RESTYPE.get(name, C.c_int)
diff --git a/literalkg_amd/build.py b/literalkg_amd/build.py
--- a/literalkg_amd/build.py
+++ b/literalkg_amd/build.py
@@ -13,7 +13,7 @@
            "lkg_gemm.hip", "lkg_batch.hip", "lkg_csr_device.hip", "lkg_gemm_tall.hip", "lkg_gemm_wgrad.hip", "lkg_layer.hip",
            "lkg_rank.hip", "lkg_topk.hip", "lkg_pairmlp.hip", "lkg_triples.hip", "lkg_relations.hip",
            "lkg_accept.hip", "lkg_retrieval.hip", "lkg_softmax.hip", "lkg_kvsall.hip", "lkg_nssa.hip", "lkg_negatives.hip",
-           "lkg_relation_loss.hip", "lkg_gemm_ordered.hip"]
+           "lkg_relation_loss.hip", "lkg_gemm_ordered.hip", "lkg_gemm_thin.hip"]
 FLAGS = ["-O3", "--offload-arch=gfx950", "-fPIC", "-std=c++17"]
 
 
@@ -21,7 +21,7 @@
     return [os.path.join(CSRC, f) for f in sorted(os.listdir(CSRC)) if f.endswith(".h")] + \
            [os.path.join(HERE, "..", "include", h) for h in ("literalkg_hip.h", "literalkg_hip_ext.h", "literalkg_hip_train.h",
                                                                 "literalkg_hip_sample.h", "literalkg_hip_relation_train.h",
-                                                                "literalkg_hip_gemm_ordered.h")]
+                                                                "literalkg_hip_gemm_ordered.h", "literalkg_hip_gemm_thin.h")]
 
 
 TAG_FILE = os.path.join(HERE, "lib", "flags.tag")
diff --git a/literalkg_amd/csrc/lkg_gemm_thin.h b/literalkg_amd/csrc/lkg_gemm_thin.h
--- /dev/null
+++ b/literalkg_amd/csrc/lkg_gemm_thin.h
@@ -0,0 +1,6 @@
+#pragma once
+#include "lkg_common.h"
+#include "../../include/literalkg_hip_gemm_thin.h"
+
+int lkg_internal_thin_launch(int kind, int64_t m, int64_t n, int64_t k, const float *a, int64_t lda, const float *b, int64_t ldb,
+                             int32_t trans_b, float beta, float *c, int64_t ldc, const float *bias, hipStream_t stream);
diff --git a/literalkg_amd/csrc/lkg_gemm_thin.hip b/literalkg_amd/csrc/lkg_gemm_thin.hip
--- /dev/null
+++ b/literalkg_amd/csrc/lkg_gemm_thin.hip
@@ -0,0 +1,181 @@
+#include <algorithm>
+
+#include "lkg_gemm_thin.h"
+
+namespace {
+
+typedef float f32x16 __attribute__((ext_vector_type(16)));
+constexpr int TILE = 32;
+constexpr int KC = 64;
+constexpr int AP = KC + 4;
+constexpr int WAVES = 4;
+constexpr int PIECES = TILE * KC / 4 / 64;
+constexpr int LDS_MAX = 160 * 1024;
+
+__device__ __forceinline__ float4 f4_sel(bool on, const float4 &v) { return on ? v : make_float4(0.f, 0.f, 0.f, 0.f); }
+
+template <bool BETA>
+__device__ __forceinline__ void store_tile(const f32x16 &acc, long row0, long m, int col, int n, float bias_v, float beta,
+                                           float *__restrict__ c, long ldc, int kk) {
+    if (col >= n) return;
+#pragma unroll
+    for (int r = 0; r < 16; ++r) {
+        const long row = row0 + (r & 3) + 8 * (r >> 2) + 4 * kk;
+        if (row >= m) continue;
+        float o = acc[r] + bias_v;
+        if constexpr (BETA) o = fmaf(beta, c[row * ldc + col], o);
+        c[row * ldc + col] = o;
+    }
+}
+
+__device__ __forceinline__ void fill_panel(float *dst, int rows, int pitch, int n, int k, const float *__restrict__ b, long ldb,
+                                           int trans_b) {
+    for (int i = threadIdx.x; i < rows * pitch; i += 256) {
+        const int col = i / pitch, kk = i % pitch;
+        dst[i] = (col < n && kk < k) ? (trans_b ? b[(long)col * ldb + kk] : b[(long)kk * ldb + col]) : 0.f;
+    }
+}
+
+template <int NT, bool BETA>
+__global__ __launch_bounds__(256) void thin_n_kernel(long m, int n, int k, const float *__restrict__ a, long lda,
+                                                      const float *__restrict__ b, long ldb, int trans_b, float beta,
+                                                      float *__restrict__ c, long ldc, const float *__restrict__ bias) {
+    extern __shared__ __attribute__((aligned(16))) float thin_smem[];
+    const int k8 = (k + 7) & ~7, wp = k8 + 4;
+    float *ws = thin_smem;
+    const int lane = threadIdx.x & 63, wv = threadIdx.x >> 6;
+    float *as = thin_smem + TILE * NT * wp + wv * (TILE * AP);
+    fill_panel(ws, TILE * NT, wp, n, k, b, ldb, trans_b);
+    __syncthreads();
+
+    const int cc = lane & 31, kk = lane >> 5;
+    const long n_tiles = (m + TILE - 1) / TILE;
+    const long first = (long)blockIdx.x * WAVES + wv, stride = (long)gridDim.x * WAVES;
+    const int n_chunks = (k + KC - 1) / KC;
+    float bv[NT];
+#pragma unroll
+    for (int j = 0; j < NT; ++j) bv[j] = (bias && 32 * j + cc < n) ? bias[32 * j + cc] : 0.f;
+
+    float4 pf[PIECES];
+    auto fetch = [&](long tile, int chunk) {
+        const long row0 = tile * TILE;
+        const int k0 = chunk * KC, kw = min(KC, k - k0);
+#pragma unroll
+        for (int q = 0; q < PIECES; ++q) {
+            const int p = lane + 64 * q, r = p >> 4, cq = (p & 15) * 4;
+            const long row = min(row0 + r, m - 1);
+            const bool on = row0 + r < m && cq < kw;
+            pf[q] = f4_sel(on, *reinterpret_cast<const float4 *>(a + row * lda + k0 + (cq < kw ? cq : 0)));
+        }
+    };
+    auto stage = [&]() {
+#pragma unroll
+        for (int q = 0; q < PIECES; ++q) {
+            const int p = lane + 64 * q;
+            *reinterpret_cast<float4 *>(as + (p >> 4) * AP + (p & 15) * 4) = pf[q];
+        }
+    };
+    long tile = first;
+    if (tile < n_tiles) fetch(tile, 0);
+    for (; tile < n_tiles; tile += stride) {
+        f32x16 acc[NT];
+#pragma unroll
+        for (int j = 0; j < NT; ++j)
+#pragma unroll
+            for (int r = 0; r < 16; ++r) acc[j][r] = 0.f;
+        for (int chunk = 0; chunk < n_chunks; ++chunk) {
+            stage();
+            if (chunk + 1 < n_chunks) fetch(tile, chunk + 1);
+            else if (tile + stride < n_tiles) fetch(tile + stride, 0);
+            __builtin_amdgcn_sched_barrier(0);
+            const int k0 = chunk * KC, blocks8 = min(KC, k8 - k0) >> 3;
+            const float *ar = as + cc * AP + 4 * kk;
+            const float *wr = ws + cc * wp + k0 + 4 * kk;
+            auto block8 = [&](int q8) {
+                const float4 a4 = *reinterpret_cast<const float4 *>(ar + 8 * q8);
+#pragma unroll
+                for (int j = 0; j < NT; ++j) {
+                    const float4 w4 = *reinterpret_cast<const float4 *>(wr + 32 * j * wp + 8 * q8);
+                    acc[j] = __builtin_amdgcn_mfma_f32_32x32x2f32(a4.x, w4.x, acc[j], 0, 0, 0);
+                    acc[j] = __builtin_amdgcn_mfma_f32_32x32x2f32(a4.y, w4.y, acc[j], 0, 0, 0);
+                    acc[j] = __builtin_amdgcn_mfma_f32_32x32x2f32(a4.z, w4.z, acc[j], 0, 0, 0);
+                    acc[j] = __builtin_amdgcn_mfma_f32_32x32x2f32(a4.w, w4.w, acc[j], 0, 0, 0);
+                }
+            };
+            if (blocks8 == KC / 8) {
+#pragma unroll
+                for (int q8 = 0; q8 < KC / 8; ++q8) block8(q8);
+            } else {
+                for (int q8 = 0; q8 < blocks8; ++q8) block8(q8);
+            }
+        }
+#pragma unroll
+        for (int j = 0; j < NT; ++j) store_tile<BETA>(acc[j], tile * TILE, m, 32 * j + cc, n, bv[j], beta, c, ldc, kk);
+    }
+}
+
+int64_t thin_lds_bytes(int64_t n, int64_t k) {
+    const int64_t k8 = (k + 7) & ~(int64_t)7, n32 = (n + 31) & ~(int64_t)31;
+    return 4 * (n32 * (k8 + 4) + WAVES * TILE * AP);
+}
+
+constexpr int N_SLOTS = 4;
+int allow_lds(const void *kernel, int slot, int64_t lds) {
+    static bool raised_on[N_SLOTS][64] = {};
+    if (lds <= 64 * 1024) return LKG_OK;
+    int dev = 0;
+    if (hipGetDevice(&dev) != hipSuccess || dev < 0 || dev >= 64) {
+        lkg_set_error("lkg_gemm_skinny_f32: cannot tell the current device");
+        return LKG_ERR_HIP;
+    }
+    if (!raised_on[slot][dev]) {
+        if (hipFuncSetAttribute(kernel, hipFuncAttributeMaxDynamicSharedMemorySize, LDS_MAX) != hipSuccess) {
+            lkg_set_error("lkg_gemm_skinny_f32: cannot raise the dynamic LDS limit");
+            return LKG_ERR_HIP;
+        }
+        raised_on[slot][dev] = true;
+    }
+    return LKG_OK;
+}
+
+template <typename Kernel>
+int launch(Kernel kernel, int slot, int64_t m, int64_t n, int64_t k, const float *a, int64_t lda, const float *b,
+           int64_t ldb, int32_t trans_b, float beta, float *c, int64_t ldc, const float *bias, hipStream_t s) {
+    const int64_t lds = thin_lds_bytes(n, k);
+    const int rc = allow_lds(reinterpret_cast<const void *>(kernel), slot, lds);
+    if (rc != LKG_OK) return rc;
+    const int64_t per_cu = std::max<int64_t>(1, std::min<int64_t>(2, LDS_MAX / lds));
+    const int64_t tiles = (m + TILE - 1) / TILE;
+    const unsigned blocks = (unsigned)std::max<int64_t>(1, std::min<int64_t>((tiles + WAVES - 1) / WAVES, 256 * per_cu));
+    hipLaunchKernelGGL(kernel, dim3(blocks), dim3(256), (size_t)lds, s, (long)m, (int)n, (int)k, a, (long)lda, b, (long)ldb,
+                       (int)trans_b, beta, c, (long)ldc, bias);
+    LKG_CHECK_LAUNCH("lkg_gemm_skinny_f32");
+    return LKG_OK;
+}
+
+}
+
+extern "C" int32_t lkg_gemm_skinny_kernel(int64_t m, int64_t n, int64_t k) {
+    if (m < 1 || n < 4 || k < 4 || n % 4 || k % 4) return 0;
+    if (n <= 64 && k <= 64) return m >= 4096 ? 1 : 0;
+    if (n <= 64 && k <= 1024) return thin_lds_bytes(n, k) <= LDS_MAX ? 2 : 0;
+    return 0;
+}
+
+int lkg_internal_thin_launch(int kind, int64_t m, int64_t n, int64_t k, const float *a, int64_t lda, const float *b, int64_t ldb,
+                             int32_t trans_b, float beta, float *c, int64_t ldc, const float *bias, hipStream_t s) {
+#define LKG_THIN(NT_, SLOT)                                                                                              \
+    (beta != 0.f ? launch(thin_n_kernel<NT_, true>, 2 * (SLOT) + 1, m, n, k, a, lda, b, ldb, trans_b, beta, c, ldc, bias, s)  \
+                 : launch(thin_n_kernel<NT_, false>, 2 * (SLOT), m, n, k, a, lda, b, ldb, trans_b, beta, c, ldc, bias, s))
+    if (kind != 2) {
+        lkg_set_error("lkg_gemm_skinny_f32: no kernel for this shape (lkg_gemm_skinny_kernel)");
+        return LKG_ERR_INVALID_ARG;
+    }
+    return n <= 32 ? LKG_THIN(1, 0) : LKG_THIN(2, 1);
+#undef LKG_THIN
+}
+
+int lkg_internal_preload_gemm_thin() {
+    hipFuncAttributes attr;
+    return hipFuncGetAttributes(&attr, reinterpret_cast<const void *>(&thin_n_kernel<1, false>)) == hipSuccess ? 0 : 1;
+}
diff --git a/literalkg_amd/csrc/lkg_gemm_wgrad.hip b/literalkg_amd/csrc/lkg_gemm_wgrad.hip
--- a/literalkg_amd/csrc/lkg_gemm_wgrad.hip
+++ b/literalkg_amd/csrc/lkg_gemm_wgrad.hip
@@ -1,8 +1,7 @@
 #include <algorithm>
-#include <cstdlib>
 #include <type_traits>
 
-#include "lkg_common.h"
+#include "lkg_gemm_thin.h"
 
 namespace {
 
@@ -652,93 +651,115 @@
 
 namespace {
 
-template <int MT>
-__global__ __launch_bounds__(256) void smallm_wgrad_kernel(long m, long n, long k, const float *__restrict__ a, long lda,
-                                                            const float *__restrict__ b, long ldb, float *__restrict__ c,
-                                                            long ldc, long rows_per_block) {
-    constexpr int RM_ = MT / 16;
-    constexpr int R = 32;
-    __shared__ __attribute__((aligned(16))) float as[R][MT], bs[R][64];
-    const int t = threadIdx.x;
-    const int bi = t >> 4, bj = t & 15;
-    const long n0 = (long)blockIdx.y * 64;
-    const long k_lo = (long)blockIdx.x * rows_per_block, k_hi = min(k, k_lo + rows_per_block);
-    if (k_lo >= k_hi) return;
-    float acc[RM_][4];
-#pragma unroll
-    for (int i = 0; i < RM_; ++i)
-#pragma unroll
-        for (int j = 0; j < 4; ++j) acc[i][j] = 0.f;
-    constexpr int APIECES = R * MT / 4, A_PER_ROW = MT / 4, NA = APIECES / 256, NB = 2;
-    float4 ra[NA], rb[NB];
-    auto load_tile = [&](long k0) {
-#pragma unroll
-        for (int q = 0; q < NA; ++q) {
-            const int p = t + 256 * q, r = p / A_PER_ROW, cq = (p % A_PER_ROW) * 4;
-            const long row = min(k0 + r, k_hi - 1);
-            const bool on = k0 + r < k_hi && cq < m;
-            const float4 v = *reinterpret_cast<const float4 *>(a + row * lda + (cq < m ? cq : 0));
-            ra[q] = on ? v : make_float4(0.f, 0.f, 0.f, 0.f);
-        }
-#pragma unroll
-        for (int q = 0; q < NB; ++q) {
-            const int p = t + 256 * q, r = p >> 4, cq = (p & 15) * 4;
-            const long row = min(k0 + r, k_hi - 1);
-            const bool on = k0 + r < k_hi && n0 + cq < n;
-            const float4 v = *reinterpret_cast<const float4 *>(b + row * ldb + (n0 + cq < n ? n0 + cq : 0));
-            rb[q] = on ? v : make_float4(0.f, 0.f, 0.f, 0.f);
-        }
-    };
-    auto store_tile = [&]() {
-#pragma unroll
-        for (int q = 0; q < NA; ++q) {
-            const int p = t + 256 * q;
-            *reinterpret_cast<float4 *>(&as[p / A_PER_ROW][(p % A_PER_ROW) * 4]) = ra[q];
-        }
-#pragma unroll
-        for (int q = 0; q < NB; ++q) {
-            const int p = t + 256 * q;
-            *reinterpret_cast<float4 *>(&bs[p >> 4][(p & 15) * 4]) = rb[q];
-        }
-    };
-    load_tile(k_lo);
-    store_tile();
+constexpr int SM_SLICE = 2048;
+constexpr int SM_WAVES = 4;
+
+template <int MT, int T, int U>
+__global__ __launch_bounds__(256) __attribute__((amdgpu_waves_per_eu(2))) void smallm_wgrad_kernel(long m, long n, long k, const float *__restrict__ a, long lda,
+                                                            const float *__restrict__ b, long ldb,
+                                                            float *__restrict__ partials) {
+    __shared__ float fold[SM_WAVES - 1][16][64];
+    const int lane = threadIdx.x & 63, wv = __builtin_amdgcn_readfirstlane(threadIdx.x >> 6);
+    const int cc = lane & 31, kk = lane >> 5;
+    const long k_lo = (long)blockIdx.x * SM_SLICE, k_hi = min(k, k_lo + SM_SLICE);
+    const long n0 = (long)blockIdx.y * (32 * T);
+    unsigned aoff[MT], boff[T];
+    const unsigned kka = 4u * (unsigned)(kk * lda), kkb = 4u * (unsigned)(kk * ldb);
+#pragma unroll
+    for (int i = 0; i < MT; ++i) aoff[i] = 4u * (unsigned)(kk * lda + min((long)(32 * i + cc), m - 1));
+#pragma unroll
+    for (int j = 0; j < T; ++j) boff[j] = 4u * (unsigned)(kk * ldb + min(n0 + 32 * j + cc, n - 1));
+    f32x16 acc[MT][T];
+#pragma unroll
+    for (int i = 0; i < MT; ++i)
+#pragma unroll
+        for (int j = 0; j < T; ++j)
+#pragma unroll
+            for (int r = 0; r < 16; ++r) acc[i][j][r] = 0.f;
+
+    const int steps = (int)((k_hi - k_lo + 2 * U - 1) / (2 * U));
+    float xa0[U][MT], xb0[U][T], xa1[U][MT], xb1[U][T];
+    auto load = [&](int s, float (&xa)[U][MT], float (&xb)[U][T]) {
+        const long r0 = k_lo + (long)s * (2 * U);
+#pragma unroll
+        for (int t = 0; t < U; ++t) {
+            const long r = min(r0 + 2 * t, k - 1);
+            const char *pa = reinterpret_cast<const char *>(a + r * lda), *pb = reinterpret_cast<const char *>(b + r * ldb);
+            const bool there = r + kk < k;
+            const unsigned da = there ? 0u : kka, db = there ? 0u : kkb;
+#pragma unroll
+            for (int i = 0; i < MT; ++i) xa[t][i] = *reinterpret_cast<const float *>(pa + (aoff[i] - da));
+#pragma unroll
+            for (int j = 0; j < T; ++j) xb[t][j] = *reinterpret_cast<const float *>(pb + (boff[j] - db));
+        }
+    };
+    auto mma = [&](int s, const float (&xa)[U][MT], const float (&xb)[U][T]) {
+        const long r0 = k_lo + (long)s * (2 * U) + kk;
+#pragma unroll
+        for (int t = 0; t < U; ++t) {
+            const bool on = r0 + 2 * t < k_hi;
+            float av[MT];
+#pragma unroll
+            for (int i = 0; i < MT; ++i) av[i] = on ? xa[t][i] : 0.f;
+#pragma unroll
+            for (int j = 0; j < T; ++j) {
+                const float bv = on ? xb[t][j] : 0.f;
+#pragma unroll
+                for (int i = 0; i < MT; ++i) acc[i][j] = __builtin_amdgcn_mfma_f32_32x32x2f32(av[i], bv, acc[i][j], 0, 0, 0);
+            }
+        }
+    };
+    load(wv, xa0, xb0);
+    for (int s = wv; s < steps; s += 2 * SM_WAVES) {
+        load(s + SM_WAVES, xa1, xb1);
+        __builtin_amdgcn_sched_barrier(0);
+        mma(s, xa0, xb0);
+        __builtin_amdgcn_sched_barrier(0);
+        load(s + 2 * SM_WAVES, xa0, xb0);
+        __builtin_amdgcn_sched_barrier(0);
+        mma(s + SM_WAVES, xa1, xb1);
+        __builtin_amdgcn_sched_barrier(0);
+    }
+
+    float *mine = partials + (long)blockIdx.x * (m * n);
+#pragma unroll
+    for (int i = 0; i < MT; ++i)
+#pragma unroll
+        for (int j = 0; j < T; ++j) {
+            __builtin_amdgcn_sched_barrier(0);
+            __syncthreads();
+            if (wv > 0) {
+#pragma unroll
+                for (int r = 0; r < 16; ++r) fold[wv - 1][r][lane] = acc[i][j][r];
+            }
+            __syncthreads();
+            if (wv == 0) {
+                const long col = n0 + 32 * j + cc;
+#pragma unroll
+                for (int r = 0; r < 16; ++r) {
+                    const long row = 32 * i + (r & 3) + 8 * (r >> 2) + 4 * kk;
+                    const float v = ((acc[i][j][r] + fold[0][r][lane]) + fold[1][r][lane]) + fold[2][r][lane];
+                    if (row < m && col < n) mine[row * n + col] = v;
+                }
+            }
+        }
+}
+
+__global__ __launch_bounds__(1024) void smallm_sums_kernel(const float *__restrict__ partials, int slices, long mn, long n,
+                                                           float *__restrict__ c, long ldc) {
+    __shared__ float red[16][65];
+    const int cl = threadIdx.x & 63, g = threadIdx.x >> 6;
+    const long e = (long)blockIdx.x * 64 + cl;
+    float v = 0.f;
+    if (e < mn)
+        for (int s = g; s < slices; s += 16) v += partials[(long)s * mn + e];
+    red[g][cl] = v;
     __syncthreads();
-    for (long k0 = k_lo; k0 < k_hi; k0 += R) {
-        const bool more = k0 + R < k_hi;
-        if (more) load_tile(k0 + R);
-#pragma unroll 8
-        for (int r = 0; r < R; ++r) {
-            const float4 bv = *reinterpret_cast<const float4 *>(&bs[r][4 * bj]);
-            float av[RM_];
-            if constexpr (RM_ == 4) {
-                const float4 x = *reinterpret_cast<const float4 *>(&as[r][4 * bi]);
-                av[0] = x.x; av[1] = x.y; av[2] = x.z; av[3] = x.w;
-            } else {
-                const float2 x = *reinterpret_cast<const float2 *>(&as[r][2 * bi]);
-                av[0] = x.x; av[1] = x.y;
-            }
-#pragma unroll
-            for (int i = 0; i < RM_; ++i) {
-                acc[i][0] = fmaf(av[i], bv.x, acc[i][0]);
-                acc[i][1] = fmaf(av[i], bv.y, acc[i][1]);
-                acc[i][2] = fmaf(av[i], bv.z, acc[i][2]);
-                acc[i][3] = fmaf(av[i], bv.w, acc[i][3]);
-            }
-        }
-        __syncthreads();
-        if (more) store_tile();
-        __syncthreads();
-    }
-#pragma unroll
-    for (int i = 0; i < RM_; ++i) {
-        const long row = RM_ * bi + i;
-        if (row >= m) continue;
-#pragma unroll
-        for (int j = 0; j < 4; ++j) {
-            const long col = n0 + 4 * bj + j;
-            if (col < n) atomicAdd(c + row * ldc + col, acc[i][j]);
-        }
+    if (g == 0 && e < mn) {
+        float t = 0.f;
+#pragma unroll
+        for (int q = 0; q < 16; ++q) t += red[q][cl];
+        c[(e / n) * ldc + e % n] = t;
     }
 }
 
@@ -746,34 +767,48 @@
 
 extern "C" int lkg_gemm_smallm_ok(int64_t m, int64_t n, int64_t k, const float *a, int64_t lda, const float *b, int64_t ldb) {
     return k >= 4096 && m >= 4 && m <= 64 && n >= 4 && m % 4 == 0 && n % 4 == 0 && lda % 4 == 0 && ldb % 4 == 0 &&
-           lkg_aligned16(a) && lkg_aligned16(b);
+           lda < (1 << 29) && ldb < (1 << 29) && n < (1 << 29) && lkg_aligned16(a) && lkg_aligned16(b);
+}
+
+extern "C" int64_t lkg_gemm_smallm_slice_rows(int64_t m, int64_t n) {
+    return m > 0 && n > 0 ? SM_SLICE : LKG_ERR_INVALID_ARG;
+}
+
+extern "C" int64_t lkg_gemm_smallm_workspace(int64_t m, int64_t n, int64_t k) {
+    if (m <= 0 || n <= 0 || k <= 0 || m > 64 || n > (int64_t)1 << 24 || k > (int64_t)1 << 40) return LKG_ERR_INVALID_ARG;
+    return (k + SM_SLICE - 1) / SM_SLICE * m * n;
 }
 
 extern "C" int lkg_gemm_smallm_f32(int64_t m, int64_t n, int64_t k, const float *a, int64_t lda, const float *b, int64_t ldb,
-                                   float *c, int64_t ldc, void *stream) {
+                                   float *c, int64_t ldc, float *workspace, int64_t workspace_floats, void *stream) {
     LKG_REQUIRE(m > 0 && n > 0 && k > 0 && a && b && c && ldc >= n && lda >= m && ldb >= n, "lkg_gemm_smallm_f32: bad arguments");
     LKG_REQUIRE(lkg_gemm_smallm_ok(m, n, k, a, lda, b, ldb), "lkg_gemm_smallm_f32: needs m <= 64, k >= 4096, widths and row "
                 "strides that are multiples of 4 floats and 16-byte aligned operands (lkg_gemm_smallm_ok)");
+    const int64_t need = lkg_gemm_smallm_workspace(m, n, k);
+    LKG_REQUIRE(need > 0 && workspace && workspace_floats >= need, "lkg_gemm_smallm_f32: workspace of %lld floats, %lld needed "
+                "(lkg_gemm_smallm_workspace)", (long long)workspace_floats, (long long)need);
     hipStream_t s = (hipStream_t)stream;
-    const hipError_t rc = ldc == n ? hipMemsetAsync(c, 0, sizeof(float) * m * n, s)
-                                   : hipMemset2DAsync(c, sizeof(float) * ldc, 0, sizeof(float) * n, m, s);
-    if (rc != hipSuccess) {
-        lkg_set_error("lkg_gemm_smallm_f32: hipMemsetAsync failed");
-        return LKG_ERR_HIP;
-    }
-    const int64_t chunks = (n + 63) / 64;
-    static const int64_t target = getenv("LKG_SMALLM_BLOCKS") ? atoll(getenv("LKG_SMALLM_BLOCKS")) : 768;
-    int64_t blocks = std::max<int64_t>(1, std::min<int64_t>(target / chunks + 1, k / 256));
-    int64_t per = ((k + blocks - 1) / blocks + 31) / 32 * 32;
-    blocks = (k + per - 1) / per;
-    const dim3 grid((unsigned)blocks, (unsigned)chunks);
-    if (m <= 32)
-        hipLaunchKernelGGL((smallm_wgrad_kernel<32>), grid, dim3(256), 0, s, (long)m, (long)n, (long)k, a, (long)lda, b, (long)ldb,
-                           c, (long)ldc, (long)per);
-    else
-        hipLaunchKernelGGL((smallm_wgrad_kernel<64>), grid, dim3(256), 0, s, (long)m, (long)n, (long)k, a, (long)lda, b, (long)ldb,
-                           c, (long)ldc, (long)per);
+    const int64_t slices = (k + SM_SLICE - 1) / SM_SLICE;
+    LKG_REQUIRE(slices < INT32_MAX && n <= 32 * 10 * 65535ll, "lkg_gemm_smallm_f32: grid too large");
+#define LKG_SMALLM(MT_, T_, U_)                                                                                              \
+    hipLaunchKernelGGL((smallm_wgrad_kernel<MT_, T_, U_>), dim3((unsigned)slices, (unsigned)((n + 32 * T_ - 1) / (32 * T_))), \
+                       dim3(256), 0, s, (long)m, (long)n, (long)k, a, (long)lda, b, (long)ldb, workspace)
+    if (m <= 32) {
+        if (n <= 32) LKG_SMALLM(1, 1, 8);
+        else if (n <= 64) LKG_SMALLM(1, 2, 8);
+        else if (n <= 160) LKG_SMALLM(1, 5, 4);
+        else LKG_SMALLM(1, 10, 2);
+    } else {
+        if (n <= 32) LKG_SMALLM(2, 1, 8);
+        else if (n <= 64) LKG_SMALLM(2, 2, 4);
+        else LKG_SMALLM(2, 5, 2);
+    }
+#undef LKG_SMALLM
     LKG_CHECK_LAUNCH("lkg_gemm_smallm_f32");
+    const int64_t mn = m * n;
+    hipLaunchKernelGGL(smallm_sums_kernel, dim3((unsigned)((mn + 63) / 64)), dim3(1024), 0, s, workspace, (int)slices, (long)mn,
+                       (long)n, c, (long)ldc);
+    LKG_CHECK_LAUNCH("lkg_gemm_smallm_f32 (sums)");
     return LKG_OK;
 }
 
@@ -840,16 +875,18 @@
 }
 
 extern "C" int lkg_gemm_skinny_ok(int64_t m, int64_t n, int64_t k, const float *a, int64_t lda, const float *c, int64_t ldc) {
-    return m >= 4096 && k >= 4 && k <= 64 && n >= 4 && n <= 64 && k % 4 == 0 && n % 4 == 0 && lda % 4 == 0 && ldc % 4 == 0 &&
-           lkg_aligned16(a) && lkg_aligned16(c);
+    return lkg_gemm_skinny_kernel(m, n, k) != 0 && lda % 4 == 0 && ldc % 4 == 0 && lkg_aligned16(a) && lkg_aligned16(c);
 }
 
 extern "C" int lkg_gemm_skinny_f32(int64_t m, int64_t n, int64_t k, const float *a, int64_t lda, const float *b, int64_t ldb,
                                    int32_t trans_b, float beta, float *c, int64_t ldc, const float *bias, void *stream) {
     LKG_REQUIRE(m > 0 && a && b && c && lda >= k && ldc >= n && ldb >= (trans_b ? k : n), "lkg_gemm_skinny_f32: bad arguments");
-    LKG_REQUIRE(lkg_gemm_skinny_ok(m, n, k, a, lda, c, ldc), "lkg_gemm_skinny_f32: needs m >= 4096, k and n <= 64 in multiples "
-                "of 4 and 16-byte aligned rows (lkg_gemm_skinny_ok)");
+    LKG_REQUIRE(lkg_gemm_skinny_ok(m, n, k, a, lda, c, ldc), "lkg_gemm_skinny_f32: needs k and n <= 64 over m >= 4096 rows, or "
+                "n <= 64 < k <= 1024 with a weight panel that fits in LDS, in multiples of 4, and 16-byte aligned rows "
+                "(lkg_gemm_skinny_ok)");
     hipStream_t s = (hipStream_t)stream;
+    const int kind = lkg_gemm_skinny_kernel(m, n, k);
+    if (kind != 1) return lkg_internal_thin_launch(kind, m, n, k, a, lda, b, ldb, trans_b, beta, c, ldc, bias, s);
     const unsigned blocks = (unsigned)std::min<int64_t>((m + 63) / 64, 256 * 8);
 #define LKG_SKINNY(CPT_)                                                                                                    \
     hipLaunchKernelGGL((skinny_gemm_kernel<CPT_>), dim3(blocks), dim3(256), 0, s, (long)m, (int)n, (int)k, a, (long)lda, b,  \
diff --git a/literalkg_amd/csrc/lkg_graph_host.cpp b/literalkg_amd/csrc/lkg_graph_host.cpp
--- a/literalkg_amd/csrc/lkg_graph_host.cpp
+++ b/literalkg_amd/csrc/lkg_graph_host.cpp
@@ -50,9 +50,10 @@
 int lkg_internal_preload_negatives();
 int lkg_internal_preload_relation_loss();
 int lkg_internal_preload_gemm_ordered();
+int lkg_internal_preload_gemm_thin();
 
 extern "C" int lkg_preload(void) {
-    const int failed = lkg_internal_preload_spmm() + lkg_internal_preload_attention() + lkg_internal_preload_batch() + lkg_internal_preload_csr_device() + lkg_internal_preload_gemm() + lkg_internal_preload_gemm_tall() + lkg_internal_preload_gemm_wgrad() + lkg_internal_preload_rowwise() + lkg_internal_preload_score() + lkg_internal_preload_layer() + lkg_internal_preload_rank() + lkg_internal_preload_topk() + lkg_internal_preload_pairmlp() + lkg_internal_preload_triples() + lkg_internal_preload_relations() + lkg_internal_preload_accept() + lkg_internal_preload_retrieval() + lkg_internal_preload_softmax() + lkg_internal_preload_kvsall() + lkg_internal_preload_nssa() + lkg_internal_preload_negatives() + lkg_internal_preload_relation_loss() + lkg_internal_preload_gemm_ordered();
+    const int failed = lkg_internal_preload_spmm() + lkg_internal_preload_attention() + lkg_internal_preload_batch() + lkg_internal_preload_csr_device() + lkg_internal_preload_gemm() + lkg_internal_preload_gemm_tall() + lkg_internal_preload_gemm_wgrad() + lkg_internal_preload_rowwise() + lkg_internal_preload_score() + lkg_internal_preload_layer() + lkg_internal_preload_rank() + lkg_internal_preload_topk() + lkg_internal_preload_pairmlp() + lkg_internal_preload_triples() + lkg_internal_preload_relations() + lkg_internal_preload_accept() + lkg_internal_preload_retrieval() + lkg_internal_preload_softmax() + lkg_internal_preload_kvsall() + lkg_internal_preload_nssa() + lkg_internal_preload_negatives() + lkg_internal_preload_relation_loss() + lkg_internal_preload_gemm_ordered() + lkg_internal_preload_gemm_thin();
     if (failed) {
         lkg_set_error("lkg_preload: %d of the library's code objects could not be loaded on the current device", failed);
         return LKG_ERR_HIP;
diff --git a/literalkg_amd/ops.py b/literalkg_amd/ops.py
--- a/literalkg_amd/ops.py
+++ b/literalkg_amd/ops.py
@@ -199,7 +199,7 @@
     m, k = (a_.shape[1], a_.shape[0]) if trans_a else a_.shape
     n = b_.shape[0] if trans_b else b_.shape[1]
     out_ptr, out_ld = (N.ptr(out), _ld(out)) if out is not None else (None, n)
-    if (not trans_a and alpha == 1.0 and _ENGINE != "f32" and (k * n <= 2048 or m < TALL_MIN_ROWS)
+    if (not trans_a and alpha == 1.0 and _ENGINE != "f32" and _skinny_shape(m, n, k)
             and N.load().lkg_gemm_skinny_ok(m, n, k, N.ptr(a_), _ld(a_), out_ptr if out is not None else N.ptr(a_), out_ld)):
         return "skinny"
     if not trans_a and k > 0 and tall_ok(m, n, (k,), single_panel_too=tagged_rowmax(a) is not None):
@@ -211,6 +211,16 @@
             return "longk"
     need = int(N.load().lkg_gemm_workspace(int(trans_a), m, n, k)) if _ENGINE != "f32" else 0
     return GEMM_F32_ENGINES[int(N.load().lkg_gemm_f32_engine(int(trans_a), int(trans_b), m, n, k, need))]
+
+
+SKINNY_MIN_ROWS = 4096
+
+
+def _skinny_shape(m: int, n: int, k: int) -> bool:
+    kind = int(N.load().lkg_gemm_skinny_kernel(m, n, k))
+    if kind == 1:
+        return k * n <= 2048 or m < TALL_MIN_ROWS
+    return kind == 2 and m >= SKINNY_MIN_ROWS
 
 
 def gemm(a: torch.Tensor, b: torch.Tensor, trans_a: bool = False, trans_b: bool = False, alpha: float = 1.0,
@@ -236,7 +246,10 @@
     if engine == "tall_f16x2":
         return gemm_tall((a,), ((b,),), bool(trans_b), bias, alpha, beta, out)
     if engine == "smallm":
-        N.call("lkg_gemm_smallm_f32", m, n, k, N.ptr(a), _ld(a), N.ptr(b), _ld(b), N.ptr(out), _ld(out), _stream())
+        need = int(N.load().lkg_gemm_smallm_workspace(m, n, k))
+        ws = _workspace(4 * need, out.device)
+        N.call("lkg_gemm_smallm_f32", m, n, k, N.ptr(a), _ld(a), N.ptr(b), _ld(b), N.ptr(out), _ld(out), N.ptr(ws), need,
+               _stream())
         return out
     if engine == "longk":
         N.call("lkg_gemm_longk_f32", m, n, k, N.ptr(a), _ld(a), N.ptr(b), _ld(b), N.ptr(out), _ld(out), _stream())
@@ -889,9 +902,11 @@
 
 
 def _skinny(x: torch.Tensor, n_out: int) -> bool:
-    return (x.dim() == 2 and x.shape[0] >= 4096 and 4 <= x.shape[1] <= 64 and 4 <= n_out <= 64 and x.shape[1] % 4 == 0
-            and x.shape[1] * n_out <= 2048
-            and n_out % 4 == 0 and _ENGINE != "f32" and x.stride(1) == 1 and x.stride(0) % 4 == 0 and x.data_ptr() % 16 == 0)
+    if not (x.dim() == 2 and x.shape[0] >= SKINNY_MIN_ROWS and _ENGINE != "f32" and x.stride(1) == 1 and x.stride(0) % 4 == 0
+            and x.data_ptr() % 16 == 0):
+        return False
+    rows, k = x.shape
+    return (k * n_out <= 2048 or max(k, n_out) > 64) and _skinny_shape(rows, n_out, k)
 
 
 def linear(x, w, b=None):
```

After: 6.645 billion. Within noise of the previous version (-0.3%).
